# anneouyang/OuterSPACE

Hardware: AMD Instinct MI355X
Metric: spgemm_output_nnz_per_s (higher is better)
Workload: dtype f64

## Files before the change

### __graft_entry__.py

```python
import os
import subprocess
import sys

ROOT = os.path.dirname(os.path.abspath(__file__))
if ROOT not in sys.path:
    sys.path.insert(0, ROOT)


def build():
    subprocess.run(["make", "-C", os.path.join(ROOT, "outerspace_amd", "csrc"), "all"], check=True)
    subprocess.run(["make", "-C", os.path.join(ROOT, "oracle"), "all"], check=True)
    import outerspace_amd
    from outerspace_amd import _lib
    L = _lib.lib()
    missing = [s for s in _lib.EXPORTS + _lib.MASKED_EXPORTS + _lib.MCL_EXPORTS + _lib.APPLY_MASK_EXPORTS + _lib.SELECT_EXPORTS + _lib.EWISE_EXPORTS
               if not hasattr(L, s)]
    if missing:
        raise RuntimeError(f"library lacks exported symbols: {missing}")


def smoke():
    import numpy as np
    os.environ.setdefault("OSP_DIRECT_MIN_NNZ", "0")
    from outerspace_amd import generators as gen
    from outerspace_amd import spgemm as S
    from oracle import oracle

    n, rows, cols, vals = gen.rmat_coo(9, 8, "g500", seed=3)
    acsc = S.coo_to_csc(n, rows, cols, vals)
    bcsr = S.coo_to_csr(n, cols, rows, vals)
    with S.Context(0) as ctx:
        res = ctx.spgemm_csc_csr(n, n, n, *acsc, *bcsr)
        want = oracle.port().spgemm(n, n, n, *acsc, *bcsr)
        assert res.info["partials"] == want["partials"], (res.info["partials"], want["partials"])
        assert np.array_equal(res.rowptr, want["rowptr"]), "rowptr differs from the oracle"
        assert np.array_equal(res.colidx, want["colidx"]), "colidx differs from the oracle"
        assert np.array_equal(res.vals, want["vals"]), "values differ from the oracle"
        print(f"smoke ok: n={n} nnzA={len(rows)} P={res.info['partials']} nnzC={res.nnz} "
              f"heavy_rows={res.info['heavy_rows']} ms={res.info['ms_total']:.3f}")
        res.close()


if __name__ == "__main__":
    build()
    if len(sys.argv) > 1 and sys.argv[1] == "smoke":
        smoke()
```

### outerspace_amd/_lib.py

```python
import ctypes as C
import os

_HERE = os.path.dirname(os.path.abspath(__file__))
LIB_PATH = os.environ.get("OSP_LIBRARY") or os.path.join(_HERE, "libouterspace_spgemm.so")

OSP_F32, OSP_F64 = 0, 1
OSP_HOST, OSP_DEVICE = 0, 1
OSP_OK = 0
ERR_DIM, ERR_ARG, ERR_ALLOC, ERR_HIP, ERR_IO, ERR_RANGE, ERR_CAPACITY, ERR_UNSORTED = 1, 2, 3, 4, 5, 6, 7, 8
ERR_DUPLICATE = 233


class OspError(RuntimeError):
    def __init__(self, status, message):
        super().__init__(f"[osp status {status}] {message}")
        self.status = status


class _Stats(C.Structure):

    def as_dict(self):
        return {name: getattr(self, name) for name, _ in self._fields_ if name != "reserved"}


# ... 92 lines not shown

class Semiring(_Stats):
    _fields_ = [("add", C.c_int32), ("mul", C.c_int32), ("reserved", C.c_uint32 * 8)]


class MxmStats(_Stats):
    _fields_ = [("nnz_a", C.c_uint64), ("nnz_b", C.c_uint64), ("products", C.c_uint64), ("nnz_out", C.c_uint64),
                ("short_rows", C.c_uint64), ("long_rows", C.c_uint64), ("batches", C.c_uint32), ("launches", C.c_uint32),
                ("ms_total", C.c_float), ("reserved", C.c_uint32 * 7)]

MXV_ADD_OPS = {name: EWISE_OPS[name] for name in ("plus", "min", "max")}


class MxvStats(_Stats):
    _fields_ = [("nnz_in", C.c_uint64), ("nnz_out", C.c_uint64), ("long_segments", C.c_uint64), ("group", C.c_uint32),
                ("launches", C.c_uint32), ("ms_total", C.c_float), ("reserved", C.c_uint32 * 7)]

MXD_MAX_COLS = 65536


class MxdStats(_Stats):
    _fields_ = [("nnz_in", C.c_uint64), ("nnz_out", C.c_uint64), ("cols", C.c_uint64), ("long_segments", C.c_uint64),
                ("lanes_per_row", C.c_uint32), ("launches", C.c_uint32), ("ms_total", C.c_float), ("reserved", C.c_uint32 * 7)]

class Transpose(_Stats):
    _fields_ = [("reserved", C.c_uint32 * 8)]


class TransposeStats(_Stats):
    _fields_ = [("nnz", C.c_uint64), ("path", C.c_uint32), ("passes", C.c_uint32), ("launches", C.c_uint32), ("ms_total", C.c_float),
                ("reserved", C.c_uint32 * 6)]

class Extract(_Stats):
    _fields_ = [("rows", C.c_void_p), ("n_rows", C.c_uint64), ("cols", C.c_void_p), ("n_cols", C.c_uint64), ("space", C.c_int32),
                ("reserved", C.c_uint32 * 7)]


class ExtractStats(_Stats):
    _fields_ = [("nnz_in", C.c_uint64), ("nnz_gathered", C.c_uint64), ("nnz_out", C.c_uint64), ("ms_total", C.c_float),
                ("launches", C.c_uint32), ("readbacks", C.c_uint32), ("reserved", C.c_uint32 * 5)]

DUP_OPS = {"error": 0, "plus": 1, "min": 2, "max": 3, "first": 4, "last": 5, "count": 6}


class Build(_Stats):
    _fields_ = [("M", C.c_uint64), ("N", C.c_uint64), ("nnz", C.c_uint64), ("rows", C.c_void_p), ("cols", C.c_void_p), ("vals", C.c_void_p),
                ("dtype", C.c_int32), ("space", C.c_int32), ("dup", C.c_int32), ("reserved", C.c_uint32 * 7)]


class BuildStats(_Stats):
    _fields_ = [("nnz_in", C.c_uint64), ("nnz_out", C.c_uint64), ("long_runs", C.c_uint64), ("ms_total", C.c_float),
                ("launches", C.c_uint32), ("readbacks", C.c_uint32), ("reserved", C.c_uint32 * 5)]

PANEL_FN = C.CFUNCTYPE(C.c_int, C.POINTER(Panel), C.c_void_p)

MULTI_MAX_RANKS = 16


class MultiRankInfo(_Stats):
    _fields_ = [("device", C.c_int), ("k_begin", C.c_uint64), ("k_end", C.c_uint64), ("row_begin", C.c_uint64), ("row_end", C.c_uint64),
                ("partials_local", C.c_uint64), ("records_received", C.c_uint64), ("bytes_sent", C.c_uint64), ("nnz_c", C.c_uint64),
                ("ms_symbolic", C.c_float), ("ms_multiply_kernel", C.c_float), ("ms_merge", C.c_float), ("ms_total", C.c_float),
                ("bytes_to", C.c_uint64 * MULTI_MAX_RANKS), ("copy_streams", C.c_int), ("max_copies_outstanding", C.c_int),
                ("max_copies_in_flight", C.c_int), ("ms_exchange", C.c_float)]


class MultiInfo(_Stats):
    _fields_ = [("nranks", C.c_int), ("subpanels", C.c_int), ("M", C.c_uint64), ("K", C.c_uint64), ("N", C.c_uint64),
                ("nnz_c", C.c_uint64), ("partials", C.c_uint64), ("bytes_exchanged", C.c_uint64), ("ms_total", C.c_float),
                ("ms_upload", C.c_float), ("rank", MultiRankInfo * MULTI_MAX_RANKS)]

    def as_dict(self):
        d = {name: getattr(self, name) for name, _ in self._fields_ if name != "rank"}
        d["ranks"] = [{n: (list(getattr(self.rank[g], n))[:self.nranks] if n == "bytes_to" else getattr(self.rank[g], n))
                       for n, _ in MultiRankInfo._fields_} for g in range(self.nranks)]
        return d


EXPORTS = [
    "osp_context_create", "osp_context_create_on_stream", "osp_context_destroy", "osp_context_trim",
    "osp_config_default", "osp_last_error_string", "osp_status_string", "osp_spgemm_csc_csr", "osp_spgemm_csc_csr_panels",
    "osp_spgemm_coo", "osp_spgemm_csc_csr_aos", "osp_context_alloc", "osp_context_free",
    "osp_spgemm_partials", "osp_result_partials", "osp_merge_record_parts",
    "osp_merge_csr_parts", "osp_result_info", "osp_result_copy_csr", "osp_result_device_ptrs",
    "osp_result_destroy", "osp_mtx_read", "osp_host_free", "osp_coo_to_compressed_f32",
    "osp_coo_to_compressed_f64", "osp_spgemm_mtx", "osp_result_write_mtx", "osp_csr_bias_relu", "osp_result_coo_rows",
    "osp_stream_copy_probe", "osp_im2col_csc", "osp_spgemm_conv2d", "osp_csr_maxpool2d",
    "osp_multi_context_create", "osp_multi_context_destroy", "osp_multi_operands_create", "osp_multi_operands_destroy", "osp_spgemm_multi",
    "osp_spgemm_csc_csr_multi", "osp_multi_result_info", "osp_multi_result_shard", "osp_multi_result_copy_csr", "osp_multi_result_destroy",
]

MASKED_EXPORTS = ["osp_spgemm_masked"]

MCL_EXPORTS = ["osp_csr_inflate_prune"]

APPLY_MASK_EXPORTS = ["osp_csr_apply_mask"]

SELECT_EXPORTS = ["osp_csr_select"]

EWISE_EXPORTS = ["osp_csr_ewise"]

VECTOR_EXPORTS = ["osp_csr_reduce", "osp_csr_apply_vectors", "osp_csr_select_vertices"]

MXM_EXPORTS = ["osp_csr_mxm"]

TRANSPOSE_EXPORTS = ["osp_csr_transpose"]

MXV_EXPORTS = ["osp_csr_mxv"]

MXD_EXPORTS = ["osp_csr_mxd"]

EXTRACT_EXPORTS = ["osp_csr_extract"]

BUILD_EXPORTS = ["osp_csr_build"]

_lib = None


def lib():
    global _lib
    if _lib is not None:
        return _lib
    if not os.path.exists(LIB_PATH):
        raise ImportError(f"{LIB_PATH} not found: build it with `make -C outerspace_amd/csrc` "
                          "(or `python -c 'import __graft_entry__ as g; g.build()'`). "
                          "There is no CPU fallback.")
    try:
        import torch
    except ImportError:
        pass
    L = C.CDLL(LIB_PATH)
    vp, u64, i32 = C.c_void_p, C.c_uint64, C.c_int
    L.osp_last_error_string.restype = C.c_char_p
    L.osp_status_string.restype = C.c_char_p
    L.osp_status_string.argtypes = [i32]
    L.osp_context_create.argtypes = [i32, C.POINTER(vp)]
    L.osp_context_create_on_stream.argtypes = [i32, vp, C.POINTER(vp)]
    L.osp_context_destroy.argtypes = [vp]
    L.osp_context_trim.argtypes = [vp]
    L.osp_context_alloc.argtypes = [vp, u64, C.POINTER(vp)]
    L.osp_context_free.argtypes = [vp, vp]
    L.osp_spgemm_csc_csr_aos.argtypes = [vp, i32, u64, u64, u64, vp, vp, vp, vp, i32, C.POINTER(Config), C.POINTER(vp)]
    L.osp_config_default.argtypes = [C.POINTER(Config)]
    L.osp_config_default.restype = None
    L.osp_spgemm_csc_csr.argtypes = [vp, i32, u64, u64, u64, vp, vp, vp, vp, vp, vp, i32,
                                     C.POINTER(Config), C.POINTER(vp)]
    L.osp_spgemm_csc_csr_panels.argtypes = [vp, i32, u64, u64, u64, vp, vp, vp, vp, vp, vp, i32, C.POINTER(Config), PANEL_FN, vp,
                                            C.POINTER(ResultInfo)]
    L.osp_spgemm_coo.argtypes = [vp, i32, u64, u64, u64, u64, vp, vp, vp, u64, vp, vp, vp, i32, C.POINTER(Config), C.POINTER(vp)]
    L.osp_spgemm_partials.argtypes = [vp, i32, u64, u64, u64, vp, vp, vp, vp, vp, vp, i32, C.POINTER(Config), C.POINTER(vp)]
    L.osp_result_partials.argtypes = [vp, C.POINTER(vp), C.POINTER(vp)]
    L.osp_merge_record_parts.argtypes = [vp, i32, u64, u64, i32, C.POINTER(vp), C.POINTER(vp), i32, C.POINTER(Config), C.POINTER(vp)]
    L.osp_merge_csr_parts.argtypes = [vp, i32, u64, u64, i32, C.POINTER(vp), C.POINTER(vp),
                                      C.POINTER(vp), i32, C.POINTER(Config), C.POINTER(vp)]
    L.osp_result_info.argtypes = [vp, C.POINTER(ResultInfo)]
    L.osp_result_copy_csr.argtypes = [vp, vp, vp, vp, i32]
    L.osp_result_device_ptrs.argtypes = [vp, C.POINTER(vp), C.POINTER(vp), C.POINTER(vp)]
    L.osp_result_destroy.argtypes = [vp]
    L.osp_mtx_read.argtypes = [C.c_char_p, i32, C.POINTER(u64), C.POINTER(u64), C.POINTER(u64),
                               C.POINTER(vp), C.POINTER(vp), C.POINTER(vp)]
    L.osp_host_free.argtypes = [vp]
    L.osp_host_free.restype = None
    for sfx in ("f32", "f64"):
        getattr(L, f"osp_coo_to_compressed_{sfx}").argtypes = [i32, u64, u64, vp, vp, vp, vp, vp, vp]
    L.osp_spgemm_mtx.argtypes = [vp, i32, C.c_char_p, C.c_char_p, i32, C.POINTER(Config), C.POINTER(vp)]
    L.osp_result_write_mtx.argtypes = [vp, C.c_char_p]
    L.osp_stream_copy_probe.argtypes = [vp, u64, i32, C.POINTER(C.c_double)]
    L.osp_multi_context_create.argtypes = [C.POINTER(i32), i32, C.POINTER(vp)]
    L.osp_multi_context_destroy.argtypes = [vp]
    L.osp_multi_operands_create.argtypes = [vp, i32, u64, u64, u64, vp, vp, vp, vp, vp, vp, C.POINTER(vp)]
    L.osp_multi_operands_destroy.argtypes = [vp]
    L.osp_spgemm_multi.argtypes = [vp, vp, C.POINTER(Config), C.POINTER(vp)]
    L.osp_spgemm_csc_csr_multi.argtypes = [C.POINTER(i32), i32, i32, u64, u64, u64, vp, vp, vp, vp, vp, vp, C.POINTER(Config), C.POINTER(vp),
                                           C.POINTER(vp)]
    L.osp_multi_result_info.argtypes = [vp, C.POINTER(MultiInfo)]
    L.osp_multi_result_shard.argtypes = [vp, i32, C.POINTER(u64), C.POINTER(u64), C.POINTER(vp)]
    L.osp_multi_result_copy_csr.argtypes = [vp, vp, vp, vp]
    L.osp_multi_result_destroy.argtypes = [vp]
    L.osp_csr_bias_relu.argtypes = [vp, vp, i32, i32, C.POINTER(vp)]
    L.osp_result_coo_rows.argtypes = [vp, vp]
    L.osp_im2col_csc.argtypes = [vp, i32, u64, u64, u64, u64, u64, vp, vp, vp, i32, C.POINTER(Conv2dGeometry), i32, C.POINTER(u64),
                                 vp, vp, vp]
    L.osp_spgemm_conv2d.argtypes = [vp, i32, u64, u64, u64, u64, u64, vp, vp, vp, u64, u64, vp, vp, vp, i32, C.POINTER(Conv2dGeometry),
                                    C.POINTER(Config), C.POINTER(vp)]
    u32 = C.c_uint32
    L.osp_csr_maxpool2d.argtypes = [vp, u64, u64, u64, u32, u32, u32, u32, C.POINTER(vp)]
    L.osp_spgemm_masked.argtypes = [vp, i32, u64, u64, u64, vp, vp, vp, vp, vp, vp, vp, vp, i32, C.POINTER(Config), C.POINTER(vp)]
    L.osp_csr_inflate_prune.argtypes = [vp, C.POINTER(MclStep), i32, C.POINTER(vp), C.POINTER(MclStats)]
    L.osp_csr_apply_mask.argtypes = [vp, u64, u64, vp, vp, i32, i32, i32, C.POINTER(vp), C.POINTER(ApplyMaskStats)]
    L.osp_csr_select.argtypes = [vp, C.POINTER(Select), C.POINTER(vp), C.POINTER(SelectStats)]
    L.osp_csr_ewise.argtypes = [vp, vp, C.POINTER(Ewise), C.POINTER(vp), C.POINTER(EwiseStats)]
    L.osp_csr_reduce.argtypes = [vp, i32, i32, vp, i32, C.POINTER(VectorStats)]
    L.osp_csr_apply_vectors.argtypes = [vp, C.POINTER(VectorApply), vp, vp, i32, C.POINTER(vp), C.POINTER(VectorStats)]
    L.osp_csr_select_vertices.argtypes = [vp, vp, vp, i32, C.POINTER(vp), C.POINTER(VectorStats)]
    L.osp_csr_mxm.argtypes = [vp, vp, C.POINTER(Semiring), C.POINTER(vp), C.POINTER(MxmStats)]
    L.osp_csr_transpose.argtypes = [vp, C.POINTER(Transpose), C.POINTER(vp), C.POINTER(TransposeStats)]
    L.osp_csr_mxv.argtypes = [vp, C.POINTER(Semiring), vp, vp, i32, C.POINTER(MxvStats)]
    L.osp_csr_mxd.argtypes = [vp, C.POINTER(Semiring), vp, u64, vp, i32, C.POINTER(MxdStats)]
    L.osp_csr_extract.argtypes = [vp, C.POINTER(Extract), C.POINTER(vp), C.POINTER(ExtractStats)]
    L.osp_csr_build.argtypes = [vp, C.POINTER(Build), C.POINTER(vp), C.POINTER(BuildStats)]
    _lib = L
    return L


def check(status):
    if status != OSP_OK:
        raise OspError(status, lib().osp_last_error_string().decode(errors="replace"))
```

### outerspace_amd/csrc/osp_api.hip

```cpp
#include <hip/hip_runtime.h>

#include <algorithm>
#include <cmath>
#include <cstdarg>
#include <cstdio>
#include <cstdlib>
#include <chrono>
#include <cstring>
#include <functional>
#include <limits>
#include <map>
#include <memory>
#include <string>
#include <vector>

#include "../../include/outerspace_spgemm.h"
#include "../../include/outerspace_spgemm_masked.h"
#include "../../include/outerspace_spgemm_mcl.h"
#include "../../include/outerspace_spgemm_apply_mask.h"
#include "../../include/outerspace_spgemm_select.h"
#include "../../include/outerspace_spgemm_ewise.h"
#include "../../include/outerspace_spgemm_vector.h"
#include "../../include/outerspace_spgemm_mxm.h"
#include "../../include/outerspace_spgemm_transpose.h"
#include "../../include/outerspace_spgemm_mxv.h"
#include "../../include/outerspace_spgemm_mxd.h"
#include "../../include/outerspace_spgemm_extract.h"
#include "../../include/outerspace_spgemm_build.h"
#include "osp_internal.h"
#include "osp_kernels.h"
#include "osp_split.h"
#include "osp_sort.h"
#include "osp_epilogue.h"
#include "osp_conv.h"
#include "osp_masked.h"
#include "osp_mcl.h"
#include "osp_apply_mask.h"
#include "osp_select.h"
#include "osp_ewise.h"
#include "osp_vector.h"
#include "osp_mxm.h"
#include "osp_transpose.h"
#include "osp_mxv.h"
#include "osp_mxd.h"
#include "osp_extract.h"
#include "osp_build.h"

namespace osp {


#define OSP_HIP(expr)                                                                      \
    do {                                                                                   \
        hipError_t e_ = (expr);                                                            \
        if (e_ != hipSuccess)                                                              \
            throw Error(e_ == hipErrorOutOfMemory ? OSP_ERR_ALLOC : OSP_ERR_HIP,           \
                        std::string(#expr) + ": " + hipGetErrorString(e_));                \
    } while (0)

#include "osp_context.h"
#include "osp_pipeline.h"

template <class T>
static const T *to_device(Scratch &sc, const T *p, uint64_t n, osp_memspace_t space, hipStream_t s) {
    if (space == OSP_DEVICE || n == 0) return p;
    T *d = sc.get<T>(n);
    copy_h2d(d, p, n * sizeof(T), s);
    return d;
}

static void check_flags(uint32_t f, const char *what) {
    if (f & kFlagPtr) throw Error(OSP_ERR_ARG, std::string(what) + ": pointer array is not a monotone 0..nnz sequence");
    if (f & kFlagRange) throw Error(OSP_ERR_RANGE, std::string(what) + ": index outside its dimension");
    if (f & kFlagDuplicate) throw Error(OSP_ERR_DUPLICATE, std::string(what) + ": duplicate coordinate (reference: throw(233))");
    if (f & kFlagUnsorted) throw Error(OSP_ERR_UNSORTED, std::string(what) + ": indices inside a segment are not ascending");
}

static void finish_timing(Result *res, EventPair &ev, PhaseTimer &tm, hipStream_t s) {
    OSP_HIP(hipEventRecord(ev.b, s));
    OSP_HIP(hipStreamSynchronize(s));
    osp_result_info_t &i = res->info;
    i.ms_total = ev.ms();
    i.ms_symbolic = tm.total(PH_SYM);
    i.ms_multiply = tm.total(PH_MUL);
    i.ms_merge = tm.total(PH_MERGE);
    i.ms_compact = tm.total(PH_COMPACT);
    i.ms_multiply_kernel = tm.total(PH_MUL_K);
    i.ms_merge_kernel = tm.total(PH_MERGE_K);
    i.ms_split_kernel = tm.total(PH_SPLIT_K);
    i.ms_direct_plan_kernel = tm.total(PH_PLAN_K);
    i.ms_hub_plan_kernel = tm.total(PH_HUB_K);
    i.ms_expand_kernel = tm.total(PH_EXPAND_K);
}

__global__ void count_partials_kernel(const int64_t *a_colptr, const int64_t *b_rowptr, uint64_t K, unsigned long long *out) {
    __shared__ uint64_t scratch[256 / kWave + 1];
    uint64_t sum = 0;
    for (uint64_t k = (uint64_t)blockIdx.x * blockDim.x + threadIdx.x; k < K; k += (uint64_t)gridDim.x * blockDim.x)
        sum += (uint64_t)(a_colptr[k + 1] - a_colptr[k]) * (uint64_t)(b_rowptr[k + 1] - b_rowptr[k]);
    uint64_t total;
    block_excl_scan<uint64_t, 256>(sum, scratch, &total);
    if (threadIdx.x == 0 && total) atomicAdd(out, (unsigned long long)total);
}

template <class T>
static void spgemm_impl(Context *ctx, Result *res, uint64_t M, uint64_t K, uint64_t N, const int64_t *a_colptr_in,
                        const uint32_t *a_rowidx_in, const T *a_vals_in, const int64_t *b_rowptr_in,
                        const uint32_t *b_colidx_in, const T *b_vals_in, osp_memspace_t space,
                        const osp_config_t &cfg, const PanelSink *sink = nullptr, bool partials_only = false) {
    hipStream_t s = ctx->stream;
    Scratch sc(ctx);
    PhaseTimer tm(s);
    EventPair ev;
    OSP_HIP(hipEventRecord(ev.a, s));
// ... 68 lines not shown
            const uint64_t nsample = (k1 - k0 + stride - 1) / stride;
            if (nnz) row_work_kernel<<<grid_for(nsample * kWave, 256), 256, 0, s>>>(a_colptr, a_rowidx, b_rowptr, k0, k1, stride, work);
            device_exclusive_scan<LoadU64, uint64_t>(LoadU64{(const uint64_t *)work}, M, pre, tmp, s);
            device_exclusive_scan<RowCost, uint64_t>(RowCost{pre, (uint64_t)TileCap<T>::value, kSplitRowMax}, M, cost_pre, tmp, s);
            shard_bounds_kernel<<<grid_for(G + 1, 64), 64, 0, s>>>(cost_pre, pre, M, G, d_b, d_b + G + 1);
            std::vector<uint64_t> h_b(2ull * (G + 1));
            copy_d2h(h_b.data(), d_b, h_b.size() * sizeof(uint64_t), s);
            r_lo = h_b[cfg.row_shard_index];
            r_hi = h_b[cfg.row_shard_index + 1];
        }
        int64_t *colptr2 = sc.get<int64_t>(K + 1);
        uint64_t nnz2 = 0;
        uint32_t *rowidx2 = nullptr;
        T *vals2 = nullptr;
        {
            Scratch cs(ctx);
            uint32_t *keep_scan = cs.get<uint32_t>(nnz + 1);
            uint32_t *tmp = cs.get<uint32_t>(scan_scratch_entries(nnz + 1));
            const RowInRange keep{a_rowidx + e0, (uint32_t)r_lo, r_hi};
            device_exclusive_scan<RowInRange, uint32_t>(keep, nnz, keep_scan, tmp, s);
            nnz2 = d2h(keep_scan + nnz, s);
            rowidx2 = sc.get<uint32_t>(nnz2);
            vals2 = sc.get<T>(nnz2);
            restrict_colptr_kernel<<<grid_for(K + 1, 256), 256, 0, s>>>(a_colptr, K, e0, nnz, keep_scan, colptr2);
            if (nnz2) restrict_compact_kernel<T><<<grid_for(nnz, 256), 256, 0, s>>>(keep, keep_scan, nnz, a_vals + e0, rowidx2, vals2);
        }
        tm.end(PH_SYM);
        a_colptr = colptr2; a_rowidx = rowidx2; a_vals = vals2;
        e0 = 0;
        e1 = (int64_t)nnz2;
    }
    const uint64_t nnz = (uint64_t)(e1 - e0);

    tm.begin(PH_SYM);
    uint64_t *row_off = sc.get<uint64_t>(M + 1);
    uint64_t *chunk_off = sc.get<uint64_t>(nnz);
    uint64_t P = 0;
    const int algo = cfg.algorithm;
    if (algo != OSP_ALGO_OUTER && algo != OSP_ALGO_ROWWISE) throw Error(OSP_ERR_ARG, "unknown algorithm");
    const bool rowwise = algo == OSP_ALGO_ROWWISE && nnz && (uint64_t)nnz_b < 0xffffffffull && nnz < 0xffffffffull && !partials_only;
    ChunkTable<T> ct{};
    const uint64_t direct_min_nnz = getenv("OSP_DIRECT_MIN_NNZ") ? strtoull(getenv("OSP_DIRECT_MIN_NNZ"), nullptr, 10) : ((getenv("OSP_GATHER") && atoi(getenv("OSP_GATHER")) == 0) ? (8ull << 20) : (2ull << 20));
    const bool dense_avg = (long double)p_all * 8.0L >= 3.0L * (long double)M * (long double)N;
    const bool direct = nnz && (nnz >= direct_min_nnz || dense_avg) && (uint64_t)nnz_b < 0xffffffffull && nnz < 0xffffffffull && !partials_only &&
                        !(getenv("OSP_DIRECT") && atoi(getenv("OSP_DIRECT")) == 0);
    const uint64_t direct_max = std::min<uint64_t>(getenv("OSP_DIRECT_MAX") ? strtoull(getenv("OSP_DIRECT_MAX"), nullptr, 10) : kSplitRowMax,
                                                   kDirectDenseMax);
    const int gather_env = getenv("OSP_GATHER") ? atoi(getenv("OSP_GATHER")) : 2;
    const bool gather_ok = nnz && !rowwise && !partials_only && (uint64_t)nnz_b < 0xffffffffull && nnz < 0xffffffffull;
    const bool gather_short = gather_ok && gather_env >= 2 && direct;
    ShortRuns<T> srun{};
    DirectSrc dsrc{};
    uint32_t n_long_rows = 1;
    if (nnz == 0) {
        OSP_HIP(hipMemsetAsync(row_off, 0, (M + 1) * sizeof(uint64_t), s));
    } else {
        Scratch ss(ctx);
        Scratch &keep = (rowwise || direct || gather_short) ? sc : ss;
        const RowSort rs(ss, nnz, std::max(1, bits_for(M)));
        uint32_t *rows_sorted = (gather_short ? keep : ss).template get<uint32_t>(nnz), *perm = keep.get<uint32_t>(nnz), *w_sorted = ss.get<uint32_t>(nnz);
        uint32_t *bs_sorted = (rowwise || direct || gather_short) ? keep.get<uint32_t>(nnz) : nullptr;
        uint32_t *rowfirst = keep.get<uint32_t>(M + 1);
        uint64_t *offs_sorted = keep.get<uint64_t>(nnz + 1);
        uint64_t *scan_tmp = ss.get<uint64_t>(scan_scratch_entries(std::max<uint64_t>(nnz, M + 1)));
        const bool table = rowwise || direct || gather_short;
        const bool with_av = gather_ok && gather_env >= 1 && (direct || gather_short);
        T *av_sorted = with_av ? keep.get<T>(nnz) : nullptr;
        uint32_t *w = ss.get<uint32_t>(with_av ? 4 * nnz : table ? 2 * nnz : nnz);
        uint32_t *bs = table ? w : nullptr;
        sym_chunk_len_kernel<<<grid_for(nnz, 256), 256, 0, s>>>(a_colptr, b_rowptr, k0, k1, e0, nnz, w, bs,
                                                                with_av ? reinterpret_cast<const uint32_t *>(a_vals) : nullptr, (uint32_t)(sizeof(T) / 4));
        SymEpilogue sym_ep{w, bs, rows_sorted, perm, w_sorted, bs_sorted};
        if (with_av) { sym_ep.av_sorted = av_sorted; sym_ep.vwords = (uint32_t)(sizeof(T) / 4); }
        rs.sort(a_rowidx + e0, sym_ep);
        device_exclusive_scan<LoadU32As64, uint64_t>(LoadU32As64{w_sorted}, nnz, offs_sorted, scan_tmp, s);
        sym_row_offsets_kernel<<<grid_for(M + 1, 256), 256, 0, s>>>(rows_sorted, offs_sorted, nnz, M, row_off, rowfirst);
        const uint64_t rw_cap = (rowwise || gather_short) ? (uint64_t)TileCap<T>::value : 0ull;
        const bool expand_rows_on = gather_short && !(getenv("OSP_EXPAND_ROWS") && atoi(getenv("OSP_EXPAND_ROWS")) == 0);
        if (!expand_rows_on) sym_scatter_offsets_kernel<<<grid_for(nnz, 256), 256, 0, s>>>(perm, offs_sorted, rows_sorted, row_off, rw_cap, nnz, chunk_off);
        if (partials_only || rowwise || row_sharded) P = d2h(offs_sorted + nnz, s);
        else P = kPartialsOnDevice;
        if (direct) {
            dsrc = DirectSrc{rowfirst, offs_sorted, bs_sorted, perm, b_colidx, chunk_off, direct_max};
            dsrc.b_rowptr = b_rowptr; dsrc.K = K; dsrc.nnz_b = (uint64_t)nnz_b; dsrc.keep = &sc;
            dsrc.gather = gather_ok && gather_env >= 1;
            dsrc.expand_rows = expand_rows_on;
            if (expand_rows_on) { dsrc.chunk_off_ready = false; dsrc.rows_sorted = rows_sorted; dsrc.row_off = row_off; dsrc.rw_cap = rw_cap; dsrc.nnz = nnz; }
            dsrc.a_vals = with_av ? (const void *)av_sorted : (const void *)(a_vals + e0); dsrc.av_in_order = with_av; dsrc.b_vals = b_vals;
            if (dsrc.gather) {
                dsrc.gstat = (unsigned long long *)sc.get<uint64_t>(3);
                zero_async(s, {{dsrc.gstat, 3 * sizeof(uint64_t)}});
            }
        }
        if (gather_short) {
            const ShortRunFlag sf{offs_sorted};
            uint32_t *cidx = ss.get<uint32_t>(nnz + 1), *cidx_tmp = ss.get<uint32_t>(scan_scratch_entries(nnz + 1));
            device_exclusive_scan<ShortRunFlag, uint32_t>(sf, nnz, cidx, cidx_tmp, s);
            RunDesc<T> *runs0 = sc.get<RunDesc<T>>(nnz);
            uint32_t *rowfirst0 = sc.get<uint32_t>(M + 1);
            short_runs_kernel<T><<<grid_for(nnz, 256), 256, 0, s>>>(sf, cidx, nnz, bs_sorted, av_sorted, runs0);
            short_rowfirst_kernel<<<grid_for(M + 1, 256), 256, 0, s>>>(rowfirst, cidx, M, rowfirst0);
            srun = ShortRuns<T>{runs0, rowfirst0, b_colidx, b_vals};
        }
        if (rowwise) {
            ct = ChunkTable<T>{offs_sorted, bs_sorted, perm, rowfirst, a_vals + e0, b_colidx, b_vals, (uint32_t)rw_cap, 1u};
            uint32_t *flag_scan = ss.get<uint32_t>(M + 1);
            device_exclusive_scan<HeavyRowFlag, uint32_t>(HeavyRowFlag{row_off, 0, (uint32_t)rw_cap}, M, flag_scan, (uint32_t *)scan_tmp, s);
            n_long_rows = d2h(flag_scan + M, s);
        }
    }
    tm.end(PH_SYM);
    res->info.partials = P;

    OuterProducer<T> prod;
    prod.ctx = ctx; prod.res = res;
    prod.a_colptr = a_colptr; prod.a_rowidx = a_rowidx; prod.a_vals = a_vals;
    prod.b_rowptr = b_rowptr; prod.b_colidx = b_colidx; prod.b_vals = b_vals;
    prod.k0 = k0; prod.k1 = k1; prod.e0 = e0; prod.chunk_off = chunk_off;
    const uint64_t nk = k1 - k0;
    prod.a_start = sc.get<int64_t>(nk); prod.a_cnt = sc.get<uint32_t>(nk);
    prod.prod = sc.get<uint64_t>(nk); prod.prod_off = sc.get<uint64_t>(nk + 1);
    prod.scan_tmp = sc.get<uint64_t>(scan_scratch_entries(nk));
    prod.nothing_staged = rowwise && n_long_rows == 0;
    prod.short_gathered = gather_short;
    if ((dsrc.gather || gather_short) && nnz && !partials_only) {
        prod.nnz = nnz;
        prod.kscan = sc.get<uint32_t>(nnz + 1);
        prod.kscan_tmp = sc.get<uint32_t>(scan_scratch_entries(std::max<uint64_t>(nnz, k1 - k0) + 1));
        prod.elist = sc.get<uint32_t>(nnz);
        prod.cscan = sc.get<uint32_t>(k1 - k0 + 1);
        prod.klist = sc.get<uint32_t>(k1 - k0 + 1);
    }

    if (partials_only) {
        if (row_sharded) throw Error(OSP_ERR_ARG, "partial products of a row shard are not supported");
        res->partials = true;
        res->rowptr = (int64_t *)ctx->alloc((M + 1) * sizeof(int64_t));
        OSP_HIP(hipMemcpyAsync(res->rowptr, row_off, (M + 1) * sizeof(uint64_t), hipMemcpyDeviceToDevice, s));
        res->vals = ctx->alloc(std::max<uint64_t>(P, 1) * sizeof(Part<T>));
        res->info.panels = 1;
        res->info.nnz_c = P;
        res->info.row_begin = 0;
        res->info.row_end = M;
        tm.begin(PH_MUL);
        if (P) prod.produce(0, M, true, 0, P, (Part<T> *)res->vals, tm, nullptr, nullptr);
        tm.end(PH_MUL);
        finish_timing(res, ev, tm, s);
        return;
    }
    const uint64_t off_lo = 0, P_rows = P;
    merge_pipeline<T>(ctx, res, prod, M, N, row_off, P_rows, cfg.partial_capacity, tm, r_lo, r_hi, off_lo, sink,
                      rowwise ? &ct : nullptr, (direct && nnz) ? &dsrc : nullptr, nullptr, gather_short ? &srun : nullptr);

    finish_timing(res, ev, tm, s);
    if (gather_short) res->info.gathered_short_partials = res->info.partials - res->info.heavy_partials;
    if (dsrc.gstat && res->info.direct_rows) {
        uint64_t gs[3] = {0, 0, 0};
        copy_d2h(gs, dsrc.gstat, sizeof(gs), s);
        res->info.gathered_rows = gs[0]; res->info.gathered_partials = gs[1]; res->info.gathered_runs = gs[2];
    }
    if (getenv("OSP_VERBOSE")) {
        fprintf(stderr, "[osp] product done in %.1f ms; pool misses so far: %llu hipMalloc calls, %.1f GB, %.1f ms\n", res->info.ms_total,
                (unsigned long long)ctx->malloc_calls, ctx->malloc_bytes / 1e9, ctx->malloc_ms);
    }
}

template <class T>
static void coo_to_compressed_device(Context *ctx, Scratch &sc, uint64_t nseg, uint64_t ninner, uint64_t nnz, const uint32_t *seg,
                                     const uint32_t *inner, const T *vals, const char *what, int64_t **ptr_out,
                                     uint32_t **idx_out, T **val_out) {
    hipStream_t s = ctx->stream;
    int64_t *ptr = sc.get<int64_t>(nseg + 1);
    uint32_t *idx = sc.get<uint32_t>(nnz);
    T *ov = sc.get<T>(nnz);
    *ptr_out = ptr; *idx_out = idx; *val_out = ov;
    if (nnz == 0) {
        OSP_HIP(hipMemsetAsync(ptr, 0, (nseg + 1) * sizeof(int64_t), s));
        return;
    }
    Scratch ss(ctx);
    uint32_t *flags = ss.get<uint32_t>(1);
    OSP_HIP(hipMemsetAsync(flags, 0, sizeof(uint32_t), s));
    const CooOrder o = coo_sort_two_keys(ss, nnz, inner, std::max(1, bits_for(ninner)), seg, std::max(1, bits_for(nseg)));
    ingest_finish_kernel<T><<<grid_for(nnz, 256), 256, 0, s>>>(o.outer_sorted, o.perm, inner, vals, nnz, nseg, ninner, idx, ov, flags);
    ingest_ptr_kernel<<<grid_for(nseg + 1, 256), 256, 0, s>>>(o.outer_sorted, nnz, nseg, ptr);
    check_flags(d2h(flags, s), what);
}

template <class T>
static void spgemm_coo_impl(Context *ctx, Result *res, uint64_t M, uint64_t K, uint64_t N, uint64_t nnz_a, const uint32_t *a_rows,
                            const uint32_t *a_cols, const T *a_vals, uint64_t nnz_b, const uint32_t *b_rows, const uint32_t *b_cols,
                            const T *b_vals, osp_memspace_t space, const osp_config_t &cfg) {
    hipStream_t s = ctx->stream;
    Scratch sc(ctx);
    EventPair ev;
    OSP_HIP(hipEventRecord(ev.a, s));
    const uint32_t *ar = to_device(sc, a_rows, nnz_a, space, s), *ac = to_device(sc, a_cols, nnz_a, space, s);
    const uint32_t *br = to_device(sc, b_rows, nnz_b, space, s), *bc = to_device(sc, b_cols, nnz_b, space, s);
    const T *av = to_device(sc, a_vals, nnz_a, space, s), *bv = to_device(sc, b_vals, nnz_b, space, s);
    int64_t *ap, *bp;
    uint32_t *ai, *bi;
    T *acv, *bcv;
    coo_to_compressed_device<T>(ctx, sc, K, M, nnz_a, ac, ar, av, "A (COO)", &ap, &ai, &acv);
    coo_to_compressed_device<T>(ctx, sc, K, N, nnz_b, br, bc, bv, "B (COO)", &bp, &bi, &bcv);
    OSP_HIP(hipEventRecord(ev.b, s));
// ... 712 lines not shown
        on_device(ctx, [&] {
            const ConvGeom g = conv_geometry(N, C, H, W, geom);
            hipStream_t s = ctx->stream;
            Scratch sc(ctx);
            with_type(dtype, [&](auto tag) {
                using T = decltype(tag);
                const uint32_t *xr = to_device(sc, x_rows, nnz_x, space, s), *xc = to_device(sc, x_cols, nnz_x, space, s);
                const T *xv = to_device(sc, (const T *)x_vals, nnz_x, space, s);
                T *va = (T *)a_vals;
                *nnz_a = im2col_impl<T>(ctx, sc, N, C, g, nnz_x, xr, xc, xv, fill, a_colptr, a_rowidx, va);
            });
        });
        return OSP_OK;
    });
}

int osp_spgemm_conv2d(osp_context_t ctx_, osp_dtype_t dtype, uint64_t N, uint64_t C, uint64_t H, uint64_t W, uint64_t nnz_x,
                      const uint32_t *x_rows, const uint32_t *x_cols, const void *x_vals, uint64_t OC, uint64_t nnz_w,
                      const uint32_t *w_rows, const uint32_t *w_cols, const void *w_vals, osp_memspace_t space,
                      const osp_conv2d_geometry_t *geom, const osp_config_t *cfg_, osp_result_t *result) {
    Context *ctx = (Context *)ctx_;
    if (!ctx || !result) return fail(OSP_ERR_ARG, "null context or result pointer");
    if ((nnz_x && (!x_rows || !x_cols || !x_vals)) || (nnz_w && (!w_rows || !w_cols || !w_vals))) return fail(OSP_ERR_ARG, "null operand array");
    return guard([&] {
        check_dtype(dtype); check_space(space);
        if (!OC || OC > 0xffffffffull || nnz_x >= 0xffffffffull || nnz_w >= 0xffffffffull)
            throw Error(OSP_ERR_ARG, "OC must be >= 1; OC or nnz exceeds the u32 index type");
        const osp_config_t cfg = config_or_default(cfg_);
        return new_result(ctx, dtype, result, [&](auto tag, Result *res) {
            using T = decltype(tag);
            const ConvGeom g = conv_geometry(N, C, H, W, geom);
            spgemm_conv2d_impl<T>(ctx, res, N, C, g, nnz_x, x_rows, x_cols, (const T *)x_vals, OC, nnz_w, w_rows, w_cols, (const T *)w_vals,
                                  space, cfg);
        });
    });
}

int osp_csr_maxpool2d(osp_result_t in_, uint64_t N, uint64_t H, uint64_t W, uint32_t kh, uint32_t kw, uint32_t stride_h,
                      uint32_t stride_w, osp_result_t *out) {
    Result *in = (Result *)in_;
    if (!in || !out) return fail(OSP_ERR_ARG, "null argument");
    if (in->partials) return fail(OSP_ERR_ARG, "a result of osp_spgemm_partials holds records, not a CSR");
    if (!N || !H || !W || !kh || !kw || !stride_h || !stride_w) return fail(OSP_ERR_ARG, "sizes, kernel and stride must be >= 1");
    if (H < kh || W < kw) return fail(OSP_ERR_ARG, "the pooling window is larger than the input: empty output");
    if (H >= 0xffffffffull || W >= 0xffffffffull || (unsigned __int128)N * H * W != in->info.M)
        return fail(OSP_ERR_ARG, "N*H*W must equal the rows of the input");
    return guard([&] {
        return new_result(in->ctx, in->dtype, out, [&](auto tag, Result *res) {
            maxpool_impl<decltype(tag)>(in->ctx, in, res, N, (uint32_t)H, (uint32_t)W, kh, kw, stride_h, stride_w);
        });
    });
}

int osp_stream_copy_probe(osp_context_t ctx_, uint64_t bytes, int reps, double *gbps) {
    Context *ctx = (Context *)ctx_;
    if (!ctx || !gbps) return fail(OSP_ERR_ARG, "null argument");
    if (bytes < 4096 || reps < 1 || reps > 1000) return fail(OSP_ERR_ARG, "bytes >= 4096, 1 <= reps <= 1000");
    return guard([&]() -> int {
        OSP_HIP(hipSetDevice(ctx->device));
        hipStream_t s = ctx->stream;
        Scratch sc(ctx);
        const uint64_t n = bytes / sizeof(u32x4);
        u32x4 *src = sc.get<u32x4>(n), *dst = sc.get<u32x4>(n);
        OSP_HIP(hipMemsetAsync(src, 0x5a, n * sizeof(u32x4), s));
        if (n > 0xffffffffull * 256ull) return fail(OSP_ERR_ARG, "probe buffer too large");
        const unsigned grid = (unsigned)((n + 255) / 256);
        double best = 0;
        for (int nt = 0; nt < 2; nt++) {
            for (int i = 0; i < 2; i++) {
                if (nt) stream_copy_kernel<true><<<grid, 256, 0, s>>>(src, dst, n); else stream_copy_kernel<false><<<grid, 256, 0, s>>>(src, dst, n);
            }
            EventPair ev;
            OSP_HIP(hipEventRecord(ev.a, s));
            for (int i = 0; i < reps; i++) {
                if (nt) stream_copy_kernel<true><<<grid, 256, 0, s>>>(src, dst, n); else stream_copy_kernel<false><<<grid, 256, 0, s>>>(src, dst, n);
            }
            OSP_HIP(hipEventRecord(ev.b, s));
            OSP_HIP(hipStreamSynchronize(s));
            OSP_HIP(hipGetLastError());
            const double ms = ev.ms();
            if (ms > 0) best = std::max(best, 2.0 * (double)(n * sizeof(u32x4)) * reps / (ms * 1e-3) / 1e9);
        }
        *gbps = best;
        return OSP_OK;
    });
}

int osp_multi_context_create(const int *devices, int ndev, osp_multi_context_t *out) {
    if (!devices || !out) return fail(OSP_ERR_ARG, "null argument");
    if (ndev < 1 || ndev > OSP_MULTI_MAX_RANKS) return fail(OSP_ERR_ARG, "between 1 and %d ranks", OSP_MULTI_MAX_RANKS);
    return guard([&]() -> int {
        std::unique_ptr<MultiContext> mc(new MultiContext);
        for (int g = 0; g < ndev; g++) {
            osp_context_t c = nullptr;
            const int st = osp_context_create(devices[g], &c);
            if (st) return st;
            mc->devices.push_back(devices[g]);
            mc->ctx.push_back((Context *)c);
            mc->copy.emplace_back((size_t)ndev, nullptr);
            mc->mctx.push_back(nullptr);
            osp_context_t c2 = nullptr;
            const int st2 = osp_context_create(devices[g], &c2);
            if (st2) return st2;
            mc->mctx.back() = (Context *)c2;
            mc->ctx.back()->sibling = mc->mctx.back();
            mc->mctx.back()->sibling = mc->ctx.back();
// ... 182 lines not shown
```

### outerspace_amd/csrc/osp_context.h

```cpp
#pragma once

struct Context {
    int device = 0;
    hipStream_t stream = nullptr;
    bool own_stream = false;
    hipStream_t aux = nullptr;
    hipEvent_t aux_fork = nullptr, aux_join = nullptr;
    void need_aux() {
        if (aux) return;
        if (hipStreamCreateWithFlags(&aux, hipStreamNonBlocking) != hipSuccess) { aux = nullptr; throw Error(OSP_ERR_HIP, "hipStreamCreate failed"); }
        if (hipEventCreateWithFlags(&aux_fork, hipEventDisableTiming) != hipSuccess || hipEventCreateWithFlags(&aux_join, hipEventDisableTiming) != hipSuccess) {
            drop_aux();
            throw Error(OSP_ERR_HIP, "hipEventCreate failed");
        }
    }
    bool fork_window = false;
    uint64_t releases_in_fork_window = 0;
    void drop_aux() {
        if (aux) { (void)hipStreamSynchronize(aux); (void)hipStreamDestroy(aux); aux = nullptr; }
        if (aux_fork) { (void)hipEventDestroy(aux_fork); aux_fork = nullptr; }
        if (aux_join) { (void)hipEventDestroy(aux_join); aux_join = nullptr; }
    }
    std::multimap<size_t, void *> free_list;
    std::map<void *, size_t> live;
// ... 331 lines not shown
    for (size_t off = 0; off < bytes; off += chunk, i ^= 1) {
        const size_t n = std::min(chunk, bytes - off);
        OSP_HIP(hipMemcpyAsync(pb.p + i * chunk, (const char *)src + off, n, hipMemcpyDeviceToHost, s));
        OSP_HIP(hipEventRecord(pb.done[i], s));
        if (have_prev) {
            OSP_HIP(hipEventSynchronize(pb.done[i ^ 1]));
            memcpy((char *)dst + off_prev, pb.p + (i ^ 1) * chunk, n_prev);
        }
        off_prev = off; n_prev = n; have_prev = true;
    }
    OSP_HIP(hipEventSynchronize(pb.done[i ^ 1]));
    memcpy((char *)dst + off_prev, pb.p + (i ^ 1) * chunk, n_prev);
}
struct ZeroRegions {
    uint32_t *p[4];
    uint64_t words[4];
    uint32_t val[4];
};
__global__ void zero_regions_kernel(const ZeroRegions z) {
#pragma unroll
    for (int r = 0; r < 4; r++)
        for (uint64_t i = (uint64_t)blockIdx.x * blockDim.x + threadIdx.x; i < z.words[r]; i += (uint64_t)gridDim.x * blockDim.x) z.p[r][i] = z.val[r];
}
struct FillRegion { void *p; size_t bytes; uint32_t word; };
static void fill_async(hipStream_t s, std::initializer_list<FillRegion> regions) {
    ZeroRegions z{};
    int n = 0;
    uint64_t most = 0;
    for (auto &r : regions) {
        if (n == 4 || (r.bytes & 3) || ((uintptr_t)r.p & 3)) throw Error(OSP_ERR_ARG, "fill_async: at most four word-aligned regions");
        z.p[n] = (uint32_t *)r.p;
        z.words[n] = r.bytes / 4;
        z.val[n] = r.word;
        most = std::max<uint64_t>(most, z.words[n]);
        n++;
    }
    if (most == 0) return;
    zero_regions_kernel<<<(unsigned)std::min<uint64_t>((most + 255) / 256, 2048), 256, 0, s>>>(z);
}
static void zero_async(hipStream_t s, std::initializer_list<std::pair<void *, size_t>> regions) {
    ZeroRegions z{};
    int n = 0;
    uint64_t most = 0;
    for (auto &r : regions) {
        if (n == 4 || (r.second & 3) || ((uintptr_t)r.first & 3)) throw Error(OSP_ERR_ARG, "zero_async: at most four word-aligned regions");
        z.p[n] = (uint32_t *)r.first;
        z.words[n] = r.second / 4;
        most = std::max<uint64_t>(most, z.words[n]);
        n++;
    }
    if (most == 0) return;
    zero_regions_kernel<<<(unsigned)std::min<uint64_t>((most + 255) / 256, 2048), 256, 0, s>>>(z);
}
constexpr int kGatherMax = 24;
struct GatherSrcs {
    const void *p[kGatherMax];
    uint8_t bytes[kGatherMax];
};
__global__ void gather_scalars_kernel(const GatherSrcs g, int n, uint64_t *out) {
    const int i = threadIdx.x;
    if (i < n) out[i] = g.bytes[i] == 8 ? *static_cast<const uint64_t *>(g.p[i]) : (uint64_t) * static_cast<const uint32_t *>(g.p[i]);
}
struct Gather {
    hipStream_t s;
    Pinned &pb;
    GatherSrcs srcs;
    void *dst[kGatherMax];
    int n = 0;
    explicit Gather(hipStream_t st) : s(st), pb(pinned_buffer()) { pb.reserve(4096); }
    template <class T> void add(T *host_dst, const T *dptr) {
        static_assert(sizeof(T) == 4 || sizeof(T) == 8, "read-backs are 32- or 64-bit scalars");
        if (n == kGatherMax) throw Error(OSP_ERR_ARG, "too many values in one read-back");
        srcs.p[n] = dptr;
        srcs.bytes[n] = (uint8_t)sizeof(T);
        dst[n++] = host_dst;
    }
    void wait() {
        if (n == 0) return;
        uint64_t *pin = reinterpret_cast<uint64_t *>(pb.p);
        if (n >= 3) {
            if (!pb.collect) OSP_HIP(hipMalloc((void **)&pb.collect, kGatherMax * sizeof(uint64_t)));
            gather_scalars_kernel<<<1, kWave, 0, s>>>(srcs, n, pb.collect);
            OSP_HIP(hipMemcpyAsync(pin, pb.collect, n * sizeof(uint64_t), hipMemcpyDeviceToHost, s));
        } else {
            for (int i = 0; i < n; i++) OSP_HIP(hipMemcpyAsync(pin + i, srcs.p[i], srcs.bytes[i], hipMemcpyDeviceToHost, s));
        }
        OSP_HIP(hipStreamSynchronize(s));
        for (int i = 0; i < n; i++) memcpy(dst[i], pin + i, srcs.bytes[i]);
        n = 0;
    }
};
template <class T> static T d2h(const T *dptr, hipStream_t s) {
    T v;
    copy_d2h(&v, dptr, sizeof(T), s);
    return v;
}
```

### outerspace_amd/csrc/osp_kernels.h

```cpp
#pragma once
#include <type_traits>
#include "osp_prims.h"

namespace osp {

template <class T> struct TileCap;
#ifndef OSP_TILE_CAP_F32
#define OSP_TILE_CAP_F32 1792
#endif
template <> struct TileCap<float> { static constexpr int value = OSP_TILE_CAP_F32; };
#ifndef OSP_TILE_CAP_F64
#define OSP_TILE_CAP_F64 1536
#endif
template <> struct TileCap<double> { static constexpr int value = OSP_TILE_CAP_F64; };
constexpr int kMergeThreads = 256;
constexpr int kTileMaxRows = kMergeThreads - 1;
constexpr int kMulThreads = 256;
#ifndef OSP_MUL_PER_WAVE
#define OSP_MUL_PER_WAVE 2048
#endif
constexpr int kMulPerWave = OSP_MUL_PER_WAVE;
constexpr int kMulPerBlock = kMulPerWave * (kMulThreads / kWave);
#ifndef OSP_MUL_BATCH_MAX
#define OSP_MUL_BATCH_MAX 4096
// ... 168 lines not shown
                                       uint64_t *row_off, uint32_t *rowfirst) {
    uint64_t i = (uint64_t)blockIdx.x * blockDim.x + threadIdx.x;
    if (i > M) return;
    uint64_t t = lower_bound_dev(rows_sorted, 0, nnz, (uint64_t)i);
    row_off[i] = offs_sorted[t];
    rowfirst[i] = (uint32_t)t;
}
struct LenGatherW {
    const uint32_t *w;
    const uint32_t *perm;
    __device__ uint32_t operator()(uint64_t t) const { return w[perm[t]]; }
};

__global__ void panel_columns_kernel(const int64_t *a_colptr, const uint32_t *a_rowidx,
                                     const int64_t *b_rowptr, uint64_t k0, uint64_t nk, uint32_t r0,
                                     uint64_t r1, int whole, int64_t *a_start, uint32_t *a_cnt,
                                     uint64_t *prod) {
    uint64_t t = (uint64_t)blockIdx.x * blockDim.x + threadIdx.x;
    if (t >= nk) return;
    uint64_t k = k0 + t;
    uint64_t lo = (uint64_t)a_colptr[k], hi = (uint64_t)a_colptr[k + 1];
    if (!whole) {
        uint64_t l2 = lower_bound_dev(a_rowidx, lo, hi, (uint64_t)r0);
        hi = lower_bound_dev(a_rowidx, l2, hi, r1);
        lo = l2;
    }
    a_start[t] = (int64_t)lo;
    a_cnt[t] = (uint32_t)(hi - lo);
    prod[t] = (hi - lo) * (uint64_t)(b_rowptr[k + 1] - b_rowptr[k]);
}
__global__ void panel_bounds_kernel(const uint64_t *row_off, uint64_t r_lo, uint64_t M, uint64_t cap, const uint64_t *cuts, uint32_t ncuts,
                                    uint32_t maxp, uint64_t *out) {
    const uint64_t *off = row_off + r_lo;
    uint64_t r = 0, bad = ~0ull;
    uint32_t p = 0, ci = 0;
    if (lane_id() == 0) { out[2] = r_lo; out[2 + maxp + 1] = off[0]; }
    while (r < M) {
        if (p == maxp) { bad = r_lo + r; break; }
        uint64_t r1 = wave_upper_bound(off, r, M + 1, off[r] + cap) - 1;
        if (r1 <= r) { bad = r_lo + r; break; }
        r1 = min(r1, M);
        while (ci < ncuts && cuts[ci] <= r_lo + r) ci++;
        if (ci < ncuts && cuts[ci] < r_lo + r1) r1 = cuts[ci] - r_lo;
        p++;
        if (lane_id() == 0) { out[2 + p] = r_lo + r1; out[2 + maxp + 1 + p] = off[r1]; }
        r = r1;
    }
    if (lane_id() == 0) { out[0] = p; out[1] = bad; }
}
struct LoadU64 {
    const uint64_t *p;
    __device__ uint64_t operator()(uint64_t i) const { return p[i]; }
};
struct PanelKeepFlag {
    const uint32_t *a_rowidx; const uint64_t *chunk_off; int64_t e0; uint32_t r0; uint64_t r1; uint32_t desc_only;
    __device__ uint32_t operator()(uint64_t t) const {
        const uint32_t r = a_rowidx[(uint64_t)e0 + t];
        if (!(r >= r0 && (uint64_t)r < r1)) return 0u;
        const uint64_t off = chunk_off[t];
        return (off != ~0ull && (!desc_only || (off >> 63))) ? 1u : 0u;
    }
};
__global__ void panel_keep_list_kernel(PanelKeepFlag f, const uint32_t *kscan, uint64_t nnz, uint32_t *elist) {
    const uint64_t t = (uint64_t)blockIdx.x * blockDim.x + threadIdx.x;
    if (t < nnz && f(t)) elist[kscan[t]] = (uint32_t)((uint64_t)f.e0 + t);
}
struct PanelKeepColFlag {
    const int64_t *a_colptr; int64_t e0; uint64_t k0; const uint32_t *kscan;
    __device__ uint32_t operator()(uint64_t t) const { return kscan[a_colptr[k0 + t + 1] - e0] != kscan[a_colptr[k0 + t] - e0] ? 1u : 0u; }
};
__global__ void panel_keep_columns_kernel(const int64_t *a_colptr, const int64_t *b_rowptr, uint64_t k0, uint64_t nk, int64_t e0,
                                          const uint32_t *kscan, const uint32_t *cscan, int64_t *a_start, uint32_t *a_cnt, uint64_t *prod,
                                          uint32_t *klist) {
    const uint64_t t = (uint64_t)blockIdx.x * blockDim.x + threadIdx.x;
    if (t >= nk) return;
    const uint64_t k = k0 + t;
    const uint32_t lo = kscan[a_colptr[k] - e0], hi = kscan[a_colptr[k + 1] - e0];
    const uint32_t ncol = cscan[nk];
    if (t >= ncol) { a_start[t] = 0; a_cnt[t] = 0; prod[t] = 0; klist[t] = (uint32_t)k0; }
    if (hi == lo) return;
    const uint32_t j = cscan[t];
    a_start[j] = (int64_t)lo;
    a_cnt[j] = hi - lo;
    prod[j] = (uint64_t)(hi - lo) * (uint64_t)(b_rowptr[k + 1] - b_rowptr[k]);
    klist[j] = (uint32_t)k;
}

__device__ __forceinline__ uint32_t wave_bcast(uint32_t v, uint32_t src) { return (uint32_t)__builtin_amdgcn_readlane((int)v, (int)src); }
__device__ __forceinline__ uint64_t wave_bcast(uint64_t v, uint32_t src) {
    return ((uint64_t)wave_bcast((uint32_t)(v >> 32), src) << 32) | wave_bcast((uint32_t)v, src);
}
__device__ __forceinline__ float wave_bcast(float v, uint32_t src) { return __uint_as_float(wave_bcast(__float_as_uint(v), src)); }
__device__ __forceinline__ double wave_bcast(double v, uint32_t src) {
    return __longlong_as_double((long long)wave_bcast((uint64_t)__double_as_longlong(v), src));
}

constexpr uint64_t kDirectBit = 1ull << 63;
__device__ __forceinline__ uint64_t direct_desc(uint32_t rowbase, uint32_t celloff, uint32_t sh) {
    return kDirectBit | ((uint64_t)(sh & 31u) << 58) | ((uint64_t)(celloff & 0x3ffffffu) << 32) | (uint64_t)rowbase;
}
constexpr uint64_t kHubCellMask = (1ull << 58) - 1ull;
__device__ __forceinline__ uint64_t hub_desc(uint64_t first_cell) { return kDirectBit | (31ull << 58) | (first_cell & kHubCellMask); }
__device__ __forceinline__ bool is_hub_desc(uint64_t desc) { return ((uint32_t)(desc >> 58) & 31u) == 31u; }
struct HubArgs {
    const uint32_t *cells = nullptr;
    const uint32_t *sx = nullptr;
// ... 403 lines not shown
                            [&](uint64_t i, uint32_t col, T val) { stream_store_part(&stage[i - base], col, val); });
}

struct CoarseStartFlag {
    const uint64_t *row_off;
    uint64_t r0, base, slot;
    const uint8_t *force;
    __device__ uint32_t operator()(uint64_t t) const {
        if (t == 0) return 1;
        const uint64_t r = r0 + t;
        if (force && force[t]) return 1;
        return ((row_off[r] - base) / slot != (row_off[r - 1] - base) / slot || (t & 0xffffu) == 0) ? 1u : 0u;
    }
};
__global__ void tile_walk_kernel(const uint32_t *cb_rows, const uint32_t *ncb_p, uint32_t ncb_max, uint64_t r_end, const uint64_t *row_off,
                                 uint64_t cap, uint32_t max_rows, const uint32_t *tile_base, uint32_t *counts,
                                 uint32_t *tile_rows) {
    const uint32_t j = blockIdx.x * blockDim.x + threadIdx.x;
    const uint32_t ncb = *ncb_p;
    if (j >= ncb) {
        if (!tile_rows && j < ncb_max) counts[j] = 0;
        return;
    }
    uint64_t r = cb_rows[j];
    const uint64_t end = (j + 1 < ncb) ? (uint64_t)cb_rows[j + 1] : r_end;
    uint32_t n = 0;
    const uint32_t out = tile_rows ? tile_base[j] : 0u;
    while (r < end) {
        if (tile_rows) tile_rows[out + n] = (uint32_t)r;
        const uint64_t lim = min(end, r + max_rows);
        uint64_t r2 = upper_bound_dev(row_off, r + 1, lim + 1, row_off[r] + cap) - 1;
        if (r2 <= r) r2 = r + 1;
        r = r2;
        n++;
    }
    if (!tile_rows) counts[j] = n;
}
struct HeavyRowFlag {
    const uint64_t *row_off;
    uint64_t r0;
    uint32_t kTileCap;
    __device__ uint32_t operator()(uint64_t t) const {
        const uint64_t r = r0 + t;
        return (row_off[r + 1] - row_off[r]) > (uint64_t)kTileCap ? 1u : 0u;
    }
};
template <class F>
__global__ void compact_flagged_kernel(F f, const uint32_t *scan, uint64_t n, uint64_t r0,
                                       uint32_t *list) {
    uint64_t t = (uint64_t)blockIdx.x * blockDim.x + threadIdx.x;
    if (t < n && f(t)) list[scan[t]] = (uint32_t)(r0 + t);
}

constexpr uint64_t kStatusAgg = 1ull << 62, kStatusPrefix = 2ull << 62, kStatusMask = (1ull << 62) - 1;

#ifndef OSP_RUN_SHORT
#define OSP_RUN_SHORT 16
#endif
constexpr int kRunShort = OSP_RUN_SHORT;
template <class T> __device__ __forceinline__ T index_as_value(uint32_t i);
template <> __device__ __forceinline__ float index_as_value<float>(uint32_t i) { return __uint_as_float(i); }
template <> __device__ __forceinline__ double index_as_value<double>(uint32_t i) { return __longlong_as_double((long long)i); }
__device__ __forceinline__ uint32_t value_as_index_impl(float v) { return __float_as_uint(v); }
__device__ __forceinline__ uint32_t value_as_index_impl(double v) { return (uint32_t)__double_as_longlong(v); }
template <class T> __device__ __forceinline__ uint32_t value_as_index(T v) { return value_as_index_impl(v); }
#ifndef OSP_DIGIT_BITS
#define OSP_DIGIT_BITS 10
#endif
constexpr int kDigitBits = OSP_DIGIT_BITS;
constexpr int kDigits = 1 << kDigitBits;

template <class T, int NT, int CAP = TileCap<T>::value>
struct alignas(8) MergeSmem {
    static constexpr int kTileCap = CAP;
    static_assert(CAP % 4 == 0, "the value area behind key0/pos0 must stay 8-byte aligned");
    static_assert(sizeof(T) <= 8, "values alias 8 bytes per entry");
    static constexpr bool kWide = sizeof(T) == 8;
#ifndef OSP_HASH_IN_CNT
#define OSP_HASH_IN_CNT 1
#endif
    static constexpr uint32_t kHashWords = (kWide ? (uint32_t)CAP * 5u / 2u : (uint32_t)CAP * 2u) +
                                           (OSP_HASH_IN_CNT ? (kWide ? 0u : 2u) + (uint32_t)(NT / kWave) * (1u << OSP_DIGIT_BITS) / 2u : 0u);
    uint32_t key0[CAP];
    uint16_t pos0[CAP];
    uint16_t pad[kWide ? CAP : 4];
    uint32_t key1[CAP];
    uint16_t pos1[CAP];
    union {
        uint16_t cnt[NT / kWave][kDigits];
        uint16_t rank[CAP + 1];
    };
    uint32_t rowo[kTileMaxRows + 1];
    uint32_t gbits[CAP / 32];
    uint32_t scratch[NT / kWave + 1];
    uint32_t nlongrun;
    uint32_t hcount;
    uint64_t excl;
    __device__ __forceinline__ uint32_t *key(int c) { return c ? key1 : key0; }
    __device__ __forceinline__ uint16_t *pos(int c) { return c ? pos1 : pos0; }
    __device__ __forceinline__ T *vals(int c) {
        return reinterpret_cast<T *>(c ? reinterpret_cast<char *>(key0) : kWide ? reinterpret_cast<char *>(pad) : reinterpret_cast<char *>(key1));
    }
    __device__ __forceinline__ uint32_t *htab() { return reinterpret_cast<uint32_t *>(pos0); }
    static constexpr int kMaxLong = CAP / kRunShort;
    static constexpr size_t kLongOff = ((CAP + 1) * sizeof(uint16_t) + 7) / 8 * 8;
    static_assert(kLongOff + kMaxLong * (sizeof(T) + sizeof(uint16_t)) <= sizeof(uint16_t) * (NT / kWave) * kDigits, "long-run list: behind rank, inside the counters");
    __device__ __forceinline__ T *long_sum() { return reinterpret_cast<T *>(reinterpret_cast<char *>(cnt) + kLongOff); }
    __device__ __forceinline__ uint16_t *long_pos() { return reinterpret_cast<uint16_t *>(reinterpret_cast<char *>(cnt) + kLongOff + kMaxLong * sizeof(T)); }
};

template <int BITS>
__device__ __forceinline__ void wave_match_digit(unsigned digit, bool valid, unsigned &rank, unsigned &count) {
    const uint64_t vm = __ballot(valid);
    uint32_t plo = (uint32_t)vm, phi = (uint32_t)(vm >> 32);
#pragma unroll
    for (int b = 0; b < BITS; b++) {
        const uint32_t bit = (digit >> b) & 1u;
        const uint64_t m = __ballot(bit != 0);
        const uint32_t sbm = 0u - bit;
        plo &= ~((uint32_t)m ^ sbm);
        phi &= ~((uint32_t)(m >> 32) ^ sbm);
    }
    rank = __builtin_amdgcn_mbcnt_hi(phi, __builtin_amdgcn_mbcnt_lo(plo, 0u));
    count = __popc(plo) + __popc(phi);
}

__global__ __launch_bounds__(256) void rank_order_selftest_kernel(uint32_t *bad) {
    __shared__ uint32_t cnt[4][64];
    const unsigned tid = threadIdx.x, lane = lane_id(), w = tid >> 6;
    uint32_t x = 0x9E3779B9u * (blockIdx.x * 256u + tid + 1u), nbad = 0;
    for (int r = 0; r < 64; r++) {
        cnt[w][lane] = 0;
        for (int it = 0; it < 4; it++) {
            x ^= x << 13; x ^= x >> 17; x ^= x << 5;
            const unsigned dg = (x >> 9) & ((r & 1) ? 3u : 127u);
            const bool valid = ((x >> 27) & 7u) != 0;
            unsigned rk, c;
            wave_match_digit<7>(dg, valid, rk, c);
            const unsigned half = 16u * (dg & 1u);
            const uint32_t before = (cnt[w][dg >> 1] >> half) & 0xffffu;
            __builtin_amdgcn_wave_barrier();
            if (valid) {
                const uint32_t got = (atomicAdd(&cnt[w][dg >> 1], 1u << half) >> half) & 0xffffu;
                nbad += got != before + rk;
            }
        }
    }
    if (nbad) atomicAdd(bad, nbad);
}

constexpr int kLookWin = 1;
__device__ __forceinline__ void lookback_publish(uint64_t *status, uint32_t t, uint64_t total) {
    __hip_atomic_store(&status[t], (t == 0 ? kStatusPrefix : kStatusAgg) | total, __ATOMIC_RELAXED, __HIP_MEMORY_SCOPE_AGENT);
}
constexpr int kTicketStride = 32;
constexpr uint32_t kLookbackSpinLimit = 1u << 22;
__device__ __forceinline__ uint32_t take_ticket(uint32_t *ticket, uint32_t nshards, uint32_t &shard, uint32_t ntiles) {
    if (nshards <= 1) return atomicAdd(ticket, 1u);
    for (uint32_t tries = 0; tries < nshards; tries++) {
        const uint32_t n = atomicAdd(&ticket[shard * kTicketStride], 1u);
        const uint64_t t = (uint64_t)n * nshards + shard;
        if (t < ntiles) return (uint32_t)t;
        shard = shard + 1 == nshards ? 0u : shard + 1;
    }
    return ntiles;
}
template <bool PUBLISH = true>
__device__ __forceinline__ uint64_t lookback_prefix(uint64_t *status, uint32_t t, uint64_t total, uint32_t *abort_word = nullptr) {
    const unsigned lane = lane_id();
    if (PUBLISH && lane == 0) lookback_publish(status, t, total);
    uint64_t excl = 0;
    int64_t b = (int64_t)t - 1;
    uint32_t spins = 0;
    while (b >= 0) {
        uint64_t sv[kLookWin];
#pragma unroll
        for (int j = 0; j < kLookWin; j++) {
            const int64_t idx = b - (int64_t)(j * kWave) - (int64_t)lane;
            sv[j] = kStatusPrefix;
            if (idx >= 0) sv[j] = __hip_atomic_load(&status[idx], __ATOMIC_RELAXED, __HIP_MEMORY_SCOPE_AGENT);
        }
        bool done = false, retry = false;
        uint64_t part = 0;
#pragma unroll
        for (int j = 0; j < kLookWin; j++) {
            if (!done && !retry) {
                const uint64_t m_prefix = __ballot((sv[j] >> 62) == 2), m_empty = __ballot((sv[j] >> 62) == 0);
                const int p = m_prefix ? __builtin_ctzll(m_prefix) : 64;
                const uint64_t need = p >= 63 ? ~0ull : ((2ull << p) - 1ull);
                if (m_empty & need) {
                    retry = true;
                } else {
                    part += ((int)lane <= p) ? (sv[j] & kStatusMask) : 0ull;
                    if (p < 64) done = true;
                }
            }
        }
        if (retry) {
            __builtin_amdgcn_s_sleep(1);
            if (abort_word && (++spins & 255u) == 0) {
                if (spins >= kLookbackSpinLimit && lane == 0) atomicExch(abort_word, 1u);
                if (spins >= kLookbackSpinLimit || __hip_atomic_load(abort_word, __ATOMIC_RELAXED, __HIP_MEMORY_SCOPE_AGENT) != 0u) break;
            }
            continue;
        }
        excl += wave_reduce_sum_u62(part);
        if (done) break;
        b -= (int64_t)kLookWin * kWave;
    }
    if (lane == 0 && t != 0)
        __hip_atomic_store(&status[t], kStatusPrefix | (excl + total), __ATOMIC_RELAXED, __HIP_MEMORY_SCOPE_AGENT);
    return excl;
}

struct TileDesc {
    uint64_t s;
    uint32_t ra, nr, n, lvl;
    uint32_t cbase, kbits;
    uint32_t rbeg, rcnt;
};
constexpr uint32_t kNoRuns = 0xffffffffu;
template <class T> struct RunDesc;
template <> struct alignas(16) RunDesc<double> { uint32_t dst, src; double av; };
template <> struct alignas(4) RunDesc<float> { uint32_t dst, src; float av; };
template <class T>
struct GatherArgs {
    const RunDesc<T> *runs = nullptr;
    const RunDesc<T> *runs0 = nullptr;
    const uint32_t *b_colidx = nullptr;
    const T *b_vals = nullptr;
};
struct ShortRunFlag {
    const uint64_t *off;
    __device__ uint32_t operator()(uint64_t c) const { return off[c + 1] > off[c] ? 1u : 0u; }
};
template <class T>
__global__ void short_runs_kernel(ShortRunFlag f, const uint32_t *cidx, uint64_t nnz, const uint32_t *bs, const T *av_sorted, RunDesc<T> *runs0) {
    const uint64_t c = (uint64_t)blockIdx.x * blockDim.x + threadIdx.x;
    if (c >= nnz || !f(c)) return;
    RunDesc<T> rd;
    rd.dst = (uint32_t)f.off[c];
    rd.src = bs[c];
    rd.av = av_sorted[c];
    runs0[cidx[c]] = rd;
}
__global__ void short_rowfirst_kernel(const uint32_t *rowfirst, const uint32_t *cidx, uint64_t M, uint32_t *rowfirst0) {
    const uint64_t i = (uint64_t)blockIdx.x * blockDim.x + threadIdx.x;
    if (i <= M) rowfirst0[i] = cidx[rowfirst[i]];
}
struct SegExpandJobs {
    const uint32_t *seglist; const uint64_t *vrow_off; const uint32_t *vrun_off;
    __device__ uint64_t operator()(uint64_t t) const {
        const uint32_t v = seglist[t];
        if (vrun_off[v] == kNoRuns) return 0ull;
        return (vrow_off[v + 1] - vrow_off[v] + kExpandJob - 1) / kExpandJob;
    }
};
template <class T>
__global__ __launch_bounds__(kExpandThreads) void expand_segments_kernel(
    const uint32_t *__restrict__ seglist, uint32_t nseg, const uint64_t *__restrict__ jobbase, const uint64_t *__restrict__ vrow_off,
    const uint32_t *__restrict__ vrun_off, const uint32_t *__restrict__ vrun_end, const RunDesc<T> *__restrict__ runs,
    const uint32_t *__restrict__ b_colidx, const T *__restrict__ b_vals, Part<T> *__restrict__ qstage) {
    const unsigned lane = lane_id(), w = threadIdx.x >> 6;
    constexpr uint32_t NW = kExpandThreads / kWave, per = kExpandJob / NW, kUnroll = 4;
    const uint64_t njobs = jobbase[nseg];
// ... 1182 lines not shown
```

### outerspace_amd/csrc/osp_pipeline.h

```cpp
#pragma once

#define OSP_WITH_RA(ctx_, ...)                                               \
    do {                                                                     \
        if ((ctx_)->rank_atomic) { constexpr bool RA = true; __VA_ARGS__; }  \
        else { constexpr bool RA = false; __VA_ARGS__; }                     \
    } while (0)

template <class T> struct Producer {
    virtual ~Producer() {}
    virtual void produce(uint64_t r0, uint64_t r1, bool whole, uint64_t base, uint64_t count,
                         Part<T> *stage, PhaseTimer &tm, const uint32_t *cells = nullptr, Part<T> *qstage = nullptr,
                         const HubArgs *hub = nullptr, bool compact = false, bool has_long = true, bool desc_only = false, bool walk_all = false) = 0;
};

template <class T> struct MergeIO {
    Part<T> *stage;
    const uint64_t *row_off; uint64_t r0, r1, base;
    int64_t *c_rowptr; uint32_t *c_col; T *c_val;
    const uint64_t *out_in; uint64_t *out_out;
    ChunkTable<T> ct{};
    uint32_t *abort_word = nullptr;
    const RunDesc<T> *runs0 = nullptr; const uint32_t *rowfirst0 = nullptr; const uint32_t *b_colidx = nullptr; const T *b_vals = nullptr;
};
template <class T> struct ShortRuns {
    const RunDesc<T> *runs0 = nullptr; const uint32_t *rowfirst0 = nullptr; const uint32_t *b_colidx = nullptr; const T *b_vals = nullptr;
};

struct TilePlan {
    uint32_t *tile_rows = nullptr;
    uint32_t ntiles = 0;
    uint32_t *long_rows = nullptr;
    uint32_t nlong = 0;
};

static TilePlan plan_tiles(Context *ctx, Scratch &sc, const uint64_t *row_off, uint64_t r0, uint64_t r1, uint64_t base,
                           uint32_t cap, uint32_t max_rows, const uint8_t *force_start, uint64_t total, uint64_t nforce) {
    hipStream_t s = ctx->stream;
    const uint64_t nr = r1 - r0;
    TilePlan pl;
    uint32_t *flag_scan = sc.get<uint32_t>(nr + 1);
    uint32_t *tmp_rows = sc.get<uint32_t>(nr + 1);
    uint64_t *scan_tmp = sc.get<uint64_t>(scan_scratch_entries(std::max<uint64_t>(nr + 1, 16)));
    const uint64_t slot = 8ull * cap;
    CoarseStartFlag csf{row_off, r0, base, slot, force_start};
    device_exclusive_scan<CoarseStartFlag, uint32_t>(csf, nr, flag_scan, (uint32_t *)scan_tmp, s);
    compact_flagged_kernel<CoarseStartFlag><<<grid_for(nr, 256), 256, 0, s>>>(csf, flag_scan, nr, r0, tmp_rows);
    const uint32_t ncb = (uint32_t)std::min<uint64_t>(nr, 2 + nforce + total / slot + nr / 65536);
    const uint32_t *ncb_p = flag_scan + nr;
    uint32_t *cb_cnt = sc.get<uint32_t>((uint64_t)ncb + 1);
    tile_walk_kernel<<<grid_for(ncb, 128), 128, 0, s>>>(tmp_rows, ncb_p, ncb, r1, row_off, cap, max_rows, nullptr, cb_cnt, nullptr);
    device_exclusive_scan<LoadU32, uint32_t>(LoadU32{cb_cnt}, ncb, cb_cnt, (uint32_t *)scan_tmp, s);
    HeavyRowFlag hrf{row_off, r0, cap};
    uint32_t *long_scan = sc.get<uint32_t>(nr + 1);
    uint32_t *long_tmp = sc.get<uint32_t>(scan_scratch_entries(std::max<uint64_t>(nr + 1, 16)));
    device_exclusive_scan<HeavyRowFlag, uint32_t>(hrf, nr, long_scan, long_tmp, s);
    pl.long_rows = sc.get<uint32_t>(nr + 1);
    compact_flagged_kernel<HeavyRowFlag><<<grid_for(nr, 256), 256, 0, s>>>(hrf, long_scan, nr, r0, pl.long_rows);
    { Gather g(s); g.add(&pl.ntiles, (const uint32_t *)cb_cnt + ncb); g.add(&pl.nlong, (const uint32_t *)long_scan + nr); g.wait(); }
    pl.tile_rows = sc.get<uint32_t>((uint64_t)pl.ntiles + 1);
    tile_walk_kernel<<<grid_for(ncb, 128), 128, 0, s>>>(tmp_rows, ncb_p, ncb, r1, row_off, cap, max_rows, cb_cnt, nullptr, pl.tile_rows);
    return pl;
}

struct DirectSrc {
    const uint32_t *rowfirst; const uint64_t *off; const uint32_t *bs; const uint32_t *perm; const uint32_t *b_colidx;
    uint64_t *chunk_off;
    uint64_t direct_max;
    const int64_t *b_rowptr = nullptr;
    uint64_t K = 0, nnz_b = 0;
    Scratch *keep = nullptr;
    mutable HubTables hub{};
    mutable bool hub_refused = false;
    bool gather = false;
    bool expand_rows = false;
    mutable bool chunk_off_ready = true;
    const uint32_t *rows_sorted = nullptr;
    const uint64_t *row_off = nullptr;
    uint64_t rw_cap = 0, nnz = 0;
    void ensure_chunk_off(hipStream_t s) const {
        if (chunk_off_ready) return;
        sym_scatter_offsets_kernel<<<grid_for(nnz, 256), 256, 0, s>>>(perm, off, rows_sorted, row_off, rw_cap, nnz, chunk_off);
        chunk_off_ready = true;
    }
    const void *a_vals = nullptr, *b_vals = nullptr;
    bool av_in_order = false;
    unsigned long long *gstat = nullptr;
};

template <class T> struct PanelPlan {
    Scratch sc;
    TilePlan p0;
    uint32_t max_rows = 0;
    uint64_t *hoff = nullptr, *hscan_tmp = nullptr, *blkbase = nullptr, *hbase = nullptr, *vbase = nullptr, *cellbase = nullptr;
    uint8_t *hbits = nullptr, *hmode = nullptr;
    uint32_t *nstretch = nullptr;
    uint64_t nh = 0, nblocks = 0, nvirt = 0, ncell = 0;
    uint64_t mode_rows[3] = {0, 0, 0}, mode_partials[3] = {0, 0, 0};
    uint32_t *ghist = nullptr, *ghist_tmp = nullptr;
    Part<T> *qstage = nullptr;
    uint64_t *vrow_off = nullptr;
    uint8_t *vfirst = nullptr;
    uint32_t *vcol0 = nullptr, *vcol1 = nullptr;
    uint32_t *cells = nullptr;
    HubArgs hub{};
    GatherArgs<T> ga{};
    uint32_t *vrun_off = nullptr, *vrun_end = nullptr;
    uint32_t *nwritten = nullptr;
    uint64_t *xjobbase = nullptr;
    uint64_t xjobs_bound = 0, xpartials = 0;
    bool expand_ok = false;
    bool may_write = false;
    const DirectSrc *split_from_b = nullptr;
    bool split_beside = false;
    explicit PanelPlan(Context *c) : sc(c) {}
};

__global__ void mode_totals_kernel(const uint32_t *rows, uint32_t nlong, const uint64_t *row_off, const uint8_t *hmode,
                                   const uint8_t *hsmall, unsigned long long *totals) {
    uint64_t part[3] = {0, 0, 0}, cnt[3] = {0, 0, 0}, nsmall = 0;
    for (uint32_t h = blockIdx.x * blockDim.x + threadIdx.x; h < nlong; h += gridDim.x * blockDim.x) {
        const uint64_t U = row_off[rows[h] + 1] - row_off[rows[h]];
        const uint8_t m = hmode[h];
        nsmall += hsmall[h] ? 1ull : 0ull;
#pragma unroll
        for (int mode = 0; mode < 3; mode++) { part[mode] += m == mode ? U : 0ull; cnt[mode] += m == mode ? 1ull : 0ull; }
    }
    for (uint8_t mode = 0; mode < 3; mode++) {
        const uint64_t p = wave_reduce_sum<uint64_t>(part[mode]), c = wave_reduce_sum<uint64_t>(cnt[mode]);
        if (lane_id() == 0 && c) { atomicAdd(&totals[mode], (unsigned long long)c); atomicAdd(&totals[3 + mode], (unsigned long long)p); }
    }
    nsmall = wave_reduce_sum<uint64_t>(nsmall);
    if (lane_id() == 0 && nsmall) atomicAdd(&totals[6], (unsigned long long)nsmall);
}

template <class T>
static void plan_panel(Context *ctx, Result *res, PhaseTimer &tm, PanelPlan<T> &pl, const uint64_t *row_off, uint64_t r0, uint64_t r1,
                       uint64_t base, uint64_t count, int colbits, const DirectSrc *ds) {
    hipStream_t s = ctx->stream;
    Scratch &sc = pl.sc;
    constexpr uint32_t kCap = (uint32_t)TileCap<T>::value;
    pl.max_rows = (uint32_t)std::min<uint64_t>(kTileMaxRows, colbits >= 32 ? 1ull : (1ull << (32 - colbits)));
    pl.p0 = plan_tiles(ctx, sc, row_off, r0, r1, base, kCap, pl.max_rows, nullptr, count, 0);
    res->info.light_tiles += pl.p0.ntiles - pl.p0.nlong;
    if (!pl.p0.nlong) return;
    const uint32_t nlong = pl.p0.nlong;
    pl.hoff = sc.get<uint64_t>((uint64_t)nlong + 1);
    pl.hscan_tmp = sc.get<uint64_t>(scan_scratch_entries(nlong));
    device_exclusive_scan<HeavyLen, uint64_t>(HeavyLen{pl.p0.long_rows, row_off}, nlong, pl.hoff, pl.hscan_tmp, s);
    pl.hbits = sc.get<uint8_t>(nlong);
    pl.hmode = sc.get<uint8_t>(nlong);
    pl.nstretch = sc.get<uint32_t>(nlong);
    uint32_t *nseg = sc.get<uint32_t>(nlong);
    uint64_t *nhist = sc.get<uint64_t>(nlong), *ncellh = sc.get<uint64_t>(nlong);
    const bool want_gather = ds && ds->gather;
    uint64_t *nrund = want_gather ? sc.get<uint64_t>(nlong) : nullptr, *rdbase = want_gather ? sc.get<uint64_t>((uint64_t)nlong + 1) : nullptr;
    uint64_t nrd = 0;
    pl.blkbase = sc.get<uint64_t>((uint64_t)nlong + 1); pl.hbase = sc.get<uint64_t>((uint64_t)nlong + 1);
    pl.vbase = sc.get<uint64_t>((uint64_t)nlong + 1); pl.cellbase = sc.get<uint64_t>((uint64_t)nlong + 1);
    unsigned long long *totals = (unsigned long long *)sc.get<uint64_t>(7);
    uint8_t *hsmall = sc.get<uint8_t>(nlong);
    SmallLimits small_lim{};
    if (want_gather && !(getenv("OSP_PLAN_SMALL") && atoi(getenv("OSP_PLAN_SMALL")) == 0) &&
        !(getenv("OSP_GATHER_OVER") && atoi(getenv("OSP_GATHER_OVER")) == 0)) {
        small_lim.cells = (uint32_t)std::clamp<long>(getenv("OSP_PLAN_SMALL_CELLS") ? atol(getenv("OSP_PLAN_SMALL_CELLS")) : (long)kSmallCells,
                                                     (long)kSmallCellsMin, (long)kSmallCellsMax);
        small_lim.chunks = (uint32_t)std::clamp<long>(getenv("OSP_PLAN_SMALL_CHUNKS") ? atol(getenv("OSP_PLAN_SMALL_CHUNKS")) : (long)kSmallChunks,
                                                      1L, (long)kSmallChunks);
    }
    uint64_t nsmall = 0;
    const uint64_t row_max = getenv("OSP_SPLIT_ROW_MAX") ? strtoull(getenv("OSP_SPLIT_ROW_MAX"), nullptr, 10) : kSplitRowMax;
    const int bits_cap = std::max(colbits - kDenseBits, 1);
    const int hub_b_want = std::min(kSplitMaxBits, bits_cap);
    const bool hub_env = !(getenv("OSP_HUB") && atoi(getenv("OSP_HUB")) == 0);
    int hub_b = 0;
    uint64_t ndcell = 0, tot[6] = {0, 0, 0, 0, 0, 0};
    const int direct_fine = 2;
    const double hub_min_share = getenv("OSP_HUB_MIN_SHARE") ? atof(getenv("OSP_HUB_MIN_SHARE")) : 0.2;
    bool hub_decided = false;
    for (int attempt = 0; attempt < 3; attempt++) {
        const bool hub_possible = ds && ds->b_rowptr && ds->keep && ctx->rank_atomic && hub_env && !ds->hub_refused;
        if (!hub_possible) hub_b = 0;
        split_params_kernel<<<grid_for(nlong, 256), 256, 0, s>>>(pl.p0.long_rows, nlong, row_off, colbits, row_max, bits_cap, ds ? ds->rowfirst : nullptr,
                                                                 ds ? ds->direct_max : 0ull, kCap, pl.hbits, pl.hmode, pl.nstretch, nseg, nhist, ncellh,
                                                                 hub_b, direct_fine, ds ? nrund : nullptr, hsmall, ds ? small_lim : SmallLimits{});
        zero_async(s, {{totals, 7 * sizeof(uint64_t)}});
        mode_totals_kernel<<<std::min(grid_for(nlong, 256), 64u), 256, 0, s>>>(pl.p0.long_rows, nlong, row_off, pl.hmode, hsmall, totals);
        device_exclusive_scan<LoadU32As64, uint64_t>(LoadU32As64{pl.nstretch}, nlong, pl.blkbase, pl.hscan_tmp, s);
        device_exclusive_scan<LoadU32As64, uint64_t>(LoadU32As64{nseg}, nlong, pl.vbase, pl.hscan_tmp, s);
        device_exclusive_scan<LoadU64, uint64_t>(LoadU64{nhist}, nlong, pl.hbase, pl.hscan_tmp, s);
        if (ds) device_exclusive_scan<LoadU64, uint64_t>(LoadU64{ncellh}, nlong, pl.cellbase, pl.hscan_tmp, s);
        if (ds && nrund) device_exclusive_scan<LoadU64, uint64_t>(LoadU64{nrund}, nlong, rdbase, pl.hscan_tmp, s);
        ndcell = 0;
        nrd = 0;
        {
            Gather g(s);
            g.add(&pl.nh, (const uint64_t *)pl.hoff + nlong); g.add(&pl.nblocks, (const uint64_t *)pl.blkbase + nlong);
            g.add(&pl.nvirt, (const uint64_t *)pl.vbase + nlong); g.add(&pl.ncell, (const uint64_t *)pl.hbase + nlong);
            if (ds) g.add(&ndcell, (const uint64_t *)pl.cellbase + nlong);
            if (ds && nrund) g.add(&nrd, (const uint64_t *)rdbase + nlong);
            for (int i = 0; i < 6; i++) g.add(&tot[i], (const uint64_t *)totals + i);
            g.add(&nsmall, (const uint64_t *)totals + 6);
            g.wait();
        }
        if (ds && ndcell >= 0xffffffffull) { ds = nullptr; hub_b = 0; continue; }
        if (hub_possible && !hub_decided && hub_b == 0 && pl.nblocks && (double)tot[3 + kModeStretch] >= hub_min_share * (double)count) {
            hub_decided = true;
            hub_b = hub_b_want;
            continue;
        }
        break;
    }
    for (int m = 0; m < 3; m++) { pl.mode_rows[m] = tot[m]; pl.mode_partials[m] = tot[3 + m]; }
    if (pl.nh >= 0xffffffffull) throw Error(OSP_ERR_CAPACITY, "long rows of one panel exceed 2^32 partial products");
    res->info.heavy_rows += nlong;
    res->info.heavy_partials += pl.nh;
    res->info.direct_rows += pl.mode_rows[kModeDirect];
    res->info.direct_partials += pl.mode_partials[kModeDirect];
    if (pl.ncell >= 0xffffffffull || pl.nblocks >= 0x7fffffffull || pl.nvirt >= 0xffffffffull || ndcell >= 0xffffffffull)
        throw Error(OSP_ERR_CAPACITY, "split histogram too large");
    if (getenv("OSP_VERBOSE"))
        fprintf(stderr, "[osp]   panel rows [%llu,%llu): %u tiles, %u long rows with %llu partial products -> %llu segments; direct: %llu rows, %llu "
                        "partial products, %llu cells\n",
                (unsigned long long)r0, (unsigned long long)r1, pl.p0.ntiles, nlong, (unsigned long long)pl.nh, (unsigned long long)pl.nvirt,
                (unsigned long long)pl.mode_rows[kModeDirect], (unsigned long long)pl.mode_partials[kModeDirect], (unsigned long long)ndcell);
    pl.ghist = sc.get<uint32_t>(pl.ncell + 1);
    pl.ghist_tmp = sc.get<uint32_t>(scan_scratch_entries(pl.ncell + 1));
    pl.vrow_off = sc.get<uint64_t>(pl.nvirt + 1);
    pl.vfirst = sc.get<uint8_t>(pl.nvirt + 1);
    pl.vcol0 = sc.get<uint32_t>(pl.nvirt + 1);
    pl.vcol1 = sc.get<uint32_t>(pl.nvirt + 1);
    if (pl.mode_rows[kModeDirect]) {
        pl.cells = sc.get<uint32_t>(ndcell);
        GatherPlan gp{};
        RunDesc<T> *runs = nullptr;
        static const uint64_t max_runs = getenv("OSP_GATHER_MAX_RUNS") ? strtoull(getenv("OSP_GATHER_MAX_RUNS"), nullptr, 10) : 0xffffffffull;
        if (ds->gather && nrund && nrd < max_runs) {
            runs = sc.get<RunDesc<T>>(std::max<uint64_t>(nrd, 1));
            pl.vrun_off = sc.get<uint32_t>(pl.nvirt + 1);
            pl.vrun_end = sc.get<uint32_t>(pl.nvirt + 1);
            gp.rdbase = rdbase; gp.vrun_off = pl.vrun_off; gp.vrun_end = pl.vrun_end;
            gp.rowruns = sc.get<uint32_t>(nlong);
            pl.nwritten = gp.nwritten = sc.get<uint32_t>(1);
            fill_async(s, {{pl.vrun_off, (pl.nvirt + 1) * sizeof(uint32_t), kNoRuns}, {gp.rowruns, (uint64_t)nlong * sizeof(uint32_t), kNoRuns},
                           {pl.nwritten, sizeof(uint32_t), 0u}});
            gp.over = !(getenv("OSP_GATHER_OVER") && atoi(getenv("OSP_GATHER_OVER")) == 0);
            gp.av_in_order = ds->av_in_order ? 1u : 0u;
            pl.may_write = !gp.over;
            pl.ga.runs = runs; pl.ga.b_colidx = ds->b_colidx; pl.ga.b_vals = (const T *)ds->b_vals;
        }
        if (!(runs && gp.over) || (hub_b && pl.nblocks)) ds->ensure_chunk_off(s);
        gp.mark_skipped = ds->chunk_off_ready ? 1u : 0u;
        const bool plan_small = runs != nullptr && gp.over && nsmall != 0;
        const bool plan_big = !plan_small || nsmall < pl.mode_rows[kModeDirect];
        if (plan_small) gp.small = hsmall;
        if (getenv("OSP_VERBOSE"))
            fprintf(stderr, "[osp]   small planner: %llu of %llu direct rows (at most %u chunks, %u cells)\n", (unsigned long long)(plan_small ? nsmall : 0),
                    (unsigned long long)pl.mode_rows[kModeDirect], small_lim.chunks, small_lim.cells);
        tm.begin(PH_PLAN_K, s);
        if (plan_small)
            direct_plan_small_kernel<T><<<nlong, kWave, direct_plan_small_lds(small_lim.cells), s>>>(
                pl.p0.long_rows, nlong, pl.hbits, nseg, pl.vbase, pl.hoff, colbits, kCap, ds->rowfirst, ds->off, ds->bs, ds->perm, ds->b_colidx,
                pl.vrow_off, pl.vcol0, pl.vcol1, ds->chunk_off, gp, (const T *)ds->a_vals, runs);
        if (!plan_big) {  }
        else if (nlong <= 4u * ctx->cus)
            direct_plan_kernel<T, kDirectCellsBig><<<nlong, kDirectThreads, 0, s>>>(pl.p0.long_rows, nlong, pl.hmode, pl.hbits, nseg, pl.vbase, pl.hoff,
                                                                                 pl.cellbase, row_off, colbits, kCap, ds->rowfirst, ds->off, ds->bs, ds->perm,
                                                                                 ds->b_colidx, pl.vrow_off, pl.vcol0, pl.vcol1, pl.cells, ds->chunk_off, gp,
                                                                                 (const T *)ds->a_vals, runs);
        else
        direct_plan_kernel<T><<<nlong, kDirectThreads, 0, s>>>(pl.p0.long_rows, nlong, pl.hmode, pl.hbits, nseg, pl.vbase, pl.hoff, pl.cellbase, row_off,
                                                              colbits, kCap, ds->rowfirst, ds->off, ds->bs, ds->perm, ds->b_colidx, pl.vrow_off,
                                                              pl.vcol0, pl.vcol1, pl.cells, ds->chunk_off, gp, (const T *)ds->a_vals, runs);
        tm.end(PH_PLAN_K);
        if (gp.rowruns && ds->gstat) gather_stats_kernel<<<std::min(grid_for(nlong, 256), 64u), 256, 0, s>>>(pl.p0.long_rows, nlong, row_off, gp.rowruns, ds->gstat);
#ifdef OSP_PLAN_PROF
        if (getenv("OSP_VERBOSE")) {
            unsigned long long hp[8] = {0}, z[8] = {0};
            OSP_HIP(hipStreamSynchronize(s));
            (void)hipMemcpyFromSymbol(hp, HIP_SYMBOL(osp_plan_prof), sizeof(hp));
            (void)hipMemcpyToSymbol(HIP_SYMBOL(osp_plan_prof), z, sizeof(z));
            double tot = 0;
            for (int k = 0; k < 6; k++) tot += (double)hp[k];
            fprintf(stderr, "[osp]   planner cycles: header %.1f %%, chunk descriptors %.1f %%, histogram pass %.1f %%, grouping %.1f %%, cell pass %.1f %%, "
                            "prefixes + output %.1f %%; %.0f cycles per row, %u rows\n", 100 * hp[0] / tot, 100 * hp[1] / tot, 100 * hp[2] / tot, 100 * hp[3] / tot,
                    100 * hp[4] / tot, 100 * hp[5] / tot, tot / std::max(1u, nlong), nlong);
            (void)hipMemcpyFromSymbol(hp, HIP_SYMBOL(osp_plan_small_prof), sizeof(hp));
            (void)hipMemcpyToSymbol(HIP_SYMBOL(osp_plan_small_prof), z, sizeof(z));
            tot = 0;
            for (int k = 0; k < 5; k++) tot += (double)hp[k];
            if (plan_small && tot > 0)
                fprintf(stderr, "[osp]   small planner cycles: header + chunk descriptors %.1f %%, histogram pass %.1f %%, grouping %.1f %%, counts %.1f %%, "
                                "prefixes + output %.1f %%; %.0f cycles per row, %llu rows\n", 100 * hp[0] / tot, 100 * hp[1] / tot, 100 * hp[2] / tot,
                        100 * hp[3] / tot, 100 * hp[4] / tot, tot / (double)nsmall, (unsigned long long)nsmall);
        }
#endif
        res->info.direct_plan_launches++;
        dbg_sync(s, "plan of the direct rows");
    }
    if (hub_b && pl.nblocks) {
        if (!ds->hub.sx) {
            Scratch &keep = *ds->keep;
            const uint64_t nb = ds->nnz_b;
            Scratch tmp(ctx);
            uint8_t *rowstart = tmp.get<uint8_t>(nb + 4);
            uint32_t *sx = keep.get<uint32_t>(nb + 1), *runstart = keep.get<uint32_t>(nb + 1);
            uint16_t *runblk = keep.get<uint16_t>(nb + 2);
            uint32_t *scan_tmp = tmp.get<uint32_t>(scan_scratch_entries(nb + 1));
            OSP_HIP(hipMemsetAsync(rowstart, 0, nb + 4, s));
            hub_rowstart_kernel<<<grid_for(ds->K, 256), 256, 0, s>>>(ds->b_rowptr, ds->K, rowstart);
            const int sh = colbits - hub_b;
            const HubRunFlag flag{rowstart, ds->b_colidx, sh};
            device_exclusive_scan<HubRunFlag, uint32_t>(flag, nb, sx, scan_tmp, s);
            compact_flagged_kernel<HubRunFlag><<<grid_for(nb, 256), 256, 0, s>>>(flag, sx, nb, 0, runstart);
            hub_runstart_end_kernel<<<1, 1, 0, s>>>(sx + nb, runstart, (uint32_t)nb);
            OSP_HIP(hipMemsetAsync(runblk, 0, (nb + 2) * sizeof(uint16_t), s));
            hub_runblk_kernel<<<std::min(grid_for(nb, 256), 4096u), 256, 0, s>>>(sx + nb, runstart, ds->b_colidx, sh, runblk);
            OSP_HIP(hipStreamSynchronize(s));
            ds->hub.sx = sx; ds->hub.runstart = runstart; ds->hub.runblk = runblk; ds->hub.sh = sh;
        }
        tm.begin(PH_HUB_K, s);
        uint64_t *jobruns = sc.get<uint64_t>(pl.nblocks + 1);
        uint64_t *jobscan_tmp = sc.get<uint64_t>(scan_scratch_entries(pl.nblocks + 1));
        const size_t hub_lds = sizeof(uint32_t) << hub_b;
        hub_plan_kernel<false><<<(unsigned)pl.nblocks, kHubThreads, hub_lds, s>>>(pl.p0.long_rows, nlong, pl.blkbase, pl.hbase, pl.hbits, pl.nstretch, row_off,
                                                                           ds->rowfirst, ds->off, ds->bs, ds->perm, ds->b_colidx, ds->hub, pl.ghist,
                                                                           pl.hoff, jobruns, nullptr, nullptr, nullptr);
        device_exclusive_scan<LoadU32, uint32_t>(LoadU32{pl.ghist}, pl.ncell, pl.ghist, pl.ghist_tmp, s);
        device_exclusive_scan<LoadU64, uint64_t>(LoadU64{jobruns}, pl.nblocks, jobruns, jobscan_tmp, s);
        const uint64_t ncells = d2h(jobruns + pl.nblocks, s);
        if (ncells >= (1ull << 40)) throw Error(OSP_ERR_CAPACITY, "hub rows: too many runs in one panel");
        if (getenv("OSP_VERBOSE"))
            fprintf(stderr, "[osp]   hub rows: %llu rows, %llu products in %llu runs (%.2f records per run), %llu jobs, 2^%d blocks\n",
                    (unsigned long long)pl.mode_rows[kModeStretch], (unsigned long long)pl.mode_partials[kModeStretch], (unsigned long long)ncells,
                    ncells ? (double)pl.mode_partials[kModeStretch] / (double)ncells : 0.0, (unsigned long long)pl.nblocks, hub_b);
        const double min_run = getenv("OSP_HUB_MIN_RUN") ? atof(getenv("OSP_HUB_MIN_RUN")) : 4.0;
        const double run = ncells ? (double)pl.mode_partials[kModeStretch] / (double)ncells : 0.0;
        const bool accept = run >= min_run;
        if (!accept) {
            ds->hub_refused = true;
            tm.end(PH_HUB_K);
        } else {
            uint32_t *hcells = sc.get<uint32_t>(ncells);
            ds->ensure_chunk_off(s);
            hub_plan_kernel<true><<<(unsigned)pl.nblocks, kHubThreads, hub_lds, s>>>(pl.p0.long_rows, nlong, pl.blkbase, pl.hbase, pl.hbits, pl.nstretch, row_off,
                                                                              ds->rowfirst, ds->off, ds->bs, ds->perm, ds->b_colidx, ds->hub, pl.ghist,
                                                                              pl.hoff, nullptr, jobruns, hcells, ds->chunk_off);
            tm.end(PH_HUB_K);
            pl.hub.cells = hcells;
            pl.hub.sx = ds->hub.sx;
            res->info.hub_plan_launches++;
            res->info.hub_cells += ncells;
            res->info.hub_rows += pl.mode_rows[kModeStretch];
            res->info.hub_partials += pl.mode_partials[kModeStretch];
        }
        dbg_sync(s, "plan of the hub rows");
    }
    if (ds && ds->expand_rows) {
        pl.expand_ok = true;
        const bool hubs = pl.hub.cells != nullptr;
        const int from_b_env = getenv("OSP_SPLIT_FROM_B") ? atoi(getenv("OSP_SPLIT_FROM_B")) : 1;
        if (!hubs && pl.nblocks != 0 && from_b_env != 0) pl.split_from_b = ds;
        pl.split_beside = from_b_env != 2;
        const bool stretch_x = !hubs && !pl.split_from_b;
        const uint64_t rows_x = pl.mode_rows[kModeSplitRow] + (stretch_x ? pl.mode_rows[kModeStretch] : 0);
        pl.xpartials = pl.mode_partials[kModeSplitRow] + (stretch_x ? pl.mode_partials[kModeStretch] : 0);
        if (getenv("OSP_VERBOSE") && pl.nblocks && !hubs)
            fprintf(stderr, "[osp]   stretch rows: %llu rows, %llu partial products split %s\n", (unsigned long long)pl.mode_rows[kModeStretch],
                    (unsigned long long)pl.mode_partials[kModeStretch], pl.split_from_b ? (pl.split_beside ? "from B" : "from B, after the join") : "from staged records");
        if (rows_x) {
            pl.xjobbase = sc.get<uint64_t>((uint64_t)nlong + 1);
            device_exclusive_scan<ExpandJobs, uint64_t>(ExpandJobs{pl.p0.long_rows, row_off, pl.hmode, kModeSplitRow, stretch_x ? kModeStretch : kModeSplitRow},
                                                        nlong, pl.xjobbase, pl.hscan_tmp, s);
            pl.xjobs_bound = pl.xpartials / kExpandJob + rows_x;
        }
    }
}

template <class T>
static void split_stretch_from_b(Context *ctx, hipStream_t s, const PanelPlan<T> &pl, const uint64_t *row_off, uint64_t base, int colbits) {
    const DirectSrc *ds = pl.split_from_b;
    const TilePlan &p0 = pl.p0;
    const uint32_t nlong = p0.nlong;
    const uint32_t *perm = ds->av_in_order ? nullptr : ds->perm;
    const RowSrc<float> cols{ds->rowfirst, ds->off, ds->bs, nullptr, nullptr, ds->b_colidx, nullptr};
    const RowSrc<T> src{ds->rowfirst, ds->off, ds->bs, perm, (const T *)ds->a_vals, ds->b_colidx, (const T *)ds->b_vals};
    split_count_kernel<true><<<(unsigned)pl.nblocks, kSplitThreads, 0, s>>>(p0.long_rows, nlong, pl.blkbase, pl.hbase, pl.hbits, pl.nstretch, row_off, base, colbits,
                                                                          nullptr, 0u, pl.ghist, cols);
    device_exclusive_scan<LoadU32, uint32_t>(LoadU32{pl.ghist}, pl.ncell, pl.ghist, pl.ghist_tmp, s);
    OSP_WITH_RA(ctx, split_scatter_kernel<T, RA, true><<<(unsigned)pl.nblocks, kSplitThreads, 0, s>>>(
                         p0.long_rows, nlong, pl.blkbase, pl.hbase, pl.hbits, pl.nstretch, row_off, base, colbits, nullptr, pl.ghist, pl.hoff, pl.qstage, src));
    split_vrows_kernel<<<grid_for(pl.nvirt + 1, 256), 256, 0, s>>>(nlong, pl.vbase, pl.hbase, pl.nstretch, pl.hbits, pl.hmode, colbits, pl.ghist, pl.hoff, pl.nvirt,
                                                                  pl.nh, pl.vrow_off, pl.vfirst, pl.vcol0, pl.vcol1);
    OSP_HIP(hipGetLastError());
}

template <class T>
static void merge_panel(Context *ctx, Result *res, PhaseTimer &tm, const MergeIO<T> &io, int colbits, PanelPlan<T> &pl) {
    hipStream_t s = ctx->stream;
    Scratch &sc = pl.sc;
    constexpr uint32_t kCap = (uint32_t)TileCap<T>::value;
    const uint32_t max_rows = pl.max_rows;
#ifdef OSP_CHECK_DESC
    crumbs_init();
#endif
    const uint64_t r1 = io.r1, base = io.base;
    const TilePlan &p0 = pl.p0;

    MergeLevels<T> lv{};
    lv.stage[0] = io.stage; lv.row_off[0] = io.row_off; lv.base[0] = base; lv.c_rowptr[0] = io.c_rowptr; lv.heavy_nnz[0] = nullptr;
    uint32_t ntot = p0.ntiles;
    TileDesc *desc = nullptr;
    TilePlan p1;
    uint64_t *vbase = pl.vbase;
    int64_t *vptr = nullptr;
    uint64_t *seg_src = nullptr;
    uint32_t *seg_nnz = nullptr;
    Part<T> *qstage = pl.qstage;
    if (p0.nlong) {
        const uint32_t nlong = p0.nlong;
        uint64_t *hoff = pl.hoff, *hscan_tmp = pl.hscan_tmp, *blkbase = pl.blkbase, *hbase = pl.hbase;
        uint8_t *hbits = pl.hbits;
        uint32_t *nstretch = pl.nstretch, *ghist = pl.ghist, *ghist_tmp = pl.ghist_tmp;
        const uint64_t nh = pl.nh, nblocks = pl.nblocks, nvirt = pl.nvirt, ncell = pl.ncell;
        uint64_t *vrow_off = pl.vrow_off;
        uint8_t *vfirst = pl.vfirst;
        if (pl.mode_rows[kModeSplitRow]) {
            tm.begin(PH_SPLIT_K);
            OSP_WITH_RA(ctx, split_row_kernel<T, RA><<<nlong, kSplitRowThreads, 0, s>>>(p0.long_rows, nlong, hbits, pl.hmode, vbase, hoff, io.row_off,
                                                                                     base, colbits, io.stage, qstage, vrow_off));
            tm.end(PH_SPLIT_K);
            res->info.split_launches++;
            res->info.split_partials += pl.mode_partials[kModeSplitRow];
            dbg_sync(s, "split: one-workgroup rows");
        }
        if (pl.split_from_b && !pl.split_beside) split_stretch_from_b<T>(ctx, s, pl, io.row_off, base, colbits);
        if (nblocks && !pl.hub.cells && !pl.split_from_b) {
            split_count_kernel<<<(unsigned)nblocks, kSplitThreads, 0, s>>>(p0.long_rows, nlong, blkbase, hbase, hbits, nstretch, io.row_off,
                                                                         base, colbits, (const char *)io.stage, (uint32_t)sizeof(Part<T>), ghist);
            device_exclusive_scan<LoadU32, uint32_t>(LoadU32{ghist}, ncell, ghist, ghist_tmp, s);
            OSP_WITH_RA(ctx, split_scatter_kernel<T, RA><<<(unsigned)nblocks, kSplitThreads, 0, s>>>(
                                 p0.long_rows, nlong, blkbase, hbase, hbits, nstretch, io.row_off, base, colbits, io.stage, ghist, hoff, qstage));
        }
        dbg_sync(s, "split: stretch rows");
        if (!pl.split_from_b)
            split_vrows_kernel<<<grid_for(nvirt + 1, 256), 256, 0, s>>>(nlong, vbase, hbase, nstretch, hbits, pl.hmode, colbits, ghist, hoff, nvirt, nh,
                                                                       vrow_off, vfirst, pl.vcol0, pl.vcol1);
        OSP_HIP(hipGetLastError());
        dbg_sync(s, "split: segment offsets");
        p1 = plan_tiles(ctx, sc, vrow_off, 0, nvirt, 0, kCap, max_rows, vfirst, nh, nlong);
        dbg_sync(s, "tiles over the segments");
        vptr = (int64_t *)sc.get<uint64_t>(nvirt + 1);
        lv.stage[1] = qstage; lv.row_off[1] = vrow_off; lv.base[1] = 0; lv.c_rowptr[1] = vptr;
        if (p1.nlong) {
            const uint32_t nseg_long = p1.nlong;
            seg_src = sc.get<uint64_t>(nseg_long);
            seg_nnz = sc.get<uint32_t>(nvirt + 1);
            lv.heavy_nnz[1] = seg_nnz;
            if (pl.ga.runs) {
                uint64_t *xsjob = sc.get<uint64_t>((uint64_t)nseg_long + 1);
                uint64_t *xsjob_tmp = sc.get<uint64_t>(scan_scratch_entries((uint64_t)nseg_long + 1));
                device_exclusive_scan<SegExpandJobs, uint64_t>(SegExpandJobs{p1.long_rows, vrow_off, pl.vrun_off}, nseg_long, xsjob, xsjob_tmp, s);
                const uint64_t job_bound = nh / kExpandJob + nseg_long;
                expand_segments_kernel<T><<<(unsigned)std::min<uint64_t>(job_bound, (uint64_t)ctx->cus * 8), kExpandThreads, 0, s>>>(
                    p1.long_rows, nseg_long, xsjob, vrow_off, pl.vrun_off, pl.vrun_end, pl.ga.runs, pl.ga.b_colidx, pl.ga.b_vals, qstage);
            }
            const uint32_t *rest_list = p1.long_rows;
            uint32_t nrest = nseg_long;
            uint32_t *hscan = sc.get<uint32_t>((uint64_t)nseg_long + 1);
            uint64_t *sscan_tmp = sc.get<uint64_t>(scan_scratch_entries(nseg_long));
            {
                const SegDenseFlag df{p1.long_rows, pl.vcol0, pl.vcol1, getenv("OSP_DENSE_SEG") ? atoi(getenv("OSP_DENSE_SEG")) : 1};
                device_exclusive_scan<SegDenseFlag, uint32_t>(df, nseg_long, hscan, (uint32_t *)sscan_tmp, s);
                const uint32_t ndense = d2h(hscan + nseg_long, s);
                if (ndense) {
                    uint32_t *dense_list = sc.get<uint32_t>(ndense), *others = sc.get<uint32_t>(nseg_long - ndense);
                    seg_split_list_kernel<SegDenseFlag><<<grid_for(nseg_long, 256), 256, 0, s>>>(df, hscan, nseg_long, dense_list, others);
                    if (ctx->dense_atomic[sizeof(T) == 8])
                        dense_segment_kernel<T, true><<<grid_for(ndense, kDenseWaves), kDenseWaves * kWave, 0, s>>>(dense_list, ndense, vrow_off, pl.vcol0, pl.vcol1,
                                                                              qstage, seg_nnz);
                    else
                        dense_segment_kernel<T, false><<<grid_for(ndense, kDenseWaves), kDenseWaves * kWave, 0, s>>>(dense_list, ndense, vrow_off, pl.vcol0, pl.vcol1,
                                                                              qstage, seg_nnz);
                    res->info.dense_segments += ndense;
                    rest_list = others;
                    nrest = nseg_long - ndense;
                }
            }
            dbg_sync(s, "over-long segments: dense accumulation");
            const uint32_t big_cap = getenv("OSP_BIGTILE_CAP") ? std::min<uint32_t>((uint32_t)strtoul(getenv("OSP_BIGTILE_CAP"), nullptr, 10), kBigTileCap)
                                                                : (uint32_t)kBigTileCap;
            uint32_t nhuge = 0, nmid = 0;
            uint32_t *huge_list = nullptr, *mid_list = nullptr;
            if (nrest) {
                const SegHugeFlag hf{rest_list, vrow_off, big_cap};
                device_exclusive_scan<SegHugeFlag, uint32_t>(hf, nrest, hscan, (uint32_t *)sscan_tmp, s);
                nhuge = d2h(hscan + nrest, s);
                nmid = nrest - nhuge;
                huge_list = sc.get<uint32_t>(nhuge);
                mid_list = sc.get<uint32_t>(nmid);
                seg_partition_kernel<<<grid_for(nrest, 256), 256, 0, s>>>(hf, hscan, nrest, huge_list, mid_list);
            }
            res->info.sorted_segments += nhuge;
            if (nmid) {
                TileDesc *bdesc = sc.get<TileDesc>(nmid);
                seg_tile_desc_kernel<<<grid_for(nmid, 256), 256, 0, s>>>(mid_list, nmid, vrow_off, pl.vcol0, pl.vcol1, bdesc);
                uint32_t *bticket = sc.get<uint32_t>(1);
                zero_async(s, {{bticket, sizeof(uint32_t)}});
                const uint32_t bgrid = ctx->cus * (uint32_t)merge_wgs_per_cu<T, kBigTileThreads, kBigTileCap>();
                OSP_WITH_RA(ctx, merge_tiles_kernel<T, kBigTileThreads, 32, kBigTileCap, kMergeMaxWgs, RA>
                            <<<std::min<uint32_t>(nmid, bgrid), kBigTileThreads, 0, s>>>(bdesc, nmid, lv, colbits, nullptr, bticket, nullptr, nullptr,
                                                                                         nullptr, nullptr));
            }
            dbg_sync(s, "over-long segments: big in-place tiles");
            if (nhuge) {
                uint64_t *soff = sc.get<uint64_t>((uint64_t)nhuge + 1);
                device_exclusive_scan<HeavyLen, uint64_t>(HeavyLen{huge_list, vrow_off}, nhuge, soff, sscan_tmp, s);
                const uint64_t ns = d2h(soff + nhuge, s);
                res->info.sorted_partials += ns;
                SortedRuns runs(sc, ns);
                heavy_fill_kernel<<<grid_for(ns, 256), 256, 0, s>>>(huge_list, soff, nhuge, vrow_off, 0, colbits, (const char *)qstage,
                                                                    (uint32_t)sizeof(Part<T>), ns, runs.keys[0], runs.poss[0]);
                runs.sort(colbits + bits_for(nhuge));
                T *sorted_val = sc.get<T>(ns);
                heavy_gather_kernel<T><<<grid_for(ns, 256), 256, 0, s>>>(runs.poss[runs.cur], qstage, ns, sorted_val);
                runs.heads();
                heavy_reduce_kernel<T><<<grid_for(ns, 256), 256, 0, s>>>(runs.keys[runs.cur], sorted_val, runs.headscan, runs.head_pos(), ns, huge_list,
                                                                         soff, nhuge, vrow_off, 0, colbits, qstage);
                heavy_rows_kernel<<<grid_for(nhuge, 256), 256, 0, s>>>(huge_list, soff, nhuge, runs.headscan, seg_nnz);
            }
            dbg_sync(s, "over-long segments: global sort");
            heavy_src_inplace_kernel<<<grid_for(nseg_long, 256), 256, 0, s>>>(p1.long_rows, nseg_long, vrow_off, 0, seg_src);
        }
        lv.heavy_nnz[1] = seg_nnz;
        uint32_t *j0 = sc.get<uint32_t>(nlong), *tb = sc.get<uint32_t>((uint64_t)nlong + 1), *extra = sc.get<uint32_t>((uint64_t)nlong + 1);
        chain_rows_kernel<<<grid_for(nlong + 1, 256), 256, 0, s>>>(p0.long_rows, nlong, p0.tile_rows, p0.ntiles, vbase, p1.tile_rows,
                                                                  p1.ntiles, j0, tb, extra);
        device_exclusive_scan<LoadU32, uint32_t>(LoadU32{extra}, nlong, extra, (uint32_t *)hscan_tmp, s);
        ntot = p0.ntiles + (p1.ntiles - nlong);
        desc = sc.get<TileDesc>(ntot);
        tile_desc_kernel<(int)kCap><<<grid_for(p0.ntiles, 256), 256, 0, s>>>(p0.tile_rows, p0.ntiles, r1, io.row_off, base, 0u, j0, extra,
                                                                           nlong, tb, pl.vcol0, pl.vcol1, desc, nullptr, nullptr, io.rowfirst0);
        tile_desc_kernel<(int)kCap><<<grid_for(p1.ntiles, 256), 256, 0, s>>>(p1.tile_rows, p1.ntiles, nvirt, vrow_off, 0, 1u, j0, extra,
                                                                           nlong, tb, pl.vcol0, pl.vcol1, desc, pl.ga.runs ? pl.vrun_off : nullptr,
                                                                           pl.vrun_end);
        dbg_sync(s, "tile chain");
    } else {
        desc = sc.get<TileDesc>(ntot);
        tile_desc_kernel<(int)kCap><<<grid_for(p0.ntiles, 256), 256, 0, s>>>(p0.tile_rows, p0.ntiles, r1, io.row_off, base, 0u, nullptr,
                                                                           nullptr, 0u, nullptr, nullptr, nullptr, desc, nullptr, nullptr, io.rowfirst0);
    }
    uint64_t *tile_status = sc.get<uint64_t>(ntot);
    const uint32_t nshards = 1u;
    uint32_t *ticket = sc.get<uint32_t>((uint64_t)(nshards + 1) * kTicketStride);
    zero_async(s, {{tile_status, (uint64_t)ntot * sizeof(uint64_t)}, {ticket, (uint64_t)(nshards + 1) * kTicketStride * sizeof(uint32_t)}});
    dbg_sync(s, "tile planning, splits, over-long segments");
    tm.begin(PH_MERGE_K);
    if (io.ct.enabled) {
        const uint32_t rw_grid = ctx->cus * (uint32_t)merge_wgs_per_cu<T, kMergeThreads, TileCap<T>::value, kMergeMaxWgs, 64>();
        OSP_WITH_RA(ctx, merge_tiles_kernel<T, kMergeThreads, 64, TileCap<T>::value, kMergeMaxWgs, RA>
                    <<<std::min<uint32_t>(ntot, rw_grid), kMergeThreads, 0, s>>>(desc, ntot, lv, colbits, tile_status, ticket, io.out_in, io.c_col,
                                                                                 io.c_val, io.out_out, io.ct, nshards, io.abort_word));
    } else if (pl.ga.runs || io.runs0) {
        GatherArgs<T> ga = pl.ga;
        ga.runs0 = io.runs0;
        if (io.runs0) { ga.b_colidx = io.b_colidx; ga.b_vals = io.b_vals; }
        const uint32_t merge_grid = ctx->cus * (uint32_t)merge_wgs_per_cu<T, kMergeThreads, TileCap<T>::value>();
        OSP_WITH_RA(ctx, merge_tiles_kernel<T, kMergeThreads, 0, TileCap<T>::value, kMergeMaxWgs, RA, true>
                    <<<std::min<uint32_t>(ntot, merge_grid), kMergeThreads, 0, s>>>(desc, ntot, lv, colbits, tile_status, ticket, io.out_in, io.c_col,
                                                                                    io.c_val, io.out_out, ChunkTable<T>{}, nshards, io.abort_word, ga));
    } else {
        const uint32_t merge_grid = ctx->cus * (uint32_t)merge_wgs_per_cu<T, kMergeThreads, TileCap<T>::value>();
        OSP_WITH_RA(ctx, merge_tiles_kernel<T, kMergeThreads, 0, TileCap<T>::value, kMergeMaxWgs, RA>
                    <<<std::min<uint32_t>(ntot, merge_grid), kMergeThreads, 0, s>>>(desc, ntot, lv, colbits, tile_status, ticket, io.out_in, io.c_col,
                                                                                    io.c_val, io.out_out, ChunkTable<T>{}, nshards, io.abort_word));
    }
    tm.end(PH_MERGE_K);
    dbg_sync(s, "merge tiles");
#ifdef OSP_MERGE_PROF
    if (getenv("OSP_VERBOSE")) {
        std::vector<TileDesc> hd(ntot);
        copy_d2h(hd.data(), desc, (size_t)ntot * sizeof(TileDesc), s);
        uint64_t byp[5] = {0}, ent[5] = {0}, gt = 0, ge = 0, gr = 0, bits[33] = {0};
        for (const TileDesc &t : hd) {
            if (t.n > kCap) continue;
            int rb = 0; while ((1u << rb) < t.nr) rb++;
            const int kb = t.kbits ? (int)t.kbits : colbits + rb;
            const int np = std::min(4, (kb + kDigitBits - 1) / kDigitBits);
            byp[np]++; ent[np] += t.n; bits[std::min(kb, 32)] += 1;
            if (t.rcnt) { gt++; ge += t.n; gr += t.rcnt; }
        }
// ... 4 lines not shown
        constexpr int lpt = ((int)kCap + kMergeThreads - 1) / kMergeThreads;
        uint64_t byq[lpt + 1] = {0}, slots = 0, need = 0, run = 0;
        for (const TileDesc &t : hd) {
            if (t.n > kCap) continue;
            const int q = std::max(1, (int)((t.n + kMergeThreads - 1) / kMergeThreads));
            int body = lpt;
            for (int c = kTileRoundClasses; c >= 1; c--) if (q <= tile_class_rounds(lpt, c, kTileRoundClasses)) body = tile_class_rounds(lpt, c, kTileRoundClasses);
            byq[q]++; slots += lpt; need += q; run += body;
        }
        fprintf(stderr, "\n[osp]   tiles by rounds (Q = ceil(n / %d)):", kMergeThreads);
        for (int q = 1; q <= lpt; q++) fprintf(stderr, " Q=%d: %llu;", q, (unsigned long long)byq[q]);
        fprintf(stderr, " slot-rounds needed %.1f %%, run %.1f %% of %d per tile (%d bodies)", slots ? 100.0 * need / slots : 0.0,
                slots ? 100.0 * run / slots : 0.0, lpt, kTileRoundClasses);
        fprintf(stderr, "\n");
    }
    if (getenv("OSP_VERBOSE")) {
        unsigned long long hp[16] = {0}, z[16] = {0};
        OSP_HIP(hipStreamSynchronize(s));
        (void)hipMemcpyFromSymbol(hp, HIP_SYMBOL(osp_merge_prof), sizeof(hp));
        (void)hipMemcpyToSymbol(HIP_SYMBOL(osp_merge_prof), z, sizeof(z));
        static const char *names[12] = {"run table / hash init", "keys + hash count", "publish", "rank", "digit scan", "scatter", "values + heads + scan",
                                        "look-back + ticket", "run sums", "compaction", "output + next tile's request", "gathered: lookup + columns"};
        double tot = 0;
        for (int k = 0; k < 12; k++) tot += (double)hp[k];
        fprintf(stderr, "[osp]   merge kernel, %u tiles, cycles of thread 0 per phase:", ntot);
        for (int k = 0; k < 12; k++) fprintf(stderr, " %s %.1f %%;", names[k], 100.0 * hp[k] / tot);
        fprintf(stderr, " %.0f cycles per tile and workgroup\n", tot / std::max(1u, ntot));
    }
#endif
    res->info.merge_launches++;
    if (p1.nlong) {
        heavy_copy_kernel<T><<<grid_for(p1.nlong, 8), 256, 0, s>>>(p1.long_rows, p1.nlong, seg_src, seg_nnz, vptr, qstage, nullptr, nullptr,
                                                                   io.c_col, io.c_val);
        heavy_copy_rest_kernel<T><<<p1.nlong, 256, 0, s>>>(p1.long_rows, p1.nlong, seg_src, seg_nnz, vptr, qstage, nullptr, nullptr,
                                                           io.c_col, io.c_val);
    }
    chain_finish_kernel<<<grid_for(std::max<uint32_t>(p0.nlong, 1), 256), 256, 0, s>>>(p0.long_rows, p0.nlong, vbase, vptr, io.out_out, r1,
                                                                                       io.c_rowptr);
    dbg_sync(s, "copy of reduced segments, chain finish");
    OSP_HIP(hipGetLastError());
}

struct PanelSink {
    osp_panel_fn fn;
    void *user;
};

constexpr uint64_t kPartialsOnDevice = ~0ull;
template <class T>
static void merge_pipeline(Context *ctx, Result *res, Producer<T> &prod, uint64_t M_all, uint64_t N,
                           const uint64_t *d_row_off,
                           uint64_t P, uint64_t cap_cfg, PhaseTimer &tm, uint64_t r_lo = 0, uint64_t r_hi = ~0ull,
                           uint64_t off_lo = 0, const PanelSink *sink = nullptr, const ChunkTable<T> *ct = nullptr,
                           const DirectSrc *ds = nullptr, const std::vector<uint64_t> *cuts = nullptr, const ShortRuns<T> *sr = nullptr) {
    if (r_hi == ~0ull) r_hi = M_all;
    const uint64_t M = r_hi - r_lo;
    res->info.M = M;
    res->info.row_begin = r_lo;
    res->info.row_end = r_hi;
    hipStream_t s = ctx->stream;
    Scratch sc(ctx);
    const int colbits = std::max(1, bits_for(N));

    const uint64_t E = 4 + sizeof(T);
    uint64_t cap_c;
    uint64_t *ub = sc.get<uint64_t>(M + 1);
    {
        Scratch us(ctx);
        uint64_t *ub_tmp = us.get<uint64_t>(scan_scratch_entries(M + 1));
        if (P != 0) device_exclusive_scan<RowUpperBound, uint64_t>(RowUpperBound{d_row_off + r_lo, N}, M, ub, ub_tmp, s);
        if (P == 0) {
            cap_c = 0;
        } else if (P == kPartialsOnDevice) {
            Gather g(s);
            g.add(&P, d_row_off + M_all);
            g.add(&cap_c, (const uint64_t *)ub + M);
            g.wait();
            res->info.partials = P;
        } else {
            cap_c = d2h(ub + M, s);
        }
    }
    if (!sink) res->rowptr = (int64_t *)ctx->alloc((M + 1) * sizeof(int64_t));
    if (P == 0) {
        res->info.nnz_c = 0;
        if (sink) {
            int64_t *zr = sc.get<int64_t>(M + 1);
            OSP_HIP(hipMemsetAsync(zr, 0, (M + 1) * sizeof(int64_t), s));
            OSP_HIP(hipStreamSynchronize(s));
            res->info.panels = 1;
            const osp_panel_t pd{r_lo, r_hi, 0, zr, nullptr, nullptr, 0, 1, {0, 0}};
            if (sink->fn(&pd, sink->user)) throw Error(OSP_ERR_ARG, "panel callback returned non-zero");
            return;
        }
        OSP_HIP(hipMemsetAsync(res->rowptr, 0, (M + 1) * sizeof(int64_t), s));
        return;
    }
    uint32_t *c_col = nullptr;
    T *c_val = nullptr;
    if (!sink) {
        res->colidx = (uint32_t *)ctx->alloc(std::max<uint64_t>(cap_c, 1) * sizeof(uint32_t));
        res->vals = ctx->alloc(std::max<uint64_t>(cap_c, 1) * sizeof(T));
        c_col = res->colidx;
        c_val = (T *)res->vals;
    }
    size_t free_b = 0, total_b = 0;
    OSP_HIP(hipMemGetInfo(&free_b, &total_b));
    free_b += ctx->pooled_bytes + (ctx->sibling ? ctx->sibling->pooled_bytes : 0);
    uint64_t cap = cap_cfg;
    const double per_record = sink ? 3.7 : (ds && ds->gather) ? 2.5 : 2.6;
    if (cap == 0) cap = std::max<uint64_t>((uint64_t)(free_b * 0.85 / (per_record * E)), 1ull << 20);
    cap = std::min<uint64_t>(cap, 0xfffffff0ull);
    if (getenv("OSP_VERBOSE"))
        fprintf(stderr, "[osp] M=%llu N=%llu P=%llu nnzC<=%llu (%.1f GB) free %.1f GB -> staging capacity %llu partial products (%.1f GB)\n",
                (unsigned long long)M, (unsigned long long)N, (unsigned long long)P, (unsigned long long)cap_c, cap_c * E / 1e9,
                free_b / 1e9, (unsigned long long)cap, cap * E / 1e9);
    std::vector<uint64_t> bounds{r_lo};
    std::vector<uint64_t> boff{off_lo};
    if (P <= cap && !(cuts && !cuts->empty())) {
        bounds.push_back(r_hi);
        boff.push_back(off_lo + P);
    } else {
        constexpr uint32_t kMaxPanels = 4096;
        const uint32_t ncuts = cuts ? (uint32_t)cuts->size() : 0u;
        uint64_t *d_b = sc.get<uint64_t>(2ull * (kMaxPanels + 1) + 2), *d_cuts = sc.get<uint64_t>(std::max<uint32_t>(ncuts, 1));
        if (ncuts) copy_h2d(d_cuts, cuts->data(), ncuts * sizeof(uint64_t), s);
        panel_bounds_kernel<<<1, kWave, 0, s>>>(d_row_off, r_lo, M, cap, d_cuts, ncuts, kMaxPanels, d_b);
        std::vector<uint64_t> hb(2ull * (kMaxPanels + 1) + 2);
        copy_d2h(hb.data(), d_b, hb.size() * sizeof(uint64_t), s);
        const uint64_t np = hb[0], bad = hb[1];
        if (bad != ~0ull)
            throw Error(OSP_ERR_CAPACITY, "output row " + std::to_string(bad) + " has more partial products than the staging capacity of " +
                        std::to_string(cap) + ", or the product needs more than " + std::to_string(kMaxPanels) + " panels");
        for (uint64_t p = 1; p <= np; p++) { bounds.push_back(hb[2 + p]); boff.push_back(hb[2 + (kMaxPanels + 1) + p]); }
        boff[0] = hb[2 + (kMaxPanels + 1)];
    }
    const bool all_rows = r_lo == 0 && r_hi == M_all;
    const uint32_t npanels = (uint32_t)bounds.size() - 1;
    res->info.panels = npanels;
    auto panel_base = [&](uint32_t p) { return (npanels == 1) ? off_lo : boff[p]; };
    auto panel_count = [&](uint32_t p) { return (npanels == 1) ? P : boff[p + 1] - boff[p]; };
    uint64_t max_panel = 0, max_rows_panel = 0;
    for (uint32_t p = 0; p < npanels; p++) {
        max_panel = std::max(max_panel, panel_count(p));
        max_rows_panel = std::max(max_rows_panel, bounds[p + 1] - bounds[p]);
    }
    Part<T> *stage = sc.get<Part<T>>(max_panel);
    uint64_t *out_nnz = sc.get<uint64_t>((uint64_t)npanels + 1);
    uint32_t *abort_word = sc.get<uint32_t>(1);
    zero_async(s, {{out_nnz, sizeof(uint64_t)}, {abort_word, sizeof(uint32_t)}});
    auto check_abort = [&](uint32_t flag) {
        if (flag) throw Error(OSP_ERR_HIP, "the merge made no progress for seconds (a tile's predecessors never published their sizes); "
                                           "with several ticket shards that happens when fewer workgroups than shards ever run side by side");
    };
    const bool overlap = npanels > 1 && !(getenv("OSP_PLAN_OVERLAP") && atoi(getenv("OSP_PLAN_OVERLAP")) == 0);
    if (overlap) ctx->need_aux();
    struct AuxScope {
        Context *c; hipStream_t main;
        explicit AuxScope(Context *ctx_) : c(ctx_), main(ctx_->stream) { c->stream = c->aux; }
        ~AuxScope() {
            if (std::uncaught_exceptions()) (void)hipStreamSynchronize(c->aux);
            c->stream = main;
        }
    };
    typedef std::unique_ptr<PanelPlan<T>> PlanPtr;
    auto plan_one = [&](uint32_t p, bool beside) -> PlanPtr {
        const uint64_t r0 = bounds[p], r1 = bounds[p + 1];
        const uint64_t base = panel_base(p), count = panel_count(p);
        PlanPtr pl(new PanelPlan<T>(ctx));
        if (beside) {
            AuxScope scope(ctx);
            OSP_HIP(hipStreamWaitEvent(ctx->stream, ctx->aux_fork, 0));
            tm.begin(PH_MERGE, ctx->stream);
            plan_panel<T>(ctx, res, tm, *pl, d_row_off, r0, r1, base, count, colbits, ds);
            tm.end(PH_MERGE);
            OSP_HIP(hipEventRecord(ctx->aux_join, ctx->stream));
            res->info.plans_overlapped++;
        } else {
            tm.begin(PH_MERGE);
            plan_panel<T>(ctx, res, tm, *pl, d_row_off, r0, r1, base, count, colbits, ds);
            tm.end(PH_MERGE);
        }
        return pl;
    };
    auto multiply_and_plan_next = [&](uint32_t p, PanelPlan<T> &plan, PlanPtr &nxt) {
        const uint64_t r0 = bounds[p], r1 = bounds[p + 1];
        const uint64_t base = panel_base(p), count = panel_count(p);
        if (plan.p0.nlong) plan.qstage = plan.sc.template get<Part<T>>(plan.nh);
        const bool beside = overlap && p + 1 < npanels;
        if (beside) { OSP_HIP(hipEventRecord(ctx->aux_fork, s)); ctx->fork_window = true; ctx->releases_in_fork_window = 0; }
        struct WindowEnd { Context *c; ~WindowEnd() { c->fork_window = false; } } window_end{ctx};
        tm.begin(PH_MUL);
        bool column_major = count != 0 && !(sr && plan.p0.nlong == 0), desc_only = false;
        if (count && plan.xjobbase && plan.xjobs_bound) {
            tm.begin(PH_EXPAND_K);
            const RowSrc<T> src{ds->rowfirst, ds->off, ds->bs, ds->av_in_order ? nullptr : ds->perm, (const T *)ds->a_vals, ds->b_colidx, (const T *)ds->b_vals};
            expand_rows_kernel<T><<<(unsigned)plan.xjobs_bound, kExpandThreads, 0, s>>>(plan.p0.long_rows, plan.p0.nlong, plan.xjobbase, d_row_off, base, src, stage);
            tm.end(PH_EXPAND_K);
            res->info.expand_launches++;
            res->info.expand_partials += plan.xpartials;
        }
        if (count && plan.split_from_b && plan.split_beside) {
            split_stretch_from_b<T>(ctx, s, plan, d_row_off, base, colbits);
            dbg_sync(s, "split: stretch rows, from B");
        }
        if (count && plan.expand_ok) {
            desc_only = true;
            const uint32_t nw = (plan.nwritten && plan.may_write) ? d2h(plan.nwritten, s) : 0u;
            column_major = plan.hub.cells != nullptr || nw != 0 || (plan.mode_rows[kModeDirect] != 0 && plan.ga.runs == nullptr);
        }
        const bool mostly_hub = plan.hub.cells != nullptr && plan.mode_partials[kModeStretch] * 3 >= count;
        if (column_major && ds) ds->ensure_chunk_off(s);
        if (column_major) prod.produce(r0, r1, npanels == 1 && all_rows, base, count, stage, tm, plan.cells, plan.qstage, plan.hub.cells ? &plan.hub : nullptr,
                                       plan.ga.runs != nullptr && !mostly_hub, plan.p0.nlong != 0, desc_only, mostly_hub);
        tm.end(PH_MUL);
        if (beside) {
            ctx->fork_window = false;
            if (ctx->releases_in_fork_window)
                throw Error(OSP_ERR_HIP, "internal: " + std::to_string(ctx->releases_in_fork_window) + " pooled buffers were released between the fork of the "
                                         "second stream and the next panel's plan (the pool is not stream-aware: see Context::fork_window)");
            nxt = plan_one(p + 1, true);
            OSP_HIP(hipStreamWaitEvent(s, ctx->aux_join, 0));
// ... 171 lines not shown
```

### outerspace_amd/csrc/osp_prims.h

```cpp
#pragma once
#include <hip/hip_runtime.h>
#include <stdint.h>

#ifndef OSP_RANK_ATOMIC
#define OSP_RANK_ATOMIC 1
#endif

namespace osp {

constexpr int kWave = 64;
constexpr int kScanThreads = 256;
constexpr int kScanItems = 8;
constexpr int kScanTile = kScanThreads * kScanItems;

__device__ __forceinline__ unsigned lane_id() { return threadIdx.x & 63u; }
__device__ __forceinline__ uint64_t lanemask_lt() { return (1ull << lane_id()) - 1ull; }

template <class T>
__device__ __forceinline__ T wave_incl_scan(T v) {
#pragma unroll
    for (int d = 1; d < kWave; d <<= 1) {
        T o = __shfl_up(v, d, kWave);
        if ((int)lane_id() >= d) v += o;
    }
// ... 216 lines not shown
    __shared__ uint32_t base[kRadix];
    __shared__ uint32_t cnt[NW][kRadix];
    base[threadIdx.x] = hist_scan[(uint64_t)threadIdx.x * nblocks + blockIdx.x];
#pragma unroll
    for (int w = 0; w < NW; w++) cnt[w][threadIdx.x] = 0;
    __syncthreads();
    const int w = threadIdx.x >> 6;
    const uint64_t tile = (uint64_t)blockIdx.x * kSortTile;
    for (int r = 0; r < kSortRounds; r++) {
        const uint64_t i = tile + (uint64_t)r * kSortThreads + threadIdx.x;
        const bool valid = i < n;
        K key = 0;
        uint32_t val = 0;
        if (valid) {
            key = keys_in[i];
            val = vals_in[i];
        }
        const unsigned d = (unsigned)(key >> shift) & 255u;
        unsigned rank = 0;
        if constexpr (RA) {
            if (valid) rank = atomicAdd(&cnt[w][d], 1u);
        } else {
            const uint64_t peers = wave_match8(d, valid);
            rank = __popcll(peers & lanemask_lt());
            if (valid && rank == 0) cnt[w][d] = (uint32_t)__popcll(peers);
        }
        __syncthreads();
        if (valid) {
            uint32_t off = base[d] + rank;
#pragma unroll
            for (int ww = 0; ww < NW; ww++)
                if (ww < w) off += cnt[ww][d];
            keys_out[off] = key;
            vals_out[off] = val;
        }
        __syncthreads();
        {
            uint32_t s = 0;
#pragma unroll
            for (int ww = 0; ww < NW; ww++) {
                s += cnt[ww][threadIdx.x];
                cnt[ww][threadIdx.x] = 0;
            }
            base[threadIdx.x] += s;
        }
        __syncthreads();
    }
}

struct LoadU32 {
    const uint32_t *p;
    __device__ uint32_t operator()(uint64_t i) const { return p[i]; }
};

inline uint64_t sort_blocks(uint64_t n) { return (n + kSortTile - 1) / kSortTile; }
inline uint64_t sort_hist_entries(uint64_t n) { return sort_blocks(n) * kRadix + 1; }

struct RadixSorted { int cur; uint32_t launches; };
template <class K>
inline RadixSorted device_radix_sort_pairs(K *keys[2], uint32_t *vals[2], uint64_t n, int nbits,
                                           uint32_t *hist, uint32_t *scan_scratch, hipStream_t stream, bool rank_atomic) {
    int cur = 0;
    uint32_t launches = 0;
    if (n == 0) return {cur, launches};
    const uint32_t nblocks = (uint32_t)sort_blocks(n);
    for (int shift = 0; shift < nbits; shift += 8) {
        sort_hist_kernel<K><<<nblocks, kSortThreads, 0, stream>>>(keys[cur], n, shift, hist, nblocks);
        launches += 2 + device_exclusive_scan<LoadU32, uint32_t>(LoadU32{hist}, (uint64_t)nblocks * kRadix, hist,
                                                                 scan_scratch, stream);
        if (rank_atomic)
            sort_scatter_kernel<K, true><<<nblocks, kSortThreads, 0, stream>>>(keys[cur], vals[cur], keys[cur ^ 1], vals[cur ^ 1], n, shift,
                                                                                hist, nblocks);
        else
            sort_scatter_kernel<K, false><<<nblocks, kSortThreads, 0, stream>>>(keys[cur], vals[cur], keys[cur ^ 1], vals[cur ^ 1], n, shift,
                                                                                 hist, nblocks);
        cur ^= 1;
    }
    return {cur, launches};
}

}
```

### outerspace_amd/csrc/osp_split.h

```cpp
#pragma once
#include "osp_kernels.h"

namespace osp {

#ifndef OSP_SPLIT_THREADS
#define OSP_SPLIT_THREADS 256
#endif
constexpr int kSplitThreads = OSP_SPLIT_THREADS;
#ifndef OSP_SPLIT_ROW_THREADS
#define OSP_SPLIT_ROW_THREADS 1024
#endif
#ifndef OSP_SPLIT_ROW_PRE
#define OSP_SPLIT_ROW_PRE 1
#endif
constexpr int kSplitRowThreads = OSP_SPLIT_ROW_THREADS;
#ifndef OSP_SPLIT_ROW_STRETCH
#define OSP_SPLIT_ROW_STRETCH 4096
#endif
constexpr int kSplitRowStretch = OSP_SPLIT_ROW_STRETCH;
#ifndef OSP_SPLIT_STRETCH
#define OSP_SPLIT_STRETCH 4096
#endif
constexpr int kSplitStretch = OSP_SPLIT_STRETCH;
#ifndef OSP_SPLIT_JOB_ROUNDS
// ... 28 lines not shown
constexpr int kSmallFineBits = 8;
constexpr int kSmallRanges = 32;
#ifndef OSP_SMALL_CELLS
#define OSP_SMALL_CELLS 512
#endif
constexpr int kSmallCells = OSP_SMALL_CELLS, kSmallCellsMin = 1 << kSmallFineBits, kSmallCellsMax = 2048;
struct SmallLimits {
    uint32_t cells = 0, chunks = kSmallChunks, ranges = kSmallRanges;
};
__global__ void split_params_kernel(const uint32_t *rows, uint32_t nheavy, const uint64_t *row_off, int colbits,
                                    uint64_t row_max, int bits_cap, const uint32_t *rowfirst, uint64_t direct_max, uint32_t cap,
                                    uint8_t *hbits, uint8_t *hmode, uint32_t *nstretch, uint32_t *nseg, uint64_t *nhist, uint64_t *ncell,
                                    int hub_b = 0, int direct_fine = 0, uint64_t *nrund = nullptr, uint8_t *hsmall = nullptr,
                                    SmallLimits sl = SmallLimits{}) {
    const uint32_t h = blockIdx.x * blockDim.x + threadIdx.x;
    if (h >= nheavy) return;
    const uint64_t U = row_off[rows[h] + 1] - row_off[rows[h]];
    const uint64_t want = (U + kSplitTarget - 1) / kSplitTarget;
    int b = 1;
    while (b < kSplitMaxBits && (1ull << b) < want) b++;
    b = min(b, min(colbits, bits_cap));
    const bool big = U > row_max || b > kSplitRowBits;
    const bool capped = (1ull << b) < want;
    const uint64_t nranges = min(2 * U / cap + 2, (1ull << b) + 1);
    const uint64_t nc = rowfirst != nullptr ? (uint64_t)(rowfirst[rows[h] + 1] - rowfirst[rows[h]]) : 0ull;
    const uint64_t dmax = (capped && direct_max) ? max(direct_max, kDirectDenseMax) : direct_max;
    const bool direct = rowfirst != nullptr && b <= kSplitRowBits && (!big || capped) && U <= dmax && nranges <= (uint64_t)kDirectMaxRanges &&
                        nc * nranges <= kDirectRowCells;
    const uint32_t ns = (big && !direct) ? (uint32_t)((U + kSplitJob - 1) / kSplitJob) : 0u;
    if (ns && hub_b) b = hub_b;
    if (direct && !capped) b = min(b + direct_fine, min(colbits, kDirectFineBits));
    hbits[h] = (uint8_t)b;
    hmode[h] = direct ? kModeDirect : big ? kModeStretch : kModeSplitRow;
    nstretch[h] = ns;
    nseg[h] = direct ? (uint32_t)nranges : 1u << b;
    nhist[h] = (uint64_t)ns << b;
    ncell[h] = direct ? ((1ull << b) + 3) / 4 + nc * nranges : 0ull;
    if (nrund) nrund[h] = direct ? min(nc * nranges, U) : 0ull;
    if (hsmall)
        hsmall[h] = direct && !capped && b <= kSmallFineBits && nc >= 1 && nc <= (uint64_t)sl.chunks && nranges <= (uint64_t)sl.ranges &&
                    nc * nranges <= (uint64_t)sl.cells && U < (1ull << 20);
}
struct HeavyLenIf {
    const uint32_t *rows;
    const uint64_t *row_off;
    const uint8_t *hmode;
    uint8_t mode;
    __device__ uint64_t operator()(uint64_t h) const { return hmode[h] == mode ? row_off[rows[h] + 1] - row_off[rows[h]] : 0ull; }
};
struct LoadU32As64 {
    const uint32_t *p;
    __device__ uint64_t operator()(uint64_t i) const { return p[i]; }
};

struct SplitJob {
    uint32_t h, st, b, nst;
    uint64_t beg, end;
    uint64_t hbase;
};
__device__ __forceinline__ SplitJob split_job(const uint32_t *rows, uint32_t nheavy, const uint64_t *blkbase,
                                              const uint64_t *hbase, const uint8_t *hbits, const uint32_t *nstretch,
                                              const uint64_t *row_off, uint64_t base) {
    SplitJob j;
    j.h = (uint32_t)(upper_bound_dev(blkbase, 0, (uint64_t)nheavy + 1, (uint64_t)blockIdx.x) - 1);
    j.st = (uint32_t)(blockIdx.x - blkbase[j.h]);
    j.b = hbits[j.h];
    j.nst = nstretch[j.h];
    const uint64_t s = row_off[rows[j.h]] - base, e = row_off[rows[j.h] + 1] - base;
    j.beg = s + (uint64_t)j.st * kSplitJob;
    j.end = min(j.beg + (uint64_t)kSplitJob, e);
    j.hbase = hbase[j.h];
    return j;
}

template <bool FROM_B = false>
__global__ __launch_bounds__(kSplitThreads) void split_count_kernel(
    const uint32_t *rows, uint32_t nheavy, const uint64_t *blkbase, const uint64_t *hbase, const uint8_t *hbits,
    const uint32_t *nstretch, const uint64_t *row_off, uint64_t base, int colbits, const char *stage, uint32_t rec_bytes,
    uint32_t *ghist, const RowSrc<float> src = RowSrc<float>{}) {
    __shared__ uint32_t hist[1 << kSplitMaxBits];
    const SplitJob j = split_job(rows, nheavy, blkbase, hbase, hbits, nstretch, row_off, base);
    const uint32_t nseg = 1u << j.b;
    for (uint32_t d = threadIdx.x; d < nseg; d += kSplitThreads) hist[d] = 0;
    __syncthreads();
    const int sh = colbits - (int)j.b;
    if constexpr (FROM_B) {
        constexpr uint32_t per = kSplitJob / (kSplitThreads / kWave);
        const uint32_t row = rows[j.h];
        const uint64_t p0 = j.beg + (uint64_t)(threadIdx.x >> 6) * per, p1 = min(p0 + per, j.end);
        if (p0 < p1)
            walk_row_slice<float, false>(src, lane_id(), src.rowfirst[row], src.rowfirst[row + 1], base + p0, base + p1,
                                         [&](uint64_t, uint32_t col, float) { atomicAdd(&hist[col >> sh], 1u); });
    } else {
        for (uint64_t i = j.beg + threadIdx.x; i < j.end; i += kSplitThreads)
            atomicAdd(&hist[*(const uint32_t *)(stage + i * rec_bytes) >> sh], 1u);
    }
    __syncthreads();
    for (uint32_t d = threadIdx.x; d < nseg; d += kSplitThreads) ghist[j.hbase + (uint64_t)d * j.nst + j.st] = hist[d];
}

__device__ __forceinline__ void wave_match_bits(unsigned digit, int bits, bool valid, unsigned &rank, unsigned &count) {
    const uint64_t vm = __ballot(valid);
    uint32_t plo = (uint32_t)vm, phi = (uint32_t)(vm >> 32);
    for (int b = 0; b < bits; b++) {
        const uint32_t bit = (digit >> b) & 1u;
        const uint64_t m = __ballot(bit != 0);
// ... 1045 lines not shown
```

Before: 69.58 billion.

## Replace multi-pass device scans with single-pass chained look-back scans

```diff
diff --git a/__graft_entry__.py b/__graft_entry__.py
--- a/__graft_entry__.py
+++ b/__graft_entry__.py
@@ -14,6 +14,7 @@
     from outerspace_amd import _lib
     L = _lib.lib()
     missing = [s for s in _lib.EXPORTS + _lib.MASKED_EXPORTS + _lib.MCL_EXPORTS + _lib.APPLY_MASK_EXPORTS + _lib.SELECT_EXPORTS + _lib.EWISE_EXPORTS
+               + _lib.SCAN_EXPORTS
                if not hasattr(L, s)]
     if missing:
         raise RuntimeError(f"library lacks exported symbols: {missing}")
diff --git a/include/outerspace_spgemm_scan.h b/include/outerspace_spgemm_scan.h
--- /dev/null
+++ b/include/outerspace_spgemm_scan.h
@@ -0,0 +1,49 @@
+#ifndef OUTERSPACE_SPGEMM_SCAN_H
+#define OUTERSPACE_SPGEMM_SCAN_H
+
+#include "outerspace_spgemm.h"
+
+#ifdef __cplusplus
+extern "C" {
+#endif
+
+typedef enum osp_scan_kind {
+    OSP_SCAN_U32 = 0,
+    OSP_SCAN_U32_AS_U64 = 1,
+    OSP_SCAN_U64 = 2,
+    OSP_SCAN_COMPACT = 3
+} osp_scan_kind_t;
+
+typedef struct osp_scan_selftest {
+    uint64_t n;
+    int32_t  kind;
+    int32_t  flag_log2;
+    uint64_t seed;
+    uint64_t r0;
+    uint32_t in_place;
+    uint32_t write_scan;
+    uint32_t repeats;
+    uint32_t pair;
+    uint32_t items;
+    uint32_t reserved[7];
+} osp_scan_selftest_t;
+
+typedef struct osp_scan_selftest_stats {
+    uint64_t mismatches;
+    uint64_t total;
+    uint64_t small_max;
+    uint32_t tile;
+    uint32_t window;
+    uint32_t error_word;
+    uint32_t launches;
+    float    ms_chained;
+    float    ms_reference;
+    uint32_t reserved[6];
+} osp_scan_selftest_stats_t;
+
+int osp_scan_selftest(osp_context_t ctx, const osp_scan_selftest_t *args, osp_scan_selftest_stats_t *stats);
+
+#ifdef __cplusplus
+}
+#endif
+#endif
diff --git a/outerspace_amd/_lib.py b/outerspace_amd/_lib.py
--- a/outerspace_amd/_lib.py
+++ b/outerspace_amd/_lib.py
@@ -168,6 +168,20 @@
     _fields_ = [("nnz_in", C.c_uint64), ("nnz_out", C.c_uint64), ("long_runs", C.c_uint64), ("ms_total", C.c_float),
                 ("launches", C.c_uint32), ("readbacks", C.c_uint32), ("reserved", C.c_uint32 * 5)]
 
+SCAN_KINDS = {"u32": 0, "u32_as_u64": 1, "u64": 2, "compact": 3}
+
+
+class ScanSelftest(_Stats):
+    _fields_ = [("n", C.c_uint64), ("kind", C.c_int32), ("flag_log2", C.c_int32), ("seed", C.c_uint64), ("r0", C.c_uint64),
+                ("in_place", C.c_uint32), ("write_scan", C.c_uint32), ("repeats", C.c_uint32), ("pair", C.c_uint32), ("items", C.c_uint32),
+                ("reserved", C.c_uint32 * 7)]
+
+
+class ScanSelftestStats(_Stats):
+    _fields_ = [("mismatches", C.c_uint64), ("total", C.c_uint64), ("small_max", C.c_uint64), ("tile", C.c_uint32), ("window", C.c_uint32),
+                ("error_word", C.c_uint32), ("launches", C.c_uint32), ("ms_chained", C.c_float), ("ms_reference", C.c_float),
+                ("reserved", C.c_uint32 * 6)]
+
 PANEL_FN = C.CFUNCTYPE(C.c_int, C.POINTER(Panel), C.c_void_p)
 
 MULTI_MAX_RANKS = 16
@@ -229,6 +243,8 @@
 EXTRACT_EXPORTS = ["osp_csr_extract"]
 
 BUILD_EXPORTS = ["osp_csr_build"]
+
+SCAN_EXPORTS = ["osp_scan_selftest"]
 
 _lib = None
 
@@ -315,6 +331,7 @@
     L.osp_csr_mxd.argtypes = [vp, C.POINTER(Semiring), vp, u64, vp, i32, C.POINTER(MxdStats)]
     L.osp_csr_extract.argtypes = [vp, C.POINTER(Extract), C.POINTER(vp), C.POINTER(ExtractStats)]
     L.osp_csr_build.argtypes = [vp, C.POINTER(Build), C.POINTER(vp), C.POINTER(BuildStats)]
+    L.osp_scan_selftest.argtypes = [vp, C.POINTER(ScanSelftest), C.POINTER(ScanSelftestStats)]
     _lib = L
     return L
 
diff --git a/outerspace_amd/csrc/osp_api.hip b/outerspace_amd/csrc/osp_api.hip
--- a/outerspace_amd/csrc/osp_api.hip
+++ b/outerspace_amd/csrc/osp_api.hip
@@ -27,6 +27,7 @@
 #include "../../include/outerspace_spgemm_mxd.h"
 #include "../../include/outerspace_spgemm_extract.h"
 #include "../../include/outerspace_spgemm_build.h"
+#include "../../include/outerspace_spgemm_scan.h"
 #include "osp_internal.h"
 #include "osp_kernels.h"
 #include "osp_split.h"
@@ -59,6 +60,7 @@
 
 #include "osp_context.h"
 #include "osp_pipeline.h"
+#include "osp_scan_test.h"
 
 template <class T>
 static const T *to_device(Scratch &sc, const T *p, uint64_t n, osp_memspace_t space, hipStream_t s) {
@@ -233,6 +235,7 @@
     ShortRuns<T> srun{};
     DirectSrc dsrc{};
     uint32_t n_long_rows = 1;
+    ScanPhase ph_sym(sc, s, {nnz, gather_short ? nnz : 0, rowwise ? M : 0});
     if (nnz == 0) {
         OSP_HIP(hipMemsetAsync(row_off, 0, (M + 1) * sizeof(uint64_t), s));
     } else {
@@ -243,7 +246,6 @@
         uint32_t *bs_sorted = (rowwise || direct || gather_short) ? keep.get<uint32_t>(nnz) : nullptr;
         uint32_t *rowfirst = keep.get<uint32_t>(M + 1);
         uint64_t *offs_sorted = keep.get<uint64_t>(nnz + 1);
-        uint64_t *scan_tmp = ss.get<uint64_t>(scan_scratch_entries(std::max<uint64_t>(nnz, M + 1)));
         const bool table = rowwise || direct || gather_short;
         const bool with_av = gather_ok && gather_env >= 1 && (direct || gather_short);
         T *av_sorted = with_av ? keep.get<T>(nnz) : nullptr;
@@ -254,12 +256,12 @@
         SymEpilogue sym_ep{w, bs, rows_sorted, perm, w_sorted, bs_sorted};
         if (with_av) { sym_ep.av_sorted = av_sorted; sym_ep.vwords = (uint32_t)(sizeof(T) / 4); }
         rs.sort(a_rowidx + e0, sym_ep);
-        device_exclusive_scan<LoadU32As64, uint64_t>(LoadU32As64{w_sorted}, nnz, offs_sorted, scan_tmp, s);
+        device_scan_chained<LoadU32As64, uint64_t>(LoadU32As64{w_sorted}, nnz, offs_sorted, ph_sym.take(nnz), s);
         sym_row_offsets_kernel<<<grid_for(M + 1, 256), 256, 0, s>>>(rows_sorted, offs_sorted, nnz, M, row_off, rowfirst);
         const uint64_t rw_cap = (rowwise || gather_short) ? (uint64_t)TileCap<T>::value : 0ull;
         const bool expand_rows_on = gather_short && !(getenv("OSP_EXPAND_ROWS") && atoi(getenv("OSP_EXPAND_ROWS")) == 0);
         if (!expand_rows_on) sym_scatter_offsets_kernel<<<grid_for(nnz, 256), 256, 0, s>>>(perm, offs_sorted, rows_sorted, row_off, rw_cap, nnz, chunk_off);
-        if (partials_only || rowwise || row_sharded) P = d2h(offs_sorted + nnz, s);
+        if (partials_only || rowwise || row_sharded) P = ph_sym.fetch((const uint64_t *)offs_sorted + nnz, s);
         else P = kPartialsOnDevice;
         if (direct) {
             dsrc = DirectSrc{rowfirst, offs_sorted, bs_sorted, perm, b_colidx, chunk_off, direct_max};
@@ -275,8 +277,8 @@
         }
         if (gather_short) {
             const ShortRunFlag sf{offs_sorted};
-            uint32_t *cidx = ss.get<uint32_t>(nnz + 1), *cidx_tmp = ss.get<uint32_t>(scan_scratch_entries(nnz + 1));
-            device_exclusive_scan<ShortRunFlag, uint32_t>(sf, nnz, cidx, cidx_tmp, s);
+            uint32_t *cidx = ss.get<uint32_t>(nnz + 1);
+            device_scan_chained<ShortRunFlag, uint32_t>(sf, nnz, cidx, ph_sym.take(nnz), s);
             RunDesc<T> *runs0 = sc.get<RunDesc<T>>(nnz);
             uint32_t *rowfirst0 = sc.get<uint32_t>(M + 1);
             short_runs_kernel<T><<<grid_for(nnz, 256), 256, 0, s>>>(sf, cidx, nnz, bs_sorted, av_sorted, runs0);
@@ -286,8 +288,8 @@
         if (rowwise) {
             ct = ChunkTable<T>{offs_sorted, bs_sorted, perm, rowfirst, a_vals + e0, b_colidx, b_vals, (uint32_t)rw_cap, 1u};
             uint32_t *flag_scan = ss.get<uint32_t>(M + 1);
-            device_exclusive_scan<HeavyRowFlag, uint32_t>(HeavyRowFlag{row_off, 0, (uint32_t)rw_cap}, M, flag_scan, (uint32_t *)scan_tmp, s);
-            n_long_rows = d2h(flag_scan + M, s);
+            device_scan_chained<HeavyRowFlag, uint32_t>(HeavyRowFlag{row_off, 0, (uint32_t)rw_cap}, M, flag_scan, ph_sym.take(M), s);
+            n_long_rows = ph_sym.fetch((const uint32_t *)flag_scan + M, s);
         }
     }
     tm.end(PH_SYM);
@@ -331,7 +333,7 @@
     }
     const uint64_t off_lo = 0, P_rows = P;
     merge_pipeline<T>(ctx, res, prod, M, N, row_off, P_rows, cfg.partial_capacity, tm, r_lo, r_hi, off_lo, sink,
-                      rowwise ? &ct : nullptr, (direct && nnz) ? &dsrc : nullptr, nullptr, gather_short ? &srun : nullptr);
+                      rowwise ? &ct : nullptr, (direct && nnz) ? &dsrc : nullptr, nullptr, gather_short ? &srun : nullptr, &ph_sym);
 
     finish_timing(res, ev, tm, s);
     if (gather_short) res->info.gathered_short_partials = res->info.partials - res->info.heavy_partials;
@@ -1150,6 +1152,24 @@
     });
 }
 
+int osp_scan_selftest(osp_context_t ctx_, const osp_scan_selftest_t *args, osp_scan_selftest_stats_t *stats) {
+    Context *ctx = (Context *)ctx_;
+    if (!ctx || !args || !stats) return fail(OSP_ERR_ARG, "null argument");
+    const osp_scan_selftest_t a = *args;
+    for (uint32_t r : a.reserved) if (r) return fail(OSP_ERR_ARG, "osp_scan_selftest_t: reserved words must be 0");
+    if (a.kind < OSP_SCAN_U32 || a.kind > OSP_SCAN_COMPACT) return fail(OSP_ERR_ARG, "unknown scan kind");
+    if (a.items != 0 && a.items != 8 && a.items != 16 && a.items != 32) return fail(OSP_ERR_ARG, "items: 0, 8, 16 or 32");
+    if (a.in_place && a.kind != OSP_SCAN_U32 && a.kind != OSP_SCAN_U64) return fail(OSP_ERR_ARG, "in place: kinds OSP_SCAN_U32 and OSP_SCAN_U64 only");
+    if (a.n > (1ull << 31) || a.r0 > 0xffffffffull || a.r0 + a.n > 0xffffffffull) return fail(OSP_ERR_ARG, "n above 2^31, or r0 + n above 2^32 - 1");
+    if (a.flag_log2 < -1 || a.flag_log2 > 40) return fail(OSP_ERR_ARG, "flag_log2: -1 to 40");
+    return guard([&]() -> int {
+        OSP_HIP(hipSetDevice(ctx->device));
+        osp_scan_selftest_stats_t st;
+        scan_selftest(ctx, a, st);
+        *stats = st;
+        return OSP_OK;
+    });
+}
 int osp_stream_copy_probe(osp_context_t ctx_, uint64_t bytes, int reps, double *gbps) {
     Context *ctx = (Context *)ctx_;
     if (!ctx || !gbps) return fail(OSP_ERR_ARG, "null argument");
diff --git a/outerspace_amd/csrc/osp_context.h b/outerspace_amd/csrc/osp_context.h
--- a/outerspace_amd/csrc/osp_context.h
+++ b/outerspace_amd/csrc/osp_context.h
@@ -407,6 +407,33 @@
     if (most == 0) return;
     zero_regions_kernel<<<(unsigned)std::min<uint64_t>((most + 255) / 256, 2048), 256, 0, s>>>(z);
 }
+struct ScanPhase {
+    uint64_t *words = nullptr;
+    uint64_t cap = 0, used = kChainHead;
+    uint32_t *ext_err = nullptr;
+    ScanPhase(Scratch &sc, hipStream_t s, std::initializer_list<uint64_t> ns, uint32_t *ext_err_ = nullptr) : ext_err(ext_err_) {
+        uint64_t w = 0;
+        for (uint64_t n : ns) w += scan_chained_words(n);
+        if (!w) return;
+        cap = kChainHead + w;
+        words = sc.get<uint64_t>(cap);
+        zero_async(s, {{words, cap * sizeof(uint64_t)}});
+    }
+    ScanState take(uint64_t n) {
+        const uint64_t w = scan_chained_words(n);
+        if (!w) return ScanState{};
+        if (used + w > cap) throw Error(OSP_ERR_ARG, "ScanPhase: more scan state taken than the phase reserved");
+        ScanState st{words + used, ext_err ? ext_err : reinterpret_cast<uint32_t *>(words)};
+        used += w;
+        return st;
+    }
+    uint32_t flag = 0;
+    void watch(struct Gather &g);
+    void check() const {
+        if (flag) throw Error(OSP_ERR_HIP, "a chained scan gave up waiting for a tile that nobody published (look-back watchdog)");
+    }
+    template <class T> T fetch(const T *dptr, hipStream_t s);
+};
 constexpr int kGatherMax = 24;
 struct GatherSrcs {
     const void *p[kGatherMax];
@@ -445,8 +472,21 @@
         n = 0;
     }
 };
+inline void ScanPhase::watch(Gather &g) {
+    if (words && !ext_err) g.add(&flag, (const uint32_t *)words);
+}
 template <class T> static T d2h(const T *dptr, hipStream_t s) {
     T v;
     copy_d2h(&v, dptr, sizeof(T), s);
     return v;
 }
+template <class T> T ScanPhase::fetch(const T *dptr, hipStream_t s) {
+    if (!words || ext_err) return d2h(dptr, s);
+    T v;
+    Gather g(s);
+    g.add(&v, dptr);
+    watch(g);
+    g.wait();
+    check();
+    return v;
+}
diff --git a/outerspace_amd/csrc/osp_kernels.h b/outerspace_amd/csrc/osp_kernels.h
--- a/outerspace_amd/csrc/osp_kernels.h
+++ b/outerspace_amd/csrc/osp_kernels.h
@@ -244,6 +244,8 @@
     const uint64_t *p;
     __device__ uint64_t operator()(uint64_t i) const { return p[i]; }
 };
+template <class TOut, int ITEMS>
+__device__ __forceinline__ bool scan_load_wide(const LoadU64 &f, uint64_t i0, TOut (&v)[ITEMS]) { return scan_load_wide_ptr(f.p + i0, v); }
 struct PanelKeepFlag {
     const uint32_t *a_rowidx; const uint64_t *chunk_off; int64_t e0; uint32_t r0; uint64_t r1; uint32_t desc_only;
     __device__ uint32_t operator()(uint64_t t) const {
@@ -753,7 +755,6 @@
     if (t < n && f(t)) list[scan[t]] = (uint32_t)(r0 + t);
 }
 
-constexpr uint64_t kStatusAgg = 1ull << 62, kStatusPrefix = 2ull << 62, kStatusMask = (1ull << 62) - 1;
 
 #ifndef OSP_RUN_SHORT
 #define OSP_RUN_SHORT 16
@@ -850,12 +851,7 @@
     if (nbad) atomicAdd(bad, nbad);
 }
 
-constexpr int kLookWin = 1;
-__device__ __forceinline__ void lookback_publish(uint64_t *status, uint32_t t, uint64_t total) {
-    __hip_atomic_store(&status[t], (t == 0 ? kStatusPrefix : kStatusAgg) | total, __ATOMIC_RELAXED, __HIP_MEMORY_SCOPE_AGENT);
-}
 constexpr int kTicketStride = 32;
-constexpr uint32_t kLookbackSpinLimit = 1u << 22;
 __device__ __forceinline__ uint32_t take_ticket(uint32_t *ticket, uint32_t nshards, uint32_t &shard, uint32_t ntiles) {
     if (nshards <= 1) return atomicAdd(ticket, 1u);
     for (uint32_t tries = 0; tries < nshards; tries++) {
@@ -865,53 +861,6 @@
         shard = shard + 1 == nshards ? 0u : shard + 1;
     }
     return ntiles;
-}
-template <bool PUBLISH = true>
-__device__ __forceinline__ uint64_t lookback_prefix(uint64_t *status, uint32_t t, uint64_t total, uint32_t *abort_word = nullptr) {
-    const unsigned lane = lane_id();
-    if (PUBLISH && lane == 0) lookback_publish(status, t, total);
-    uint64_t excl = 0;
-    int64_t b = (int64_t)t - 1;
-    uint32_t spins = 0;
-    while (b >= 0) {
-        uint64_t sv[kLookWin];
-#pragma unroll
-        for (int j = 0; j < kLookWin; j++) {
-            const int64_t idx = b - (int64_t)(j * kWave) - (int64_t)lane;
-            sv[j] = kStatusPrefix;
-            if (idx >= 0) sv[j] = __hip_atomic_load(&status[idx], __ATOMIC_RELAXED, __HIP_MEMORY_SCOPE_AGENT);
-        }
-        bool done = false, retry = false;
-        uint64_t part = 0;
-#pragma unroll
-        for (int j = 0; j < kLookWin; j++) {
-            if (!done && !retry) {
-                const uint64_t m_prefix = __ballot((sv[j] >> 62) == 2), m_empty = __ballot((sv[j] >> 62) == 0);
-                const int p = m_prefix ? __builtin_ctzll(m_prefix) : 64;
-                const uint64_t need = p >= 63 ? ~0ull : ((2ull << p) - 1ull);
-                if (m_empty & need) {
-                    retry = true;
-                } else {
-                    part += ((int)lane <= p) ? (sv[j] & kStatusMask) : 0ull;
-                    if (p < 64) done = true;
-                }
-            }
-        }
-        if (retry) {
-            __builtin_amdgcn_s_sleep(1);
-            if (abort_word && (++spins & 255u) == 0) {
-                if (spins >= kLookbackSpinLimit && lane == 0) atomicExch(abort_word, 1u);
-                if (spins >= kLookbackSpinLimit || __hip_atomic_load(abort_word, __ATOMIC_RELAXED, __HIP_MEMORY_SCOPE_AGENT) != 0u) break;
-            }
-            continue;
-        }
-        excl += wave_reduce_sum_u62(part);
-        if (done) break;
-        b -= (int64_t)kLookWin * kWave;
-    }
-    if (lane == 0 && t != 0)
-        __hip_atomic_store(&status[t], kStatusPrefix | (excl + total), __ATOMIC_RELAXED, __HIP_MEMORY_SCOPE_AGENT);
-    return excl;
 }
 
 struct TileDesc {
diff --git a/outerspace_amd/csrc/osp_pipeline.h b/outerspace_amd/csrc/osp_pipeline.h
--- a/outerspace_amd/csrc/osp_pipeline.h
+++ b/outerspace_amd/csrc/osp_pipeline.h
@@ -38,25 +38,21 @@
     hipStream_t s = ctx->stream;
     const uint64_t nr = r1 - r0;
     TilePlan pl;
-    uint32_t *flag_scan = sc.get<uint32_t>(nr + 1);
     uint32_t *tmp_rows = sc.get<uint32_t>(nr + 1);
-    uint64_t *scan_tmp = sc.get<uint64_t>(scan_scratch_entries(std::max<uint64_t>(nr + 1, 16)));
     const uint64_t slot = 8ull * cap;
+    const uint32_t ncb = (uint32_t)std::min<uint64_t>(nr, 2 + nforce + total / slot + nr / 65536);
+    ScanPhase ph(sc, s, {nr, ncb, nr});
+    uint32_t *counts = sc.get<uint32_t>(2);
     CoarseStartFlag csf{row_off, r0, base, slot, force_start};
-    device_exclusive_scan<CoarseStartFlag, uint32_t>(csf, nr, flag_scan, (uint32_t *)scan_tmp, s);
-    compact_flagged_kernel<CoarseStartFlag><<<grid_for(nr, 256), 256, 0, s>>>(csf, flag_scan, nr, r0, tmp_rows);
-    const uint32_t ncb = (uint32_t)std::min<uint64_t>(nr, 2 + nforce + total / slot + nr / 65536);
-    const uint32_t *ncb_p = flag_scan + nr;
+    device_scan_compact<CoarseStartFlag>(csf, nr, r0, tmp_rows, counts, ph.take(nr), s);
+    const uint32_t *ncb_p = counts;
     uint32_t *cb_cnt = sc.get<uint32_t>((uint64_t)ncb + 1);
     tile_walk_kernel<<<grid_for(ncb, 128), 128, 0, s>>>(tmp_rows, ncb_p, ncb, r1, row_off, cap, max_rows, nullptr, cb_cnt, nullptr);
-    device_exclusive_scan<LoadU32, uint32_t>(LoadU32{cb_cnt}, ncb, cb_cnt, (uint32_t *)scan_tmp, s);
+    device_scan_chained<LoadU32, uint32_t>(LoadU32{cb_cnt}, ncb, cb_cnt, ph.take(ncb), s);
     HeavyRowFlag hrf{row_off, r0, cap};
-    uint32_t *long_scan = sc.get<uint32_t>(nr + 1);
-    uint32_t *long_tmp = sc.get<uint32_t>(scan_scratch_entries(std::max<uint64_t>(nr + 1, 16)));
-    device_exclusive_scan<HeavyRowFlag, uint32_t>(hrf, nr, long_scan, long_tmp, s);
     pl.long_rows = sc.get<uint32_t>(nr + 1);
-    compact_flagged_kernel<HeavyRowFlag><<<grid_for(nr, 256), 256, 0, s>>>(hrf, long_scan, nr, r0, pl.long_rows);
-    { Gather g(s); g.add(&pl.ntiles, (const uint32_t *)cb_cnt + ncb); g.add(&pl.nlong, (const uint32_t *)long_scan + nr); g.wait(); }
+    device_scan_compact<HeavyRowFlag>(hrf, nr, r0, pl.long_rows, counts + 1, ph.take(nr), s);
+    { Gather g(s); g.add(&pl.ntiles, (const uint32_t *)cb_cnt + ncb); g.add(&pl.nlong, (const uint32_t *)counts + 1); ph.watch(g); g.wait(); ph.check(); }
     pl.tile_rows = sc.get<uint32_t>((uint64_t)pl.ntiles + 1);
     tile_walk_kernel<<<grid_for(ncb, 128), 128, 0, s>>>(tmp_rows, ncb_p, ncb, r1, row_off, cap, max_rows, cb_cnt, nullptr, pl.tile_rows);
     return pl;
@@ -91,12 +87,14 @@
     Scratch sc;
     TilePlan p0;
     uint32_t max_rows = 0;
-    uint64_t *hoff = nullptr, *hscan_tmp = nullptr, *blkbase = nullptr, *hbase = nullptr, *vbase = nullptr, *cellbase = nullptr;
+    uint64_t *hoff = nullptr, *blkbase = nullptr, *hbase = nullptr, *vbase = nullptr, *cellbase = nullptr;
     uint8_t *hbits = nullptr, *hmode = nullptr;
     uint32_t *nstretch = nullptr;
     uint64_t nh = 0, nblocks = 0, nvirt = 0, ncell = 0;
     uint64_t mode_rows[3] = {0, 0, 0}, mode_partials[3] = {0, 0, 0};
-    uint32_t *ghist = nullptr, *ghist_tmp = nullptr;
+    uint32_t *ghist = nullptr;
+    ScanState ghist_scan{};
+    uint32_t *abort_word = nullptr;
     Part<T> *qstage = nullptr;
     uint64_t *vrow_off = nullptr;
     uint8_t *vfirst = nullptr;
@@ -145,8 +143,8 @@
     if (!pl.p0.nlong) return;
     const uint32_t nlong = pl.p0.nlong;
     pl.hoff = sc.get<uint64_t>((uint64_t)nlong + 1);
-    pl.hscan_tmp = sc.get<uint64_t>(scan_scratch_entries(nlong));
-    device_exclusive_scan<HeavyLen, uint64_t>(HeavyLen{pl.p0.long_rows, row_off}, nlong, pl.hoff, pl.hscan_tmp, s);
+    ScanPhase ph_len(sc, s, {nlong});
+    device_scan_chained<HeavyLen, uint64_t>(HeavyLen{pl.p0.long_rows, row_off}, nlong, pl.hoff, ph_len.take(nlong), s);
     pl.hbits = sc.get<uint8_t>(nlong);
     pl.hmode = sc.get<uint8_t>(nlong);
     pl.nstretch = sc.get<uint32_t>(nlong);
@@ -185,15 +183,18 @@
                                                                  hub_b, direct_fine, ds ? nrund : nullptr, hsmall, ds ? small_lim : SmallLimits{});
         zero_async(s, {{totals, 7 * sizeof(uint64_t)}});
         mode_totals_kernel<<<std::min(grid_for(nlong, 256), 64u), 256, 0, s>>>(pl.p0.long_rows, nlong, row_off, pl.hmode, hsmall, totals);
-        device_exclusive_scan<LoadU32As64, uint64_t>(LoadU32As64{pl.nstretch}, nlong, pl.blkbase, pl.hscan_tmp, s);
-        device_exclusive_scan<LoadU32As64, uint64_t>(LoadU32As64{nseg}, nlong, pl.vbase, pl.hscan_tmp, s);
-        device_exclusive_scan<LoadU64, uint64_t>(LoadU64{nhist}, nlong, pl.hbase, pl.hscan_tmp, s);
-        if (ds) device_exclusive_scan<LoadU64, uint64_t>(LoadU64{ncellh}, nlong, pl.cellbase, pl.hscan_tmp, s);
-        if (ds && nrund) device_exclusive_scan<LoadU64, uint64_t>(LoadU64{nrund}, nlong, rdbase, pl.hscan_tmp, s);
+        ScanPhase ph(sc, s, {nlong, nlong, nlong, nlong, nlong});
+        device_scan_chained<LoadU32As64, uint64_t>(LoadU32As64{pl.nstretch}, nlong, pl.blkbase, ph.take(nlong), s);
+        device_scan_chained<LoadU32As64, uint64_t>(LoadU32As64{nseg}, nlong, pl.vbase, ph.take(nlong), s);
+        device_scan_chained<LoadU64, uint64_t>(LoadU64{nhist}, nlong, pl.hbase, ph.take(nlong), s);
+        if (ds) device_scan_chained<LoadU64, uint64_t>(LoadU64{ncellh}, nlong, pl.cellbase, ph.take(nlong), s);
+        if (ds && nrund) device_scan_chained<LoadU64, uint64_t>(LoadU64{nrund}, nlong, rdbase, ph.take(nlong), s);
         ndcell = 0;
         nrd = 0;
         {
             Gather g(s);
+            ph.watch(g);
+            if (attempt == 0) ph_len.watch(g);
             g.add(&pl.nh, (const uint64_t *)pl.hoff + nlong); g.add(&pl.nblocks, (const uint64_t *)pl.blkbase + nlong);
             g.add(&pl.nvirt, (const uint64_t *)pl.vbase + nlong); g.add(&pl.ncell, (const uint64_t *)pl.hbase + nlong);
             if (ds) g.add(&ndcell, (const uint64_t *)pl.cellbase + nlong);
@@ -201,6 +202,8 @@
             for (int i = 0; i < 6; i++) g.add(&tot[i], (const uint64_t *)totals + i);
             g.add(&nsmall, (const uint64_t *)totals + 6);
             g.wait();
+            ph.check();
+            ph_len.check();
         }
         if (ds && ndcell >= 0xffffffffull) { ds = nullptr; hub_b = 0; continue; }
         if (hub_possible && !hub_decided && hub_b == 0 && pl.nblocks && (double)tot[3 + kModeStretch] >= hub_min_share * (double)count) {
@@ -224,7 +227,7 @@
                 (unsigned long long)r0, (unsigned long long)r1, pl.p0.ntiles, nlong, (unsigned long long)pl.nh, (unsigned long long)pl.nvirt,
                 (unsigned long long)pl.mode_rows[kModeDirect], (unsigned long long)pl.mode_partials[kModeDirect], (unsigned long long)ndcell);
     pl.ghist = sc.get<uint32_t>(pl.ncell + 1);
-    pl.ghist_tmp = sc.get<uint32_t>(scan_scratch_entries(pl.ncell + 1));
+    { ScanPhase ph_split(sc, s, {pl.ncell}, pl.abort_word); pl.ghist_scan = ph_split.take(pl.ncell); }
     pl.vrow_off = sc.get<uint64_t>(pl.nvirt + 1);
     pl.vfirst = sc.get<uint8_t>(pl.nvirt + 1);
     pl.vcol0 = sc.get<uint32_t>(pl.nvirt + 1);
@@ -305,13 +308,12 @@
             uint8_t *rowstart = tmp.get<uint8_t>(nb + 4);
             uint32_t *sx = keep.get<uint32_t>(nb + 1), *runstart = keep.get<uint32_t>(nb + 1);
             uint16_t *runblk = keep.get<uint16_t>(nb + 2);
-            uint32_t *scan_tmp = tmp.get<uint32_t>(scan_scratch_entries(nb + 1));
+            ScanPhase ph_runs(tmp, s, {nb}, pl.abort_word);
             OSP_HIP(hipMemsetAsync(rowstart, 0, nb + 4, s));
             hub_rowstart_kernel<<<grid_for(ds->K, 256), 256, 0, s>>>(ds->b_rowptr, ds->K, rowstart);
             const int sh = colbits - hub_b;
             const HubRunFlag flag{rowstart, ds->b_colidx, sh};
-            device_exclusive_scan<HubRunFlag, uint32_t>(flag, nb, sx, scan_tmp, s);
-            compact_flagged_kernel<HubRunFlag><<<grid_for(nb, 256), 256, 0, s>>>(flag, sx, nb, 0, runstart);
+            device_scan_compact<HubRunFlag>(flag, nb, 0, runstart, nullptr, ph_runs.take(nb), s, sx);
             hub_runstart_end_kernel<<<1, 1, 0, s>>>(sx + nb, runstart, (uint32_t)nb);
             OSP_HIP(hipMemsetAsync(runblk, 0, (nb + 2) * sizeof(uint16_t), s));
             hub_runblk_kernel<<<std::min(grid_for(nb, 256), 4096u), 256, 0, s>>>(sx + nb, runstart, ds->b_colidx, sh, runblk);
@@ -320,14 +322,14 @@
         }
         tm.begin(PH_HUB_K, s);
         uint64_t *jobruns = sc.get<uint64_t>(pl.nblocks + 1);
-        uint64_t *jobscan_tmp = sc.get<uint64_t>(scan_scratch_entries(pl.nblocks + 1));
+        ScanPhase ph_hub(sc, s, {pl.ncell, pl.nblocks});
         const size_t hub_lds = sizeof(uint32_t) << hub_b;
         hub_plan_kernel<false><<<(unsigned)pl.nblocks, kHubThreads, hub_lds, s>>>(pl.p0.long_rows, nlong, pl.blkbase, pl.hbase, pl.hbits, pl.nstretch, row_off,
                                                                            ds->rowfirst, ds->off, ds->bs, ds->perm, ds->b_colidx, ds->hub, pl.ghist,
                                                                            pl.hoff, jobruns, nullptr, nullptr, nullptr);
-        device_exclusive_scan<LoadU32, uint32_t>(LoadU32{pl.ghist}, pl.ncell, pl.ghist, pl.ghist_tmp, s);
-        device_exclusive_scan<LoadU64, uint64_t>(LoadU64{jobruns}, pl.nblocks, jobruns, jobscan_tmp, s);
-        const uint64_t ncells = d2h(jobruns + pl.nblocks, s);
+        device_scan_chained<LoadU32, uint32_t>(LoadU32{pl.ghist}, pl.ncell, pl.ghist, ph_hub.take(pl.ncell), s);
+        device_scan_chained<LoadU64, uint64_t>(LoadU64{jobruns}, pl.nblocks, jobruns, ph_hub.take(pl.nblocks), s);
+        const uint64_t ncells = ph_hub.fetch((const uint64_t *)jobruns + pl.nblocks, s);
         if (ncells >= (1ull << 40)) throw Error(OSP_ERR_CAPACITY, "hub rows: too many runs in one panel");
         if (getenv("OSP_VERBOSE"))
             fprintf(stderr, "[osp]   hub rows: %llu rows, %llu products in %llu runs (%.2f records per run), %llu jobs, 2^%d blocks\n",
@@ -369,8 +371,9 @@
                     (unsigned long long)pl.mode_partials[kModeStretch], pl.split_from_b ? (pl.split_beside ? "from B" : "from B, after the join") : "from staged records");
         if (rows_x) {
             pl.xjobbase = sc.get<uint64_t>((uint64_t)nlong + 1);
-            device_exclusive_scan<ExpandJobs, uint64_t>(ExpandJobs{pl.p0.long_rows, row_off, pl.hmode, kModeSplitRow, stretch_x ? kModeStretch : kModeSplitRow},
-                                                        nlong, pl.xjobbase, pl.hscan_tmp, s);
+            ScanPhase ph_x(sc, s, {nlong}, pl.abort_word);
+            device_scan_chained<ExpandJobs, uint64_t>(ExpandJobs{pl.p0.long_rows, row_off, pl.hmode, kModeSplitRow, stretch_x ? kModeStretch : kModeSplitRow},
+                                                      nlong, pl.xjobbase, ph_x.take(nlong), s);
             pl.xjobs_bound = pl.xpartials / kExpandJob + rows_x;
         }
     }
@@ -386,7 +389,7 @@
     const RowSrc<T> src{ds->rowfirst, ds->off, ds->bs, perm, (const T *)ds->a_vals, ds->b_colidx, (const T *)ds->b_vals};
     split_count_kernel<true><<<(unsigned)pl.nblocks, kSplitThreads, 0, s>>>(p0.long_rows, nlong, pl.blkbase, pl.hbase, pl.hbits, pl.nstretch, row_off, base, colbits,
                                                                           nullptr, 0u, pl.ghist, cols);
-    device_exclusive_scan<LoadU32, uint32_t>(LoadU32{pl.ghist}, pl.ncell, pl.ghist, pl.ghist_tmp, s);
+    device_scan_chained<LoadU32, uint32_t>(LoadU32{pl.ghist}, pl.ncell, pl.ghist, pl.ghist_scan, s);
     OSP_WITH_RA(ctx, split_scatter_kernel<T, RA, true><<<(unsigned)pl.nblocks, kSplitThreads, 0, s>>>(
                          p0.long_rows, nlong, pl.blkbase, pl.hbase, pl.hbits, pl.nstretch, row_off, base, colbits, nullptr, pl.ghist, pl.hoff, pl.qstage, src));
     split_vrows_kernel<<<grid_for(pl.nvirt + 1, 256), 256, 0, s>>>(nlong, pl.vbase, pl.hbase, pl.nstretch, pl.hbits, pl.hmode, colbits, pl.ghist, pl.hoff, pl.nvirt,
@@ -418,9 +421,9 @@
     Part<T> *qstage = pl.qstage;
     if (p0.nlong) {
         const uint32_t nlong = p0.nlong;
-        uint64_t *hoff = pl.hoff, *hscan_tmp = pl.hscan_tmp, *blkbase = pl.blkbase, *hbase = pl.hbase;
+        uint64_t *hoff = pl.hoff, *blkbase = pl.blkbase, *hbase = pl.hbase;
         uint8_t *hbits = pl.hbits;
-        uint32_t *nstretch = pl.nstretch, *ghist = pl.ghist, *ghist_tmp = pl.ghist_tmp;
+        uint32_t *nstretch = pl.nstretch, *ghist = pl.ghist;
         const uint64_t nh = pl.nh, nblocks = pl.nblocks, nvirt = pl.nvirt, ncell = pl.ncell;
         uint64_t *vrow_off = pl.vrow_off;
         uint8_t *vfirst = pl.vfirst;
@@ -437,7 +440,7 @@
         if (nblocks && !pl.hub.cells && !pl.split_from_b) {
             split_count_kernel<<<(unsigned)nblocks, kSplitThreads, 0, s>>>(p0.long_rows, nlong, blkbase, hbase, hbits, nstretch, io.row_off,
                                                                          base, colbits, (const char *)io.stage, (uint32_t)sizeof(Part<T>), ghist);
-            device_exclusive_scan<LoadU32, uint32_t>(LoadU32{ghist}, ncell, ghist, ghist_tmp, s);
+            device_scan_chained<LoadU32, uint32_t>(LoadU32{ghist}, ncell, ghist, pl.ghist_scan, s);
             OSP_WITH_RA(ctx, split_scatter_kernel<T, RA><<<(unsigned)nblocks, kSplitThreads, 0, s>>>(
                                  p0.long_rows, nlong, blkbase, hbase, hbits, nstretch, io.row_off, base, colbits, io.stage, ghist, hoff, qstage));
         }
@@ -458,8 +461,8 @@
             lv.heavy_nnz[1] = seg_nnz;
             if (pl.ga.runs) {
                 uint64_t *xsjob = sc.get<uint64_t>((uint64_t)nseg_long + 1);
-                uint64_t *xsjob_tmp = sc.get<uint64_t>(scan_scratch_entries((uint64_t)nseg_long + 1));
-                device_exclusive_scan<SegExpandJobs, uint64_t>(SegExpandJobs{p1.long_rows, vrow_off, pl.vrun_off}, nseg_long, xsjob, xsjob_tmp, s);
+                ScanPhase ph_xs(sc, s, {nseg_long}, io.abort_word);
+                device_scan_chained<SegExpandJobs, uint64_t>(SegExpandJobs{p1.long_rows, vrow_off, pl.vrun_off}, nseg_long, xsjob, ph_xs.take(nseg_long), s);
                 const uint64_t job_bound = nh / kExpandJob + nseg_long;
                 expand_segments_kernel<T><<<(unsigned)std::min<uint64_t>(job_bound, (uint64_t)ctx->cus * 8), kExpandThreads, 0, s>>>(
                     p1.long_rows, nseg_long, xsjob, vrow_off, pl.vrun_off, pl.vrun_end, pl.ga.runs, pl.ga.b_colidx, pl.ga.b_vals, qstage);
@@ -467,11 +470,11 @@
             const uint32_t *rest_list = p1.long_rows;
             uint32_t nrest = nseg_long;
             uint32_t *hscan = sc.get<uint32_t>((uint64_t)nseg_long + 1);
-            uint64_t *sscan_tmp = sc.get<uint64_t>(scan_scratch_entries(nseg_long));
             {
                 const SegDenseFlag df{p1.long_rows, pl.vcol0, pl.vcol1, getenv("OSP_DENSE_SEG") ? atoi(getenv("OSP_DENSE_SEG")) : 1};
-                device_exclusive_scan<SegDenseFlag, uint32_t>(df, nseg_long, hscan, (uint32_t *)sscan_tmp, s);
-                const uint32_t ndense = d2h(hscan + nseg_long, s);
+                ScanPhase ph(sc, s, {nseg_long});
+                device_scan_chained<SegDenseFlag, uint32_t>(df, nseg_long, hscan, ph.take(nseg_long), s);
+                const uint32_t ndense = ph.fetch((const uint32_t *)hscan + nseg_long, s);
                 if (ndense) {
                     uint32_t *dense_list = sc.get<uint32_t>(ndense), *others = sc.get<uint32_t>(nseg_long - ndense);
                     seg_split_list_kernel<SegDenseFlag><<<grid_for(nseg_long, 256), 256, 0, s>>>(df, hscan, nseg_long, dense_list, others);
@@ -493,8 +496,9 @@
             uint32_t *huge_list = nullptr, *mid_list = nullptr;
             if (nrest) {
                 const SegHugeFlag hf{rest_list, vrow_off, big_cap};
-                device_exclusive_scan<SegHugeFlag, uint32_t>(hf, nrest, hscan, (uint32_t *)sscan_tmp, s);
-                nhuge = d2h(hscan + nrest, s);
+                ScanPhase ph(sc, s, {nrest});
+                device_scan_chained<SegHugeFlag, uint32_t>(hf, nrest, hscan, ph.take(nrest), s);
+                nhuge = ph.fetch((const uint32_t *)hscan + nrest, s);
                 nmid = nrest - nhuge;
                 huge_list = sc.get<uint32_t>(nhuge);
                 mid_list = sc.get<uint32_t>(nmid);
@@ -514,8 +518,9 @@
             dbg_sync(s, "over-long segments: big in-place tiles");
             if (nhuge) {
                 uint64_t *soff = sc.get<uint64_t>((uint64_t)nhuge + 1);
-                device_exclusive_scan<HeavyLen, uint64_t>(HeavyLen{huge_list, vrow_off}, nhuge, soff, sscan_tmp, s);
-                const uint64_t ns = d2h(soff + nhuge, s);
+                ScanPhase ph(sc, s, {nhuge});
+                device_scan_chained<HeavyLen, uint64_t>(HeavyLen{huge_list, vrow_off}, nhuge, soff, ph.take(nhuge), s);
+                const uint64_t ns = ph.fetch((const uint64_t *)soff + nhuge, s);
                 res->info.sorted_partials += ns;
                 SortedRuns runs(sc, ns);
                 heavy_fill_kernel<<<grid_for(ns, 256), 256, 0, s>>>(huge_list, soff, nhuge, vrow_off, 0, colbits, (const char *)qstage,
@@ -535,7 +540,8 @@
         uint32_t *j0 = sc.get<uint32_t>(nlong), *tb = sc.get<uint32_t>((uint64_t)nlong + 1), *extra = sc.get<uint32_t>((uint64_t)nlong + 1);
         chain_rows_kernel<<<grid_for(nlong + 1, 256), 256, 0, s>>>(p0.long_rows, nlong, p0.tile_rows, p0.ntiles, vbase, p1.tile_rows,
                                                                   p1.ntiles, j0, tb, extra);
-        device_exclusive_scan<LoadU32, uint32_t>(LoadU32{extra}, nlong, extra, (uint32_t *)hscan_tmp, s);
+        ScanPhase ph_chain(sc, s, {nlong}, io.abort_word);
+        device_scan_chained<LoadU32, uint32_t>(LoadU32{extra}, nlong, extra, ph_chain.take(nlong), s);
         ntot = p0.ntiles + (p1.ntiles - nlong);
         desc = sc.get<TileDesc>(ntot);
         tile_desc_kernel<(int)kCap><<<grid_for(p0.ntiles, 256), 256, 0, s>>>(p0.tile_rows, p0.ntiles, r1, io.row_off, base, 0u, j0, extra,
@@ -646,7 +652,8 @@
                            const uint64_t *d_row_off,
                            uint64_t P, uint64_t cap_cfg, PhaseTimer &tm, uint64_t r_lo = 0, uint64_t r_hi = ~0ull,
                            uint64_t off_lo = 0, const PanelSink *sink = nullptr, const ChunkTable<T> *ct = nullptr,
-                           const DirectSrc *ds = nullptr, const std::vector<uint64_t> *cuts = nullptr, const ShortRuns<T> *sr = nullptr) {
+                           const DirectSrc *ds = nullptr, const std::vector<uint64_t> *cuts = nullptr, const ShortRuns<T> *sr = nullptr,
+                           ScanPhase *ph_before = nullptr) {
     if (r_hi == ~0ull) r_hi = M_all;
     const uint64_t M = r_hi - r_lo;
     res->info.M = M;
@@ -661,18 +668,28 @@
     uint64_t *ub = sc.get<uint64_t>(M + 1);
     {
         Scratch us(ctx);
-        uint64_t *ub_tmp = us.get<uint64_t>(scan_scratch_entries(M + 1));
-        if (P != 0) device_exclusive_scan<RowUpperBound, uint64_t>(RowUpperBound{d_row_off + r_lo, N}, M, ub, ub_tmp, s);
+        ScanPhase ph(us, s, {P != 0 ? M : 0});
+        if (P != 0) device_scan_chained<RowUpperBound, uint64_t>(RowUpperBound{d_row_off + r_lo, N}, M, ub, ph.take(M), s);
         if (P == 0) {
             cap_c = 0;
         } else if (P == kPartialsOnDevice) {
             Gather g(s);
             g.add(&P, d_row_off + M_all);
             g.add(&cap_c, (const uint64_t *)ub + M);
+            ph.watch(g);
+            if (ph_before) ph_before->watch(g);
             g.wait();
+            ph.check();
+            if (ph_before) ph_before->check();
             res->info.partials = P;
         } else {
-            cap_c = d2h(ub + M, s);
+            Gather g(s);
+            g.add(&cap_c, (const uint64_t *)ub + M);
+            ph.watch(g);
+            if (ph_before) ph_before->watch(g);
+            g.wait();
+            ph.check();
+            if (ph_before) ph_before->check();
         }
     }
     if (!sink) res->rowptr = (int64_t *)ctx->alloc((M + 1) * sizeof(int64_t));
@@ -762,6 +779,7 @@
         const uint64_t r0 = bounds[p], r1 = bounds[p + 1];
         const uint64_t base = panel_base(p), count = panel_count(p);
         PlanPtr pl(new PanelPlan<T>(ctx));
+        pl->abort_word = abort_word;
         if (beside) {
             AuxScope scope(ctx);
             OSP_HIP(hipStreamWaitEvent(ctx->stream, ctx->aux_fork, 0));
diff --git a/outerspace_amd/csrc/osp_prims.h b/outerspace_amd/csrc/osp_prims.h
--- a/outerspace_amd/csrc/osp_prims.h
+++ b/outerspace_amd/csrc/osp_prims.h
@@ -292,6 +292,231 @@
     const uint32_t *p;
     __device__ uint32_t operator()(uint64_t i) const { return p[i]; }
 };
+
+constexpr uint64_t kStatusAgg = 1ull << 62, kStatusPrefix = 2ull << 62, kStatusMask = (1ull << 62) - 1;
+constexpr int kLookWin = 1;
+__device__ __forceinline__ void lookback_publish(uint64_t *status, uint32_t t, uint64_t total) {
+    __hip_atomic_store(&status[t], (t == 0 ? kStatusPrefix : kStatusAgg) | total, __ATOMIC_RELAXED, __HIP_MEMORY_SCOPE_AGENT);
+}
+constexpr uint32_t kLookbackSpinLimit = 1u << 22;
+template <bool PUBLISH = true>
+__device__ __forceinline__ uint64_t lookback_prefix(uint64_t *status, uint32_t t, uint64_t total, uint32_t *abort_word = nullptr) {
+    const unsigned lane = lane_id();
+    if (PUBLISH && lane == 0) lookback_publish(status, t, total);
+    uint64_t excl = 0;
+    int64_t b = (int64_t)t - 1;
+    uint32_t spins = 0;
+    while (b >= 0) {
+        uint64_t sv[kLookWin];
+#pragma unroll
+        for (int j = 0; j < kLookWin; j++) {
+            const int64_t idx = b - (int64_t)(j * kWave) - (int64_t)lane;
+            sv[j] = kStatusPrefix;
+            if (idx >= 0) sv[j] = __hip_atomic_load(&status[idx], __ATOMIC_RELAXED, __HIP_MEMORY_SCOPE_AGENT);
+        }
+        bool done = false, retry = false;
+        uint64_t part = 0;
+#pragma unroll
+        for (int j = 0; j < kLookWin; j++) {
+            if (!done && !retry) {
+                const uint64_t m_prefix = __ballot((sv[j] >> 62) == 2), m_empty = __ballot((sv[j] >> 62) == 0);
+                const int p = m_prefix ? __builtin_ctzll(m_prefix) : 64;
+                const uint64_t need = p >= 63 ? ~0ull : ((2ull << p) - 1ull);
+                if (m_empty & need) {
+                    retry = true;
+                } else {
+                    part += ((int)lane <= p) ? (sv[j] & kStatusMask) : 0ull;
+                    if (p < 64) done = true;
+                }
+            }
+        }
+        if (retry) {
+            __builtin_amdgcn_s_sleep(1);
+            if (abort_word && (++spins & 255u) == 0) {
+                if (spins >= kLookbackSpinLimit && lane == 0) atomicExch(abort_word, 1u);
+                if (spins >= kLookbackSpinLimit || __hip_atomic_load(abort_word, __ATOMIC_RELAXED, __HIP_MEMORY_SCOPE_AGENT) != 0u) break;
+            }
+            continue;
+        }
+        excl += wave_reduce_sum_u62(part);
+        if (done) break;
+        b -= (int64_t)kLookWin * kWave;
+    }
+    if (lane == 0 && t != 0)
+        __hip_atomic_store(&status[t], kStatusPrefix | (excl + total), __ATOMIC_RELAXED, __HIP_MEMORY_SCOPE_AGENT);
+    return excl;
+}
+
+constexpr int kChainThreads = 256;
+constexpr int kChainItems = 16;
+constexpr int kChainTile = kChainThreads * kChainItems;
+constexpr int kChainItemsLong = 32;
+constexpr uint64_t kChainLongMin = 1ull << 20;
+constexpr uint64_t kChainHead = 16;
+constexpr uint64_t kChainSmallMax = kScanSmallTiles * kScanTile;
+constexpr int kChainSmallThreads = 1024, kChainSmallItems = 8;
+constexpr int kChainTinyThreads = 256;
+struct ScanState {
+    uint64_t *words = nullptr;
+    uint32_t *err = nullptr;
+};
+inline uint64_t scan_chained_words(uint64_t n, uint64_t tile = kChainTile) {
+    if (n <= kChainSmallMax) return 0;
+    return kChainHead + ((n + tile - 1) / tile + 15) / 16 * 16;
+}
+
+template <class T> struct Vec16;
+template <> struct Vec16<uint32_t> { typedef uint32_t type __attribute__((ext_vector_type(4))); };
+template <> struct Vec16<uint64_t> { typedef uint64_t type __attribute__((ext_vector_type(2))); };
+template <class E, class TOut, int ITEMS>
+__device__ __forceinline__ bool scan_load_wide_ptr(const E *p, TOut (&v)[ITEMS]) {
+    typedef typename Vec16<E>::type V;
+    constexpr int W = 16 / (int)sizeof(E);
+    static_assert(ITEMS % W == 0, "a thread's entries are whole 16-byte words");
+    if ((uintptr_t)p & 15u) return false;
+    V x[ITEMS / W];
+#pragma unroll
+    for (int k = 0; k < ITEMS / W; k++) x[k] = reinterpret_cast<const V *>(p)[k];
+#pragma unroll
+    for (int k = 0; k < ITEMS / W; k++)
+#pragma unroll
+        for (int j = 0; j < W; j++) v[k * W + j] = (TOut)x[k][j];
+    return true;
+}
+template <class F, class TOut, int ITEMS>
+__device__ __forceinline__ bool scan_load_wide(const F &, uint64_t, TOut (&)[ITEMS]) { return false; }
+template <class TOut, int ITEMS>
+__device__ __forceinline__ bool scan_load_wide(const LoadU32 &f, uint64_t i0, TOut (&v)[ITEMS]) { return scan_load_wide_ptr(f.p + i0, v); }
+
+template <class F, class TOut, int ITEMS>
+__device__ __forceinline__ void scan_load_items(const F &f, uint64_t i0, uint64_t n, TOut (&v)[ITEMS]) {
+    if (i0 + ITEMS <= n) {
+        if (scan_load_wide(f, i0, v)) return;
+#pragma unroll
+        for (int i = 0; i < ITEMS; i++) v[i] = (TOut)f(i0 + i);
+    } else {
+#pragma unroll
+        for (int i = 0; i < ITEMS; i++) v[i] = i0 + i < n ? (TOut)f(i0 + i) : (TOut)0;
+    }
+}
+template <bool COMPACT, class TOut, int ITEMS>
+__device__ __forceinline__ void scan_store_items(TOut *out, uint64_t i0, uint64_t n, TOut ex, const TOut (&v)[ITEMS], uint64_t r0, uint32_t *list) {
+    TOut o[ITEMS];
+#pragma unroll
+    for (int i = 0; i < ITEMS; i++) {
+        o[i] = ex;
+        ex += v[i];
+    }
+    if (COMPACT) {
+#pragma unroll
+        for (int i = 0; i < ITEMS; i++)
+            if (v[i] != 0 && i0 + i < n) list[o[i]] = (uint32_t)(r0 + i0 + i);
+        if (!out) return;
+    }
+    typedef typename Vec16<TOut>::type V;
+    constexpr int W = 16 / (int)sizeof(TOut);
+    if (i0 + ITEMS <= n && ((uintptr_t)(out + i0) & 15u) == 0) {
+#pragma unroll
+        for (int k = 0; k < ITEMS / W; k++) {
+            V x;
+#pragma unroll
+            for (int j = 0; j < W; j++) x[j] = o[k * W + j];
+            reinterpret_cast<V *>(out + i0)[k] = x;
+        }
+    } else {
+#pragma unroll
+        for (int i = 0; i < ITEMS; i++)
+            if (i0 + i < n) out[i0 + i] = o[i];
+    }
+}
+
+template <class F, class TOut, int ITEMS, bool COMPACT>
+__global__ __launch_bounds__(kChainThreads) void scan_chained_kernel(F f, uint64_t n, TOut *out, uint64_t *state, uint32_t *err, uint64_t r0,
+                                                                     uint32_t *list, TOut *count) {
+    constexpr uint64_t kTile = (uint64_t)kChainThreads * ITEMS;
+    __shared__ TOut scratch[kChainThreads / kWave + 1];
+    __shared__ uint32_t s_tile;
+    __shared__ uint64_t s_excl;
+    if (threadIdx.x == 0) s_tile = atomicAdd(reinterpret_cast<uint32_t *>(state), 1u);
+    __syncthreads();
+    const uint32_t t = s_tile;
+    const uint64_t i0 = (uint64_t)t * kTile + (uint64_t)threadIdx.x * ITEMS;
+    TOut v[ITEMS];
+    scan_load_items(f, i0, n, v);
+    TOut s = 0;
+#pragma unroll
+    for (int i = 0; i < ITEMS; i++) s += v[i];
+    TOut total;
+    TOut ex = block_excl_scan<TOut, kChainThreads>(s, scratch, &total);
+    if (threadIdx.x < kWave) {
+        const uint64_t excl = lookback_prefix(state + kChainHead, t, (uint64_t)total, err);
+        if (threadIdx.x == 0) s_excl = excl;
+    }
+    __syncthreads();
+    const TOut excl = (TOut)s_excl;
+    scan_store_items<COMPACT>(out, i0, n, (TOut)(ex + excl), v, r0, list);
+    if (threadIdx.x == 0 && (uint64_t)(t + 1) * kTile >= n) {
+        if (out) out[n] = excl + total;
+        if (count) *count = excl + total;
+    }
+}
+
+template <class F, class TOut, bool COMPACT, int NT>
+__global__ __launch_bounds__(NT) void scan_chained_small_kernel(F f, uint64_t n, TOut *out, uint64_t r0, uint32_t *list, TOut *count) {
+    constexpr int ITEMS = kChainSmallItems;
+    constexpr uint64_t kPass = (uint64_t)NT * ITEMS;
+    __shared__ TOut scratch[NT / kWave + 1];
+    TOut carry = 0;
+    TOut v[ITEMS];
+    scan_load_items(f, (uint64_t)threadIdx.x * ITEMS, n, v);
+    for (uint64_t base = 0; base < n; base += kPass) {
+        const uint64_t i0 = base + (uint64_t)threadIdx.x * ITEMS;
+        TOut nx[ITEMS];
+        scan_load_items(f, i0 + kPass, n, nx);
+        TOut s = 0;
+#pragma unroll
+        for (int i = 0; i < ITEMS; i++) s += v[i];
+        TOut total;
+        const TOut ex = block_excl_scan<TOut, NT>(s, scratch, &total) + carry;
+        scan_store_items<COMPACT>(out, i0, n, ex, v, r0, list);
+        carry += total;
+#pragma unroll
+        for (int i = 0; i < ITEMS; i++) v[i] = nx[i];
+    }
+    if (threadIdx.x == 0) {
+        if (out) out[n] = carry;
+        if (count) *count = carry;
+    }
+}
+
+template <class F, class TOut, bool COMPACT, int ITEMS = 0>
+inline void launch_scan_chained(F f, uint64_t n, TOut *out, ScanState st, uint64_t r0, uint32_t *list, TOut *count, hipStream_t stream) {
+    if (n <= (uint64_t)kChainTinyThreads * kChainSmallItems) {
+        scan_chained_small_kernel<F, TOut, COMPACT, kChainTinyThreads><<<1, kChainTinyThreads, 0, stream>>>(f, n, out, r0, list, count);
+        return;
+    }
+    if (n <= kChainSmallMax) {
+        scan_chained_small_kernel<F, TOut, COMPACT, kChainSmallThreads><<<1, kChainSmallThreads, 0, stream>>>(f, n, out, r0, list, count);
+        return;
+    }
+    if (ITEMS == 0) {
+        if (n >= kChainLongMin) launch_scan_chained<F, TOut, COMPACT, kChainItemsLong>(f, n, out, st, r0, list, count, stream);
+        else launch_scan_chained<F, TOut, COMPACT, kChainItems>(f, n, out, st, r0, list, count, stream);
+        return;
+    }
+    constexpr int kItems = ITEMS ? ITEMS : kChainItems;
+    const uint64_t ntiles = (n + (uint64_t)kChainThreads * kItems - 1) / ((uint64_t)kChainThreads * kItems);
+    scan_chained_kernel<F, TOut, kItems, COMPACT><<<(unsigned)ntiles, kChainThreads, 0, stream>>>(f, n, out, st.words, st.err, r0, list, count);
+}
+template <class F, class TOut>
+inline void device_scan_chained(F f, uint64_t n, TOut *out, ScanState st, hipStream_t stream) {
+    launch_scan_chained<F, TOut, false>(f, n, out, st, 0, nullptr, (TOut *)nullptr, stream);
+}
+template <class F>
+inline void device_scan_compact(F flag, uint64_t n, uint64_t r0, uint32_t *list, uint32_t *count, ScanState st, hipStream_t stream,
+                                uint32_t *scan_out = nullptr) {
+    launch_scan_chained<F, uint32_t, true>(flag, n, scan_out, st, r0, list, count, stream);
+}
 
 inline uint64_t sort_blocks(uint64_t n) { return (n + kSortTile - 1) / kSortTile; }
 inline uint64_t sort_hist_entries(uint64_t n) { return sort_blocks(n) * kRadix + 1; }
diff --git a/outerspace_amd/csrc/osp_split.h b/outerspace_amd/csrc/osp_split.h
--- a/outerspace_amd/csrc/osp_split.h
+++ b/outerspace_amd/csrc/osp_split.h
@@ -104,6 +104,8 @@
     const uint32_t *p;
     __device__ uint64_t operator()(uint64_t i) const { return p[i]; }
 };
+template <class TOut, int ITEMS>
+__device__ __forceinline__ bool scan_load_wide(const LoadU32As64 &f, uint64_t i0, TOut (&v)[ITEMS]) { return scan_load_wide_ptr(f.p + i0, v); }
 
 struct SplitJob {
     uint32_t h, st, b, nst;
```

Result: no change. 70.03 billion (median of 6 runs) (+0.6%).
